# lunarlab-gatech/MorphSym-HGNN

Hardware: NVIDIA B200
Metric: train-step graphs/s (MS-HGNN K4 Mini Cheetah contact, H=128, L=8, fwd+loss+bwd+allreduce+Adam) (higher is better)
Workload: dtype f16x2-split (f32 accumulate)

## Files before the change

include/mshgnn_b200.h:

```cpp
#ifndef MSHGNN_B200_H
#define MSHGNN_B200_H

#include <stdint.h>

#ifdef __cplusplus
extern "C" {
#endif

#define MSHGNN_MAX_NODE_TYPES 4
#define MSHGNN_MAX_EDGE_TYPES 16

#define MSHGNN_OK              0
#define MSHGNN_ERR_ARG        -1
#define MSHGNN_ERR_CUDA       -2
#define MSHGNN_ERR_WORKSPACE  -3

#define MSHGNN_F32 0
#define MSHGNN_F64 1
#define MSHGNN_I64 2
#define MSHGNN_F16 3

#define MSHGNN_MODE_FP32   0
#define MSHGNN_MODE_TC     1
#define MSHGNN_MODE_TC_1X  2

#define MSHGNN_LOSS_MSE 0
#define MSHGNN_LOSS_CE2 1

#define MSHGNN_P_ENC_W   0
#define MSHGNN_P_ENC_B   1
#define MSHGNN_P_REL_W   2
#define MSHGNN_P_REL_B   3
#define MSHGNN_P_ROOT_W  4
#define MSHGNN_P_MLP_W   5
#define MSHGNN_P_MLP_B   6
#define MSHGNN_P_DEC_W   7
#define MSHGNN_P_DEC_B   8

typedef struct mshgnn_plan mshgnn_plan;

typedef struct mshgnn_desc {
    int32_t n_node_types;
    int32_t nodes_per_graph[MSHGNN_MAX_NODE_TYPES];
    int32_t in_width[MSHGNN_MAX_NODE_TYPES];
    int32_t n_edge_types;
    int32_t edge_src_type[MSHGNN_MAX_EDGE_TYPES];
    int32_t edge_dst_type[MSHGNN_MAX_EDGE_TYPES];
    int32_t edge_mean[MSHGNN_MAX_EDGE_TYPES];
    int32_t edge_count[MSHGNN_MAX_EDGE_TYPES];
    const int32_t* edge_src[MSHGNN_MAX_EDGE_TYPES];
    const int32_t* edge_dst[MSHGNN_MAX_EDGE_TYPES];
    int32_t hidden;
    int32_t num_layers;
    int32_t morph_sym;
    int32_t mlp_type;
    int32_t decode_type;
    int32_t out_channels;
    const float* in_sign[MSHGNN_MAX_NODE_TYPES];
    const float* out_sign;
} mshgnn_desc;

int  mshgnn_plan_create(const mshgnn_desc* desc, mshgnn_plan** plan_out);
#define MSHGNN_PLAN_PAD_HIDDEN 1
int  mshgnn_plan_create_ex(const mshgnn_desc* desc, int32_t flags, mshgnn_plan** plan_out);
void mshgnn_plan_destroy(mshgnn_plan* plan);

int64_t mshgnn_param_count(const mshgnn_plan* plan);
int  mshgnn_param_offset(const mshgnn_plan* plan, int32_t kind, int32_t layer, int32_t idx,
                         int64_t* offset_out, int64_t* numel_out);

int64_t mshgnn_workspace_bytes(const mshgnn_plan* plan, int64_t B, int32_t train, int32_t mode);
int64_t mshgnn_out_rows(const mshgnn_plan* plan, int64_t B);

int mshgnn_forward(const mshgnn_plan* plan, int64_t B,
                   const void* const* x, int32_t x_dtype,
                   const float* params, float* out,
                   void* workspace, int64_t workspace_bytes,
                   int32_t train, int32_t mode, void* stream);

int mshgnn_loss(const mshgnn_plan* plan, int64_t B, int32_t loss_kind,
                const float* out, const void* labels, int32_t label_dtype,
                float loss_scale, float* loss_out, float* dout,
                void* workspace, int64_t workspace_bytes, void* stream);

int mshgnn_backward(const mshgnn_plan* plan, int64_t B,
                    const void* const* x, int32_t x_dtype,
                    const float* params, const float* dout, float* grads,
                    void* workspace, int64_t workspace_bytes,
                    int32_t mode, void* stream);

int mshgnn_backward_staged(const mshgnn_plan* plan, int64_t B,
                           const void* const* x, int32_t x_dtype,
                           const float* params, const float* dout, float* grads,
                           void* workspace, int64_t workspace_bytes,
                           int32_t mode, void* stream, void* layers_ready_event);

int mshgnn_input_grad(const mshgnn_plan* plan, int64_t B, const float* params, float* const* dx,
                      void* workspace, int64_t workspace_bytes, int32_t mode, void* stream);

int mshgnn_adam_step(float* params, const float* grads, float* exp_avg, float* exp_avg_sq,
                     int64_t n, int64_t step, float lr, float beta1, float beta2, float eps,
                     float weight_decay, void* stream);
int mshgnn_sgd_step(float* params, const float* grads, int64_t n, float lr, void* stream);

typedef struct mshgnn_window_desc {
    int32_t history_length;
    int32_t seq_cols;
    int32_t label_cols;
    int32_t n_node_types;
    int32_t nodes_per_graph[MSHGNN_MAX_NODE_TYPES];
    int32_t blocks_per_node[MSHGNN_MAX_NODE_TYPES];
    int32_t block_len[MSHGNN_MAX_NODE_TYPES];
    int32_t normalize;
    int32_t n_labels;
    const int32_t* block_col;
    const int32_t* block_sign;
    const int32_t* label_col;
    const int32_t* label_sign;
} mshgnn_window_desc;

int mshgnn_build_windows(const mshgnn_window_desc* desc, const void* seq, const void* label_seq, int32_t seq_dtype,
                         int64_t n_rows, const int64_t* starts, int64_t B, float* const* x, float* y, void* stream);

#define MSHGNN_METRIC_SLOTS   32
#define MSHGNN_METRIC_SCRATCH (296 * 32)
int mshgnn_step_metrics(int32_t loss_kind, int64_t n, int32_t feet, const float* out, const void* labels, int32_t label_dtype,
                        double* batch, double* epoch, double* scratch, void* stream);

#define MSHGNN_METRIC_COM       2
#define MSHGNN_METRIC_GRF_WORLD 3
typedef struct {
    int32_t n_base;
    const double* y_mean;
    const double* y_std;
    const void* quat;
    int32_t quat_dtype;
    int32_t z_only;
} mshgnn_metric_args;
int mshgnn_step_metrics_ex(int32_t kind, const mshgnn_metric_args* args, int64_t n, const float* out, const void* labels,
                           int32_t label_dtype, double* batch, double* epoch, double* scratch, void* stream);

int64_t mshgnn_plan_describe(const mshgnn_plan* plan, char* buf, int64_t cap);

#define MSHGNN_NUM_KERNEL_KINDS 21
int mshgnn_profile_enable(int32_t on);
int mshgnn_profile_read(double* ms_out, int64_t* launches_out, int32_t n);
const char* mshgnn_kernel_kind_name(int32_t kind);

int mshgnn_relu_mask_offset(const mshgnn_plan* plan, int64_t B, int32_t mode, int32_t layer,
                            int64_t* byte_off, int64_t* n_slots, int64_t* rows_padded);

int64_t mshgnn_dw_layout(const mshgnn_plan* plan, int64_t B, int32_t mode, int32_t* out, int64_t cap);

int mshgnn_check_edges(const mshgnn_plan* plan, int64_t B, const int64_t* const* edge_index, int32_t* flag, void* stream);

int mshgnn_set_option(const char* name, int32_t value);
int32_t mshgnn_get_option(const char* name);
int mshgnn_stack_status(const mshgnn_plan* plan, int64_t B, int32_t train, int32_t mode, const void* workspace, int32_t* status_out);
int64_t mshgnn_stack_timing_offset(const mshgnn_plan* plan, int64_t B, int32_t train, int32_t mode);

int64_t mshgnn_launch_count(void);
const char* mshgnn_last_error(void);
const char* mshgnn_version(void);

#ifdef __cplusplus
}
#endif
#endif
```

morphsym-hgnn_b200/csrc/api.cu:

```cuda
#include <algorithm>
#include <atomic>
#include <cmath>
#include <cstdarg>
#include <cstdio>
#include <cstdlib>
#include <cstring>
#include <mutex>
#include <new>
#include <vector>

#include "kernels_simt.cuh"
#include "kernels_tc.cuh"
#include "kernels_enc.cuh"
#include "kernels_dx.cuh"
#include "kernels_stack.cuh"
#include "kernels_stack2.cuh"
#include "kernels_pad.cuh"
#include "plan.cuh"
#include "windows.cuh"
#include "metrics.cuh"

using namespace mshgnn;

struct mshgnn_plan {
    Plan p;
};

namespace {

thread_local char g_err[512] = "";
std::atomic<long long> g_launches{0};

int fail(int code, const char* fmt, ...) {
    va_list ap;
    va_start(ap, fmt);
    vsnprintf(g_err, sizeof g_err, fmt, ap);
    va_end(ap);
    return code;
}

#define CUDA_TRY(expr)                                                                     \
    do {                                                                                   \
        cudaError_t _e = (expr);                                                           \
        if (_e != cudaSuccess)                                                             \
            return fail(MSHGNN_ERR_CUDA, "%s failed: %s (%s:%d)", #expr, cudaGetErrorString(_e), __FILE__, __LINE__); \
    } while (0)

enum Kind : int { K_DERIVE = 0, K_ENC_FWD, K_CONV_FWD, K_MLP_FWD, K_DEC_FWD, K_LOSS, K_DEC_BWD, K_MLP_BWD, K_DX_BWD,
                  K_DW_LAYER, K_DW_ENC, K_REDUCE, K_OPTIM, K_MEMSET, K_WINDOWS, K_METRICS, K_STACK_FWD, K_STACK_BWD, K_EDGES, K_DX_ENC, K_PAD, K_NKINDS };
static_assert(K_NKINDS == MSHGNN_NUM_KERNEL_KINDS, "kernel kind table out of sync with the header");
constexpr int K_NKINDS_V1 = 19;
const char* const kKindNames[MSHGNN_NUM_KERNEL_KINDS] = {
    "derive_weights", "encoder_fwd", "conv_fwd", "base_mlp_fwd", "decoder_fwd", "loss",
    "decoder_bwd", "base_mlp_bwd", "dx_bwd", "dw_layers", "dw_encoder",
    "reduce_partials", "optimizer", "memset", "window_builder", "step_metrics", "stack_fwd", "stack_bwd", "check_edges", "dx_encoder", "pad_params"};
struct ProfRec { int kind; cudaEvent_t a, b; };
std::mutex g_prof_mu;
bool g_prof_on = false;
std::vector<ProfRec> g_prof;
std::vector<cudaEvent_t> g_prof_pool;

struct ProfScope {
    cudaStream_t st; cudaEvent_t a = nullptr, b = nullptr; int kind; bool on;
    ProfScope(int k, cudaStream_t s) : st(s), kind(k), on(g_prof_on) {
        if (!on) return;
        std::lock_guard<std::mutex> lk(g_prof_mu);
        auto get = [&]() { cudaEvent_t e; if (!g_prof_pool.empty()) { e = g_prof_pool.back(); g_prof_pool.pop_back(); } else cudaEventCreate(&e); return e; };
        a = get(); b = get();
        cudaEventRecord(a, st);
    }
    ~ProfScope() {
        if (!on) return;
        cudaEventRecord(b, st);
        std::lock_guard<std::mutex> lk(g_prof_mu);
        g_prof.push_back({kind, a, b});
    }
};

#define LAUNCH_CHECK()                                                                     \
    do {                                                                                   \
        g_launches.fetch_add(1, std::memory_order_relaxed);                                \
        cudaError_t _e = cudaGetLastError();                                               \
        if (_e != cudaSuccess)                                                             \
            return fail(MSHGNN_ERR_CUDA, "kernel launch failed: %s (%s:%d)", cudaGetErrorString(_e), __FILE__, __LINE__); \
    } while (0)

template <typename T>
int upload(const Plan& p, const std::vector<T>& v, T** d) {
    *d = nullptr;
    if (v.empty()) return 0;
    CUDA_TRY(cudaMalloc((void**)d, v.size() * sizeof(T)));
    p.d_allocs.push_back(*d);
    CUDA_TRY(cudaMemcpy(*d, v.data(), v.size() * sizeof(T), cudaMemcpyHostToDevice));
    return 0;
}

int ensure_uploaded(const Plan& p) {
    std::lock_guard<std::mutex> lk(p.mu);
    int dev = -1;
    CUDA_TRY(cudaGetDevice(&dev));
    if (p.uploaded) {
        if (dev != p.device) return fail(MSHGNN_ERR_ARG, "plan tables live on device %d but the current device is %d", p.device, dev);
        return 0;
    }
    int rc;
    if ((rc = upload(p, p.tiles, &p.d_tiles))) return rc;
    if ((rc = upload(p, p.stack_items, &p.d_stack_items))) return rc;
    {
        std::vector<int> tpl;
        for (int e = 0; e < p.n_etypes; ++e) { tpl.insert(tpl.end(), p.e_src[e].begin(), p.e_src[e].end()); tpl.insert(tpl.end(), p.e_dst[e].begin(), p.e_dst[e].end()); }
        if (tpl.empty()) tpl.push_back(0);
        if ((rc = upload(p, tpl, &p.d_edge_tpl))) return rc;
    }
    if ((rc = upload(p, p.rtasks, &p.d_rtasks))) return rc;
    if ((rc = upload(p, p.rpairs, &p.d_rpairs))) return rc;
    if ((rc = upload(p, p.groups, &p.d_groups))) return rc;
    if ((rc = upload(p, p.derive_ops, &p.d_derive))) return rc;
    if ((rc = upload(p, p.derive16_ops, &p.d_derive16))) return rc;
    if ((rc = upload(p, p.signs, &p.d_signs))) return rc;
    if ((rc = upload(p, p.enc_units, &p.d_enc_units))) return rc;
    if ((rc = upload(p, p.enc_groups, &p.d_enc_groups))) return rc;
    if ((rc = upload(p, p.dx_units, &p.d_dx_units))) return rc;
    if ((rc = upload(p, p.pad_segs, &p.d_pad_segs))) return rc;
    p.device = dev;
    p.uploaded = true;
    return 0;
}

void fill_bufs(const Plan& p, const WsLayout& w, char* ws, BufTable& bt) {
    for (int id = 0; id < MAX_BUFS; ++id) bt.p[id] = w.buf[id] < 0 ? nullptr : ws + w.buf[id];
    bt.p[BUF_SIGNS] = p.d_signs;
}

void fill_rows16(const WsLayout& w, BufRows& br) {
    auto row = [](int64_t off) { return off < 0 ? 0 : (int)(off / 256); };
    for (int id = 0; id < MAX_BUFS; ++id) { br.hi[id] = row(w.buf16[id][0]); br.lo[id] = row(w.buf16[id][1]); }
    br.w_hi = row(w.w16[0]); br.w_lo = row(w.w16[1]);
}

__half* image16(char* ws, const WsLayout& w, int id, int i) { return w.buf16[id][i] < 0 ? nullptr : (__half*)(ws + w.buf16[id][i]); }

int launch_rowgemm(int kind, const Plan& p, const Launch& L, const BufTable& bt, int64_t B, int64_t Bp, int x_f64, cudaStream_t st) {
    if (L.count == 0) return 0;
    ProfScope ps(kind, st);
    dim3 grid((unsigned)(Bp / TILE_M), (unsigned)L.count);
    k_rowgemm<<<grid, 256, 0, st>>>(p.d_tiles + L.begin, bt, B, Bp, x_f64);
    LAUNCH_CHECK();
    return 0;
}

typedef CUresult (*EncodeTiledFn)(CUtensorMap*, CUtensorMapDataType, cuuint32_t, void*, const cuuint64_t*, const cuuint64_t*,
                                  const cuuint32_t*, const cuuint32_t*, CUtensorMapInterleave, CUtensorMapSwizzle,
                                  CUtensorMapL2promotion, CUtensorMapFloatOOBfill);

int encode_map(CUtensorMap* m, CUtensorMapDataType type, cuuint32_t rank, const void* base, const cuuint64_t* dims, const cuuint64_t* strides,
               const cuuint32_t* box, CUtensorMapSwizzle sw, const char* what) {
    static EncodeTiledFn enc = nullptr;
    if (!enc) {
        void* ptr = nullptr;
        cudaDriverEntryPointQueryResult qres;
        CUDA_TRY(cudaGetDriverEntryPoint("cuTensorMapEncodeTiled", &ptr, cudaEnableDefault, &qres));
        if (qres != cudaDriverEntryPointSuccess || !ptr) return fail(MSHGNN_ERR_CUDA, "cuTensorMapEncodeTiled is not available in this driver");
        enc = (EncodeTiledFn)ptr;
    }
    static thread_local bool ctx_bound = false;
    if (!ctx_bound) { CUDA_TRY(cudaFree(0)); ctx_bound = true; }
    const cuuint32_t estr[3] = {1, 1, 1};
    CUresult r = enc(m, type, rank, const_cast<void*>(base), dims, strides, box, estr, CU_TENSOR_MAP_INTERLEAVE_NONE,
                     sw, CU_TENSOR_MAP_L2_PROMOTION_L2_256B, CU_TENSOR_MAP_FLOAT_OOB_FILL_NONE);
    if (r != CUDA_SUCCESS) return fail(MSHGNN_ERR_CUDA, "cuTensorMapEncodeTiled%s failed with CUresult %d", what, (int)r);
    return 0;
}

int make_map_2d(CUtensorMap* m, const void* base, int64_t rows, int64_t cols, int box_cols, int box_rows, CUtensorMapSwizzle sw) {
    if (!base || rows < 1) return fail(MSHGNN_ERR_ARG, "internal: bad fp16 tensor for a TMA map");
    const cuuint64_t dims[2] = {(cuuint64_t)cols, (cuuint64_t)rows};
    const cuuint64_t strides[1] = {(cuuint64_t)cols * 2};
    const cuuint32_t box[2] = {(cuuint32_t)box_cols, (cuuint32_t)box_rows};
    return encode_map(m, CU_TENSOR_MAP_DATA_TYPE_FLOAT16, 2, base, dims, strides, box, sw, "");
}

int make_map_x3d(CUtensorMap* m, const void* base, int64_t B, int nodes, int K, int box_rows = 128, int box_cols = 64,
                 CUtensorMapSwizzle sw = CU_TENSOR_MAP_SWIZZLE_NONE) {
    const cuuint64_t dims[3] = {(cuuint64_t)K, (cuuint64_t)nodes, (cuuint64_t)B};
    const cuuint64_t strides[2] = {(cuuint64_t)K * 4, (cuuint64_t)nodes * K * 4};
    const cuuint32_t box[3] = {(cuuint32_t)box_cols, 1, (cuuint32_t)box_rows};
    return encode_map(m, CU_TENSOR_MAP_DATA_TYPE_FLOAT32, 3, base, dims, strides, box, sw, " (features)");
}

struct WsMaps {
    TcMaps tc;
    CUtensorMap dw;
};
int make_ws_maps(WsMaps* m, const void* ws, const WsLayout& w) {
    if (w.total / 256 > 0x7fffffffLL) return fail(MSHGNN_ERR_ARG, "workspace too large for one TMA map");
    int rc;
    if ((rc = make_map_2d(&m->tc.k, ws, w.total / 256, H, TC_KB, 128, CU_TENSOR_MAP_SWIZZLE_64B))) return rc;
    if ((rc = make_map_2d(&m->tc.o, ws, w.total / 256, H, 64, 128, CU_TENSOR_MAP_SWIZZLE_128B))) return rc;
    if ((rc = make_map_2d(&m->dw, ws, w.total / 256, H, 64, DW_KB, CU_TENSOR_MAP_SWIZZLE_128B))) return rc;
    return 0;
}

constexpr int MAX_DEVICES = 64;
int sm_count(int* out) {
    static std::atomic<int> n[MAX_DEVICES];
    int dev = 0;
    CUDA_TRY(cudaGetDevice(&dev));
    int v = dev < MAX_DEVICES ? n[dev].load(std::memory_order_relaxed) : 0;
    if (!v) {
        CUDA_TRY(cudaDeviceGetAttribute(&v, cudaDevAttrMultiProcessorCount, dev));
        if (dev < MAX_DEVICES) n[dev].store(v, std::memory_order_relaxed);
    }
    *out = v;
    return 0;
}
bool first_on_device(std::atomic<bool> (&flags)[MAX_DEVICES]) {
    int dev = 0;
    if (cudaGetDevice(&dev) != cudaSuccess || dev < 0 || dev >= MAX_DEVICES) return true;
    return !flags[dev].exchange(true);
}

static std::atomic<int> g_encoder_kernel{-1}, g_encoder_tpi{0}, g_encoder_dw_tma{-1};

int launch_tc_encoder(const Plan& p, const Launch& L, const WsLayout& w, const BufTable& bt, const BufRows& br, const WsMaps& wm, char* ws,
                      const float* params, int64_t B, int xf64, int split, cudaStream_t st) {
    if (L.count == 0) return 0;
    static std::atomic<bool> attr_set[64];
    static const int which_env = [] { const char* e = getenv("MSHGNN_ENCODER"); return !e ? 0 : (!strcmp(e, "v1") ? 1 : (!strcmp(e, "pair") ? 2 : 0)); }();
    const int which = g_encoder_kernel.load() >= 0 ? g_encoder_kernel.load() : which_env;
    if (first_on_device(attr_set)) {
        CUDA_TRY(cudaFuncSetAttribute(k_tc_encoder, cudaFuncAttributeMaxDynamicSharedMemorySize, ENC_SMEM_BYTES));
        CUDA_TRY(cudaFuncSetAttribute(k_tc_encoder_pair, cudaFuncAttributeMaxDynamicSharedMemorySize, ENCP_SMEM_BYTES));
        CUDA_TRY(cudaFuncSetAttribute(k_tc_encoder_stream, cudaFuncAttributeMaxDynamicSharedMemorySize, ENQ_SMEM_BYTES));
    }
    __half* e_hi = (__half*)(ws + w.wenc16[0]);
    __half* e_lo = (__half*)(ws + w.wenc16[1]);
    EncMaps maps;
    int rc;
    if ((rc = make_map_2d(&maps.w_hi, e_hi, (int64_t)p.n_types * H, p.enc_kmax, 64, 128, CU_TENSOR_MAP_SWIZZLE_128B))) return rc;
    if ((rc = make_map_2d(&maps.w_lo, e_lo, (int64_t)p.n_types * H, p.enc_kmax, 64, 128, CU_TENSOR_MAP_SWIZZLE_128B))) return rc;
    maps.o = wm.tc.o;
    bool stream_ok = xf64 == 0 && L.count <= ENQ_MAX_SLOTS;
    for (int i = 0; i < L.count && stream_ok; ++i) {
        const Chunk& ch = p.tiles[L.begin + i].chunks[0];
        stream_ok = ch.a_buf >= BUF_X0 && ch.a_buf < BUF_X0 + p.n_types && enq_rows_ok(bt.p[ch.a_buf], ch.K, ch.sign_off);
    }
    ProfScope ps(K_ENC_FWD, st);
    const unsigned n_row_tiles = (unsigned)(w.Bp / TILE_M);
    if (which == 1) k_tc_encoder<<<dim3(n_row_tiles, (unsigned)L.count), ENC_THREADS, ENC_SMEM_BYTES, st>>>(maps, p.d_tiles + L.begin, bt, br, B, w.Bp, xf64, split);
    else if (which == 2 || !stream_ok) {
        static const int pf = [] { const char* e = getenv("MSHGNN_ENC_PREFETCH"); return e ? atoi(e) : 0; }();
        k_tc_encoder_pair<<<dim3((n_row_tiles + 1) / 2, (unsigned)L.count), ENC_THREADS, ENCP_SMEM_BYTES, st>>>(maps, p.d_tiles + L.begin, bt, br, B, w.Bp, xf64, split, pf);
    } else {
        int n_sm = 0;
        if ((rc = sm_count(&n_sm))) return rc;
        static const int force_tpi = [] { const char* e = getenv("MSHGNN_ENC_TPI"); return e ? atoi(e) : 0; }();
        const int opt_tpi = g_encoder_tpi.load() ? g_encoder_tpi.load() : force_tpi;
        const int tpi = opt_tpi == 1 || opt_tpi == 2 ? opt_tpi : ((int64_t)L.count * ((n_row_tiles + 1) / 2) >= 4 * (int64_t)n_sm ? 2 : 1);
        const int64_t n_items = (int64_t)L.count * ((n_row_tiles + tpi - 1) / tpi);
        const unsigned grid = (unsigned)(n_items < n_sm ? n_items : n_sm);
        static const int pf_kb = [] { const char* e = getenv("MSHGNN_ENC_PF"); return e ? atoi(e) : 0; }();
        static const int dbg = [] { const char* e = getenv("MSHGNN_ENC_DEBUG"); return e ? atoi(e) : 0; }();
        EnqMaps em;
        em.w_hi = maps.w_hi; em.w_lo = maps.w_lo; em.o = maps.o;
        for (int t = 0; t < p.n_types; ++t) {
            if (p.in_w[t] % 4 || (reinterpret_cast<uintptr_t>(bt.p[BUF_X0 + t]) & 15)) { em.x[t] = maps.o; continue; }
            if ((rc = make_map_x3d(&em.x[t], bt.p[BUF_X0 + t], B, p.nodes[t], p.in_w[t]))) return rc;
        }
        for (int t = p.n_types; t < 4; ++t) em.x[t] = maps.o;
        k_tc_encoder_stream<<<grid, ENQ_THREADS, ENQ_SMEM_BYTES, st>>>(em, p.d_tiles + L.begin, L.count, (int)BUF_X0, bt, br, B, w.Bp, split, (uint32_t*)(ws + w.enc_sync), tpi, pf_kb, dbg);
    }
    LAUNCH_CHECK();
    return 0;
}

int launch_tc_rowgemm(int kind, const Plan& p, const Launch& L, const BufTable& bt, const BufRows& br, const WsMaps& wm,
                      int64_t B, int64_t Bp, int split, cudaStream_t st) {
    if (L.count == 0) return 0;
    static std::atomic<bool> attr_set[64];
    static const bool use_v2 = [] { const char* e = getenv("MSHGNN_ROWGEMM"); return e && !strcmp(e, "tile"); }();
    static const bool use_single = [] { const char* e = getenv("MSHGNN_ROWGEMM"); return e && !strcmp(e, "single"); }();
    if (first_on_device(attr_set)) {
        CUDA_TRY(cudaFuncSetAttribute(k_tc_rowgemm, cudaFuncAttributeMaxDynamicSharedMemorySize, TC_SMEM_BYTES));
        CUDA_TRY(cudaFuncSetAttribute(k_tc_rowgemm_persistent, cudaFuncAttributeMaxDynamicSharedMemorySize, PK_SMEM_BYTES));
        CUDA_TRY(cudaFuncSetAttribute(k_tc_rowgemm_pair, cudaFuncAttributeMaxDynamicSharedMemorySize, PP_SMEM_BYTES));
    }
    for (int i = 0; i < L.count; ++i)
        for (int c = 0; c < p.tiles[L.begin + i].n_chunks; ++c)
            if (p.tiles[L.begin + i].chunks[c].a_kind != A_SLAB)
                return fail(MSHGNN_ERR_ARG, "internal: a tensor-core row-GEMM launch must read slab buffers");
    ProfScope ps(kind, st);
    if (use_v2 || L.count > PK_MAX_TILES) {
        dim3 grid((unsigned)L.count, (unsigned)(Bp / TILE_M));
        k_tc_rowgemm<<<grid, TC_THREADS, TC_SMEM_BYTES, st>>>(wm.tc, p.d_tiles + L.begin, bt, br, B, Bp, split);
    } else {
        int n_sm = 0, rc;
        if ((rc = sm_count(&n_sm))) return rc;
        const bool pair = !use_single && Bp >= 2 * TILE_M && (int64_t)L.count * ((Bp / TILE_M + 1) / 2) >= 4 * (int64_t)n_sm;
        const int64_t n_items = (int64_t)L.count * (pair ? (Bp / TILE_M + 1) / 2 : Bp / TILE_M);
        if (n_items > 0x7fffffffLL) return fail(MSHGNN_ERR_ARG, "batch too large for one row-GEMM launch");
        const unsigned grid = (unsigned)(n_items < n_sm ? n_items : n_sm);
        cudaLaunchConfig_t cfg = {};
        cfg.gridDim = dim3(grid); cfg.blockDim = dim3(PK_THREADS); cfg.dynamicSmemBytes = pair ? PP_SMEM_BYTES : PK_SMEM_BYTES; cfg.stream = st;
        cudaLaunchAttribute at[1];
        at[0].id = cudaLaunchAttributeProgrammaticStreamSerialization;
        at[0].val.programmaticStreamSerializationAllowed = g_prof_on ? 0 : 1;
        cfg.attrs = at; cfg.numAttrs = 1;
        const Tile* d_tiles = p.d_tiles + L.begin;
        const int n_tiles = L.count, n_it = (int)n_items;
        if (pair) CUDA_TRY(cudaLaunchKernelEx(&cfg, k_tc_rowgemm_pair, wm.tc, d_tiles, n_tiles, n_it, bt, br, B, Bp, split));
        else CUDA_TRY(cudaLaunchKernelEx(&cfg, k_tc_rowgemm_persistent, wm.tc, d_tiles, n_tiles, n_it, bt, br, B, Bp, split));
    }
    LAUNCH_CHECK();
    return 0;
}

int launch_tc_dw(int kind, const Plan& p, int layer, const Launch& L, const WsLayout& w, const BufRows& br, const WsMaps& wm, int64_t B, int split,
                 float* part_w, float* part_b, cudaStream_t st) {
    if (L.count == 0) return 0;
    static std::atomic<bool> attr_set[64];
    if (first_on_device(attr_set)) CUDA_TRY(cudaFuncSetAttribute(k_tc_reducegemm, cudaFuncAttributeMaxDynamicSharedMemorySize, DW_SMEM_BYTES));
    for (int i = 0; i < L.count; ++i) {
        const RTask& T = p.rtasks[L.begin + i];
        if (T.n_pairs > DW_MAX_PAIRS) return fail(MSHGNN_ERR_ARG, "internal: weight-gradient task with more than %d pairs", DW_MAX_PAIRS);
        for (int j = 0; j < T.n_pairs; ++j)
            if (p.rpairs[T.pair_begin + j].a_kind != A_SLAB) return fail(MSHGNN_ERR_ARG, "internal: tensor-core weight-gradient task must read slabs");
    }
    ProfScope ps(kind, st);
    dim3 grid((unsigned)L.count, (unsigned)w.dw_ns[layer]);
    k_tc_reducegemm<<<grid, TC_THREADS, DW_SMEM_BYTES, st>>>(wm.dw, p.d_rtasks, p.d_rpairs, L.begin, br, B, w.Bp, w.dw_rows[layer], w.dw_slot0[layer],
                                                             split, part_w, part_b);
    LAUNCH_CHECK();
    return 0;
}

int stack_rows_per_chunk(const Plan& p) {
    static const int env = [] { const char* e = getenv("MSHGNN_STACK_RC"); return e ? atoi(e) : 0; }();
    if (env > 0) return env;
    const int64_t per_row_tile = (int64_t)2 * p.S * TILE_M * H * 4;
    int rc = (int)((int64_t)84 * 1024 * 1024 / per_row_tile);
    return rc < 16 ? 16 : (rc > 64 ? 64 : rc);
}
int stack_delay(const Plan::Stack& sp, int n_row_tiles, int n_sm) {
    static const int env = [] { const char* e = getenv("MSHGNN_STACK_DELAY"); return e ? atoi(e) : 0; }();
    if (env > 0) return env;
    const int per_slot = sp.prog.items_per_row > 0 ? sp.prog.items_per_row : 1;
    int d = (4 * n_sm + per_slot - 1) / per_slot;
    const int most = n_row_tiles / (sp.prog.n_phases > 0 ? sp.prog.n_phases : 1);
    if (d > most) d = most;
    return d < 1 ? 1 : d;
}

int stack_sync_reset(const WsLayout& w, char* ws, cudaStream_t st) {
    if (!w.stack) return 0;
    ProfScope ps(K_MEMSET, st);
    CUDA_TRY(cudaMemsetAsync(ws + w.stack_sync, 0, (size_t)w.stack_sync_bytes, st));
    return 0;
}

int launch_stack(int kind, const Plan& p, const Plan::Stack& sp, const WsLayout& w, const BufTable& bt, const BufRows& br, const WsMaps& wm,
                 char* ws, int64_t B, int split, cudaStream_t st) {
    if (sp.prog.n_phases == 0) return 0;
    static std::atomic<bool> attr_set[64];
    static const bool timing = [] { const char* e = getenv("MSHGNN_STACK_TIMING"); return e && !strcmp(e, "1"); }();
    if (first_on_device(attr_set)) {
        CUDA_TRY(cudaFuncSetAttribute(k_tc_stack<false, false>, cudaFuncAttributeMaxDynamicSharedMemorySize, SK_SMEM_BYTES));
        CUDA_TRY(cudaFuncSetAttribute(k_tc_stack<true, false>, cudaFuncAttributeMaxDynamicSharedMemorySize, SK_SMEM_BYTES));
        CUDA_TRY(cudaFuncSetAttribute(k_tc_stack<false, true>, cudaFuncAttributeMaxDynamicSharedMemorySize, SK_SMEM_BYTES));
        CUDA_TRY(cudaFuncSetAttribute(k_tc_stack<true, true>, cudaFuncAttributeMaxDynamicSharedMemorySize, SK_SMEM_BYTES));
    }
    bool has_priv = false;
    for (int i = 0; i < sp.tiles.count; ++i) {
        const Tile& T = p.tiles[sp.tiles.begin + i];
        has_priv = has_priv || T.priv != 0;
        for (int c = 0; c < T.n_chunks; ++c)
            if (T.chunks[c].a_kind != A_SLAB) return fail(MSHGNN_ERR_ARG, "internal: a stack program must read slab buffers");
    }
    int n_prog_items = 0;
    for (int ph = 0; ph < sp.prog.n_phases; ++ph) n_prog_items = std::max(n_prog_items, sp.prog.first_item[ph] + sp.prog.n_items[ph]);
    for (int i = 0; i < n_prog_items; ++i) {
        const StackItem& it = p.stack_items[sp.item0 + i];
        int chunks = 0;
        for (int st_ = 0; st_ < it.n_steps; ++st_) chunks += p.tiles[sp.tiles.begin + it.tile + st_].n_chunks;
        if (chunks > SK_QCHUNKS || it.n_steps > SK_QSTEPS) return fail(MSHGNN_ERR_ARG, "internal: stack item with %d chunks / %d steps (queue holds %d / %d)", chunks, it.n_steps, SK_QCHUNKS, SK_QSTEPS);
    }
    StackArgs a;
    a.prog = sp.prog;
    a.n_row_tiles = (int)(w.Bp / TILE_M);
    const int64_t n_total = (int64_t)a.n_row_tiles * sp.prog.items_per_row;
    if (n_total > 0x7fffffffLL) return fail(MSHGNN_ERR_ARG, "batch too large for one stack launch");
    a.n_total = (int)n_total;
    a.split = split; a.B = B; a.Bp = w.Bp; a.n_slots = p.S;
    a.sync = (uint32_t*)(ws + w.stack_sync);
    a.err = (uint32_t*)(ws + w.stack_sync + w.stack_sync_bytes - 4);
    a.next = (uint32_t*)(ws + w.stack_sync + w.stack_sync_bytes - 8);
    a.timing = (unsigned long long*)(ws + w.stack_timing);
    a.ws = ws;
    static const int env_dbg = [] { const char* e = getenv("MSHGNN_STACK_DEBUG"); return e ? atoi(e) : 0; }();
    a.debug = env_dbg;
    if ((int64_t)sp.prog.n_phases * a.n_row_tiles * p.S + 2 > w.stack_sync_bytes / 4) return fail(MSHGNN_ERR_WORKSPACE, "internal: stack counters do not fit");
    int n_sm = 0, rc;
    if ((rc = sm_count(&n_sm))) return rc;
    static const bool chunked = [] { const char* e = getenv("MSHGNN_STACK_ORDER"); return !(e && !strcmp(e, "diag")); }();
    static const int env_la = [] { const char* e = getenv("MSHGNN_STACK_LOOKAHEAD"); return e ? atoi(e) : 0; }();
    a.lookahead = env_la > 0 ? (env_la > 4 ? 4 : env_la) : 1;
    a.chunked = chunked ? 1 : 0;
    a.delay = chunked ? stack_rows_per_chunk(p) : stack_delay(sp, a.n_row_tiles, n_sm);
    if (w.stack_pair && !timing) {
        if (a.n_row_tiles & 1) return fail(MSHGNN_ERR_ARG, "internal: the CTA-pair stack kernel needs an even number of row tiles");
        static std::atomic<bool> attr2_set[64];
        static std::atomic<int> max_clusters[64];
        int dev = 0;
        CUDA_TRY(cudaGetDevice(&dev));
        if (first_on_device(attr2_set)) {
            CUDA_TRY(cudaFuncSetAttribute(k_tc_stack2<false>, cudaFuncAttributeMaxDynamicSharedMemorySize, S2_SMEM_BYTES));
            CUDA_TRY(cudaFuncSetAttribute(k_tc_stack2<true>, cudaFuncAttributeMaxDynamicSharedMemorySize, S2_SMEM_BYTES));
        }
        const int64_t n_pairs_total = (int64_t)(a.n_row_tiles / 2) * sp.prog.items_per_row;
        a.n_total = (int)n_pairs_total;
        if (a.chunked) { a.delay = a.delay / 2; if (a.delay < 1) a.delay = 1; }
        else a.delay = stack_delay(sp, a.n_row_tiles / 2, n_sm / 2);
        cudaLaunchConfig_t cfg = {};
        cfg.blockDim = dim3(SK_THREADS); cfg.dynamicSmemBytes = S2_SMEM_BYTES; cfg.stream = st;
        cudaLaunchAttribute at[2];
        at[0].id = cudaLaunchAttributeClusterDimension;
        at[0].val.clusterDim.x = 2; at[0].val.clusterDim.y = 1; at[0].val.clusterDim.z = 1;
        at[1].id = cudaLaunchAttributeProgrammaticStreamSerialization;
        at[1].val.programmaticStreamSerializationAllowed = g_prof_on ? 0 : 1;
        cfg.attrs = at; cfg.numAttrs = 2;
        int mc = dev < 64 ? max_clusters[dev].load(std::memory_order_relaxed) : 0;
        if (!mc) {
            cfg.gridDim = dim3((unsigned)n_sm);
            CUDA_TRY(cudaOccupancyMaxActiveClusters(&mc, k_tc_stack2<true>, &cfg));
            if (mc < 1) return fail(MSHGNN_ERR_CUDA, "the CTA-pair stack kernel does not fit on this device (0 active clusters)");
            if (dev < 64) max_clusters[dev].store(mc, std::memory_order_relaxed);
        }
        const int64_t clusters = n_pairs_total < mc ? n_pairs_total : mc;
        cfg.gridDim = dim3((unsigned)(2 * clusters));
        const Tile* d_tiles = p.d_tiles + sp.tiles.begin;
        const StackItem* d_items = p.d_stack_items + sp.item0;
        ProfScope ps(kind, st);
        if (has_priv) CUDA_TRY(cudaLaunchKernelEx(&cfg, k_tc_stack2<true>, wm.tc, wm.dw, d_tiles, d_items, a, bt, br));
        else CUDA_TRY(cudaLaunchKernelEx(&cfg, k_tc_stack2<false>, wm.tc, wm.dw, d_tiles, d_items, a, bt, br));
        LAUNCH_CHECK();
        return 0;
    }
    ProfScope ps(kind, st);
    cudaLaunchConfig_t cfg = {};
    cfg.gridDim = dim3((unsigned)(n_total < n_sm ? n_total : n_sm)); cfg.blockDim = dim3(SK_THREADS); cfg.dynamicSmemBytes = SK_SMEM_BYTES; cfg.stream = st;
    cudaLaunchAttribute at[1];
    at[0].id = cudaLaunchAttributeProgrammaticStreamSerialization;
    at[0].val.programmaticStreamSerializationAllowed = g_prof_on ? 0 : 1;
    cfg.attrs = at; cfg.numAttrs = 1;
    const Tile* d_tiles = p.d_tiles + sp.tiles.begin;
    const StackItem* d_items = p.d_stack_items + sp.item0;
    if (timing && has_priv) CUDA_TRY(cudaLaunchKernelEx(&cfg, k_tc_stack<true, true>, wm.tc, d_tiles, d_items, a, bt, br));
    else if (timing) CUDA_TRY(cudaLaunchKernelEx(&cfg, k_tc_stack<true, false>, wm.tc, d_tiles, d_items, a, bt, br));
    else if (has_priv) CUDA_TRY(cudaLaunchKernelEx(&cfg, k_tc_stack<false, true>, wm.tc, d_tiles, d_items, a, bt, br));
    else CUDA_TRY(cudaLaunchKernelEx(&cfg, k_tc_stack<false, false>, wm.tc, d_tiles, d_items, a, bt, br));
    LAUNCH_CHECK();
    return 0;
}

int compact_grads(const Plan& p, int first, int count, const float* in, float* ext, cudaStream_t st) {
    if (count == 0) return 0;
    ProfScope ps(K_PAD, st);
    k_compact_grads<<<dim3(PAD_BLOCKS_X, (unsigned)count), 256, 0, st>>>(p.d_pad_segs + first, in, ext);
    LAUNCH_CHECK();
    return 0;
}

float grad_scale(const Plan& p, int64_t B) {
    int e = 0;
    std::frexp((double)(B * p.dec.n_dec), &e);
    return (float)std::ldexp(1.0, e - 1);
}

int check_plan_mode(const mshgnn_plan* plan, int32_t mode) {
    if (!plan) return fail(MSHGNN_ERR_ARG, "plan is NULL");
    if (mode != MSHGNN_MODE_FP32 && mode != MSHGNN_MODE_TC && mode != MSHGNN_MODE_TC_1X) return fail(MSHGNN_ERR_ARG, "unknown mode %d", mode);
    return 0;
}

struct Call {
    const Plan* p = nullptr;
    WsLayout w;
    char* ws = nullptr;
    bool tc = false;
    int split = 0;
    float G = 1.f;
    const float* params = nullptr;
    float* grads = nullptr;
    BufTable bt;
    BufRows br;
    WsMaps wm;
};

int open_call(Call& c, const mshgnn_plan* plan, int64_t B, int train, int32_t mode, void* ws, int64_t ws_bytes) {
    if (B < 1) return fail(MSHGNN_ERR_ARG, "B must be >= 1 (got %lld)", (long long)B);
    const Plan& p = plan->p;
    c.p = &p;
    c.w = ws_layout(p, B, train, mode);
    if (!ws) return fail(MSHGNN_ERR_ARG, "workspace is NULL");
    if (ws_bytes < c.w.total) return fail(MSHGNN_ERR_WORKSPACE, "workspace too small: %lld < %lld bytes", (long long)ws_bytes, (long long)c.w.total);
    if (reinterpret_cast<uintptr_t>(ws) & 255) return fail(MSHGNN_ERR_ARG, "workspace must be 256-byte aligned");
    c.ws = (char*)ws;
    c.tc = mode != MSHGNN_MODE_FP32;
    c.split = mode == MSHGNN_MODE_TC;
    c.G = c.tc ? grad_scale(p, B) : 1.f;
    return 0;
}

int bind_call(Call& c, const float* params, float* grads, const void* const* x) {
    const Plan& p = *c.p;
    int rc;
    if ((rc = ensure_uploaded(p))) return rc;
    if (p.padded) {
        params = (const float*)(c.ws + c.w.pad_params);
        if (grads) grads = (float*)(c.ws + c.w.pad_grads);
    }
    c.params = params;
    c.grads = grads;
    fill_bufs(p, c.w, c.ws, c.bt);
    c.bt.p[BUF_PARAMS] = (void*)params;
    c.bt.p[BUF_GRADS] = grads;
    for (int t = 0; x && t < p.n_types; ++t) {
        if (!x[t]) return fail(MSHGNN_ERR_ARG, "x[%d] is NULL", t);
        c.bt.p[BUF_X0 + t] = (void*)x[t];
    }
    fill_rows16(c.w, c.br);
    if (c.tc && (rc = make_ws_maps(&c.wm, c.ws, c.w))) return rc;
    return 0;
}

int launch_tc_encoder_dw(const Call& c, int64_t B, int xf64, cudaStream_t st) {
    const Plan& p = *c.p;
    const WsLayout& w = c.w;
    const BufTable& bt = c.bt;
    static std::atomic<bool> attr_set[64];
    if (first_on_device(attr_set)) {
        CUDA_TRY(cudaFuncSetAttribute(k_tc_encoder_dw<false>, cudaFuncAttributeMaxDynamicSharedMemorySize, EDW_SMEM_BYTES));
        CUDA_TRY(cudaFuncSetAttribute(k_tc_encoder_dw<true>, cudaFuncAttributeMaxDynamicSharedMemorySize, EDW_SMEM_BYTES));
    }
    static const bool want_xt = [] { const char* e = getenv("MSHGNN_ENC_DW"); return e && !strcmp(e, "tma"); }();
    bool xt = xf64 == 0 && (g_encoder_dw_tma.load() >= 0 ? g_encoder_dw_tma.load() != 0 : want_xt);
    for (const EncDwUnit& eu : p.enc_units)
        if (xt) xt = eu.x_buf >= BUF_X0 && eu.x_buf < BUF_X0 + p.n_types && enq_rows_ok(bt.p[eu.x_buf], eu.K, 0);
    EncXMaps xm;
    int rc;
    for (int t = 0; t < 4; ++t) {
        if (xt && t < p.n_types && p.in_w[t] % 4 == 0 && (reinterpret_cast<uintptr_t>(bt.p[BUF_X0 + t]) & 15) == 0) {
            if ((rc = make_map_x3d(&xm.x[t], bt.p[BUF_X0 + t], B, p.nodes[t], p.in_w[t], 64))) return rc;
        } else xm.x[t] = c.wm.dw;
    }
    float* pe_w = (float*)(c.ws + w.part_enc_w);
    float* pe_b = (float*)(c.ws + w.part_enc_b);
    {
        ProfScope ps(K_DW_ENC, st);
        dim3 grid((unsigned)p.enc_units.size(), (unsigned)w.n_splits_enc);
        if (xt) k_tc_encoder_dw<true><<<grid, ENC_THREADS, EDW_SMEM_BYTES, st>>>(c.wm.dw, xm, (int)BUF_X0, p.d_enc_units, bt, c.br, B, w.Bp, w.rows_per_enc, w.n_splits_enc, xf64,
                                                                                 c.split, pe_w, pe_b);
        else k_tc_encoder_dw<false><<<grid, ENC_THREADS, EDW_SMEM_BYTES, st>>>(c.wm.dw, xm, (int)BUF_X0, p.d_enc_units, bt, c.br, B, w.Bp, w.rows_per_enc, w.n_splits_enc, xf64,
                                                                               c.split, pe_w, pe_b);
        LAUNCH_CHECK();
    }
    {
        ProfScope ps(K_REDUCE, st);
        dim3 grid((unsigned)p.enc_groups.size(), 48);
        k_reduce_enc<<<grid, 256, 0, st>>>(p.d_enc_groups, pe_w, pe_b, w.n_splits_enc, c.grads, 1.f / c.G);
        LAUNCH_CHECK();
    }
    return 0;
}

}

extern "C" {

int mshgnn_plan_create_ex(const mshgnn_desc* desc, int32_t flags, mshgnn_plan** plan_out) {
    if (!plan_out) return fail(MSHGNN_ERR_ARG, "plan_out is NULL");
    *plan_out = nullptr;
    mshgnn_plan* pl = new (std::nothrow) mshgnn_plan();
    if (!pl) return fail(MSHGNN_ERR_ARG, "out of host memory");
    std::string e = build_plan(desc, flags, pl->p);
    if (!e.empty()) { delete pl; return fail(MSHGNN_ERR_ARG, "%s", e.c_str()); }
    *plan_out = pl;
    return 0;
}

int mshgnn_plan_create(const mshgnn_desc* desc, mshgnn_plan** plan_out) { return mshgnn_plan_create_ex(desc, 0, plan_out); }

void mshgnn_plan_destroy(mshgnn_plan* plan) {
    if (!plan) return;
    Plan& p = plan->p;
    for (void* d : p.d_allocs) cudaFree(d);
    delete plan;
}

int64_t mshgnn_param_count(const mshgnn_plan* plan) { return plan ? plan->p.ext.n : -1; }

int mshgnn_param_offset(const mshgnn_plan* plan, int32_t kind, int32_t layer, int32_t idx, int64_t* off, int64_t* numel) {
    if (!plan || !off || !numel) return fail(MSHGNN_ERR_ARG, "NULL argument");
    const Plan& p = plan->p;
    const ParamLayout& y = p.ext;
    const int64_t h = p.hidden;
    auto lay_ok = [&]() { return layer >= 0 && layer < p.L && idx >= 0 && idx < p.n_etypes; };
    switch (kind) {
        case MSHGNN_P_ENC_W: if (idx < 0 || idx >= p.n_types) break; *off = y.enc_w[idx]; *numel = h * p.in_w[idx]; return 0;
        case MSHGNN_P_ENC_B: if (idx < 0 || idx >= p.n_types) break; *off = y.enc_b[idx]; *numel = h; return 0;
        case MSHGNN_P_REL_W: if (!lay_ok()) break; *off = y.rel_w[layer * p.n_etypes + idx]; *numel = h * h; return 0;
        case MSHGNN_P_REL_B: if (!lay_ok()) break; *off = y.rel_b[layer * p.n_etypes + idx]; *numel = h; return 0;
        case MSHGNN_P_ROOT_W: if (!lay_ok()) break; *off = y.root_w[layer * p.n_etypes + idx]; *numel = h * h; return 0;
        case MSHGNN_P_MLP_W: if (!p.morph_sym || idx < 0 || idx > 1) break; *off = y.mlp_w[idx]; *numel = h * h; return 0;
        case MSHGNN_P_MLP_B: if (!p.morph_sym || idx < 0 || idx > 1) break; *off = y.mlp_b[idx]; *numel = h; return 0;
        case MSHGNN_P_DEC_W: *off = y.dec_w; *numel = p.C * h; return 0;
        case MSHGNN_P_DEC_B: *off = y.dec_b; *numel = p.C; return 0;
        default: break;
    }
    return fail(MSHGNN_ERR_ARG, "no such parameter (kind=%d layer=%d idx=%d)", kind, layer, idx);
}

int64_t mshgnn_workspace_bytes(const mshgnn_plan* plan, int64_t B, int32_t train, int32_t mode) {
    if (!plan || B < 1) return -1;
    const WsLayout w = ws_layout(plan->p, B, train, mode);
    if (train && mode != MSHGNN_MODE_FP32 && getenv("MSHGNN_DEBUG_LAYOUT")) {
        fprintf(stderr, "mshgnn layout B=%lld: dW default %d x %d rows, %lld partial slots;", (long long)B, w.n_splits_tc, w.rows_per_tc, (long long)w.part_slots);
        for (size_t l = 0; l < plan->p.dw_layer.size(); ++l) fprintf(stderr, " L%zu[%d tasks]: %d x %d", l, plan->p.dw_layer[l].count, w.dw_ns[l], w.dw_rows[l]);
        fprintf(stderr, "; segments");
        for (int i = 0; i < w.segs.n; ++i) fprintf(stderr, " [tasks %d..%d) x %d @ slot %d", w.segs.begin[i], w.segs.begin[i + 1], w.segs.ns[i], w.segs.base[i]);
        fprintf(stderr, "\n");
    }
    return w.total;
}

int64_t mshgnn_dw_layout(const mshgnn_plan* plan, int64_t B, int32_t mode, int32_t* out, int64_t cap) {
    if (!plan || B < 1 || !out) return -1;
    const Plan& p = plan->p;
    const WsLayout w = ws_layout(p, B, 1, mode);
    const bool tc = mode != MSHGNN_MODE_FP32;
    for (int l = 0; l < p.L && 4 * (int64_t)l + 3 < cap; ++l) {
        out[4 * l] = p.dw_layer[l].count;
        out[4 * l + 1] = tc ? w.dw_ns[l] : w.n_splits;
        out[4 * l + 2] = tc ? w.dw_rows[l] : (int32_t)round_up((B + w.n_splits - 1) / w.n_splits, RG_BK);
        out[4 * l + 3] = w.dw_slot0[l];
    }
    return p.L;
}

int64_t mshgnn_out_rows(const mshgnn_plan* plan, int64_t B) { return plan ? B * plan->p.nodes[plan->p.dec_type] : -1; }

int64_t mshgnn_plan_describe(const mshgnn_plan* plan, char* buf, int64_t cap) {
    if (!plan) return -1;
    const std::string s = describe_plan(plan->p);
    if (buf && cap > 0) {
        const int64_t n = (int64_t)s.size() < cap - 1 ? (int64_t)s.size() : cap - 1;
        memcpy(buf, s.data(), n);
        buf[n] = 0;
    }
    return (int64_t)s.size() + 1;
}

int mshgnn_forward(const mshgnn_plan* plan, int64_t B, const void* const* x, int32_t x_dtype, const float* params,
                   float* out, void* workspace, int64_t workspace_bytes, int32_t train, int32_t mode, void* stream) {
    int rc;
    if ((rc = check_plan_mode(plan, mode))) return rc;
    const Plan& p = plan->p;
    if (x_dtype != MSHGNN_F32 && x_dtype != MSHGNN_F64 && x_dtype != MSHGNN_F16) return fail(MSHGNN_ERR_ARG, "x_dtype must be F32, F64 or F16");
    if (!x || !params || !out) return fail(MSHGNN_ERR_ARG, "NULL argument");
    Call c;
    if ((rc = open_call(c, plan, B, train, mode, workspace, workspace_bytes))) return rc;
    for (int t = 0; t < p.n_types; ++t)
        if (!x[t]) return fail(MSHGNN_ERR_ARG, "x[%d] is NULL", t);
    if ((rc = bind_call(c, params, nullptr, x))) return rc;
    cudaStream_t st = (cudaStream_t)stream;
    const WsLayout& w = c.w;
    const BufTable& bt = c.bt;
    if (p.padded) {
        ProfScope ps(K_PAD, st);
        k_pad_params<<<dim3(PAD_BLOCKS_X, (unsigned)p.pad_segs.size()), 256, 0, st>>>(p.d_pad_segs, params, (float*)c.params);
        LAUNCH_CHECK();
    }
    params = c.params;
    const int xf64 = x_dtype == MSHGNN_F64 ? 1 : (x_dtype == MSHGNN_F16 ? 2 : 0);

    if (!c.tc) {
        {
            ProfScope ps(K_DERIVE, st);
            const unsigned n_ops = (unsigned)p.derive_ops.size();
            if (n_ops > 0) {
                dim3 grid(16, n_ops);
                k_derive<<<grid, 256, 0, st>>>(p.d_derive, params, (float*)bt.p[BUF_DERIVED]);
                LAUNCH_CHECK();
            }
        }
        if ((rc = launch_rowgemm(K_ENC_FWD, p, train ? p.enc_train : p.enc_launch, bt, B, w.Bp, xf64, st))) return rc;
        for (int l = 0; l < p.L; ++l) {
            if ((rc = launch_rowgemm(K_CONV_FWD, p, train ? p.conv_train[l] : p.conv_infer[l], bt, B, w.Bp, 0, st))) return rc;
            if ((rc = launch_rowgemm(K_MLP_FWD, p, (train ? p.mlp1_train[l] : p.mlp1[l]), bt, B, w.Bp, 0, st))) return rc;
            if ((rc = launch_rowgemm(K_MLP_FWD, p, p.mlp2[l], bt, B, w.Bp, 0, st))) return rc;
        }
    } else {
        const BufRows& br = c.br;
        const WsMaps& wm = c.wm;
        __half* w_hi = (__half*)((char*)workspace + w.w16[0]);
        __half* w_lo = (__half*)((char*)workspace + w.w16[1]);
        const int split = c.split;
        {
            ProfScope ps(K_DERIVE, st);
            FwdPrologue fp;
            fp.ops = p.d_derive; fp.n_bias = p.n_derive_bias;
            fp.ops16 = p.d_derive16; fp.n16 = (int)p.derive16_ops.size();
            fp.ed.n_types = p.n_types;
            for (int t = 0; t < p.n_types; ++t) { fp.ed.w_off[t] = p.off_enc_w[t]; fp.ed.K[t] = p.in_w[t]; }
            fp.kmax = p.enc_kmax;
            fp.zero = w.stack ? (uint32_t*)((char*)workspace + w.stack_sync) : nullptr;
            fp.zero_words = w.stack ? w.stack_sync_bytes / 4 : 0;
            fp.zero_blocks = w.stack ? 16 : 0;
            fp.enc_sync = (uint32_t*)((char*)workspace + w.enc_sync);
            const unsigned blocks = (unsigned)(fp.n_bias + 8 * fp.n16 + 64 * p.n_types + fp.zero_blocks);
            k_fwd_prologue<<<blocks, 256, 0, st>>>(fp, params, (float*)bt.p[BUF_DERIVED], w_hi, w_lo, (__half*)((char*)workspace + w.wenc16[0]),
                                                    (__half*)((char*)workspace + w.wenc16[1]));
            LAUNCH_CHECK();
        }
        if ((rc = launch_tc_encoder(p, train ? p.enc_train : p.enc_launch, w, bt, br, wm, (char*)workspace, params, B, xf64, split, st))) return rc;
        if (w.stack) {
            if ((rc = launch_stack(K_STACK_FWD, p, train ? p.stack_train : p.stack_infer, w, bt, br, wm, (char*)workspace, B, split, st))) return rc;
        } else
        for (int l = 0; l < p.L; ++l) {
            if ((rc = launch_tc_rowgemm(K_CONV_FWD, p, train ? p.conv_train[l] : p.conv_infer[l], bt, br, wm, B, w.Bp, split, st))) return rc;
            if ((rc = launch_tc_rowgemm(K_MLP_FWD, p, train ? p.mlp1_train[l] : p.mlp1[l], bt, br, wm, B, w.Bp, split, st))) return rc;
            if ((rc = launch_tc_rowgemm(K_MLP_FWD, p, p.mlp2[l], bt, br, wm, B, w.Bp, split, st))) return rc;
        }
    }
    {
        const int64_t rows = B * p.dec.n_dec;
        int blocks = (int)((rows + 7) / 8);
        if (blocks > 148 * 8) blocks = 148 * 8;
        ProfScope ps(K_DEC_FWD, st);
#define MSHGNN_DEC_FWD(CM) k_decoder_fwd<CM><<<blocks, 256, 0, st>>>(p.dec, (const float*)bt.p[BUF_H0 + p.L], image16(c.ws, w, BUF_H0 + p.L, 0), \
                                              image16(c.ws, w, BUF_H0 + p.L, 1), params, p.d_signs, out, B, w.Bp)
        if (p.dec.C <= 2) MSHGNN_DEC_FWD(2); else if (p.dec.C <= 4) MSHGNN_DEC_FWD(4); else MSHGNN_DEC_FWD(8);
#undef MSHGNN_DEC_FWD
        LAUNCH_CHECK();
    }
    return 0;
}

int mshgnn_loss(const mshgnn_plan* plan, int64_t B, int32_t loss_kind, const float* out, const void* labels,
                int32_t label_dtype, float loss_scale, float* loss_out, float* dout, void* workspace,
                int64_t workspace_bytes, void* stream) {
    if (!plan) return fail(MSHGNN_ERR_ARG, "plan is NULL");
    const Plan& p = plan->p;
    if (!out || !labels || !loss_out || !workspace) return fail(MSHGNN_ERR_ARG, "NULL argument");
    if (B < 1) return fail(MSHGNN_ERR_ARG, "B must be >= 1");
    if (label_dtype < 0 || label_dtype > 2) return fail(MSHGNN_ERR_ARG, "bad label_dtype");
    if (loss_kind == MSHGNN_LOSS_CE2 && p.C != 2) return fail(MSHGNN_ERR_ARG, "CE2 loss needs out_channels == 2");
    if (loss_kind != MSHGNN_LOSS_CE2 && loss_kind != MSHGNN_LOSS_MSE) return fail(MSHGNN_ERR_ARG, "bad loss_kind");
    if (workspace_bytes < LOSS_BLOCKS * 8) return fail(MSHGNN_ERR_WORKSPACE, "workspace too small for the loss partials");
    cudaStream_t st = (cudaStream_t)stream;
    double* partial = (double*)((char*)workspace + ((workspace_bytes - LOSS_BLOCKS * 8) & ~(int64_t)255));
    const int64_t rows = B * p.dec.n_dec;
    const int64_t n = loss_kind == MSHGNN_LOSS_MSE ? rows * p.C : rows;
    int blocks = (int)((n + 255) / 256);
    if (blocks > LOSS_BLOCKS) blocks = LOSS_BLOCKS;
    ProfScope ps(K_LOSS, st);
    k_loss_partial<<<blocks, 256, 0, st>>>(loss_kind, out, labels, label_dtype, n, loss_scale / (float)n, dout, partial);
    LAUNCH_CHECK();
    k_loss_final<<<1, 32, 0, st>>>(partial, blocks, 1.0 / (double)n, loss_kind == MSHGNN_LOSS_CE2, loss_out);
    LAUNCH_CHECK();
    return 0;
}

int mshgnn_backward(const mshgnn_plan* plan, int64_t B, const void* const* x, int32_t x_dtype, const float* params,
                    const float* dout, float* grads, void* workspace, int64_t workspace_bytes, int32_t mode, void* stream) {
    return mshgnn_backward_staged(plan, B, x, x_dtype, params, dout, grads, workspace, workspace_bytes, mode, stream, nullptr);
}

int mshgnn_backward_staged(const mshgnn_plan* plan, int64_t B, const void* const* x, int32_t x_dtype, const float* params,
                           const float* dout, float* grads, void* workspace, int64_t workspace_bytes, int32_t mode, void* stream,
                           void* layers_ready_event) {
    int rc;
    if ((rc = check_plan_mode(plan, mode))) return rc;
    const Plan& p = plan->p;
    if (x_dtype != MSHGNN_F32 && x_dtype != MSHGNN_F64 && x_dtype != MSHGNN_F16) return fail(MSHGNN_ERR_ARG, "x_dtype must be F32, F64 or F16");
    if (!x || !params || !dout) return fail(MSHGNN_ERR_ARG, "NULL argument");
    const bool want_dw = grads != nullptr;
    Call c;
    if ((rc = open_call(c, plan, B, 1, mode, workspace, workspace_bytes))) return rc;
    if ((rc = bind_call(c, params, grads, x))) return rc;
    float* const grads_out = grads;
    grads = c.grads;
    params = c.params;
    cudaStream_t st = (cudaStream_t)stream;
    const WsLayout& w = c.w;
    const BufTable& bt = c.bt;
    const BufRows& br = c.br;
    const WsMaps& wm = c.wm;
    char* ws = c.ws;
    const bool tc = c.tc;
    const int split = c.split;
    const float G = c.G;
    const int xf64 = x_dtype == MSHGNN_F64 ? 1 : (x_dtype == MSHGNN_F16 ? 2 : 0);
    float* part_w = (float*)(ws + w.part_w);
    float* part_b = (float*)(ws + w.part_b);
    float* dec_part = (float*)(ws + w.dec_part);

    if (!want_dw) {
        if ((rc = stack_sync_reset(w, ws, st))) return rc;
    } else if (w.stack && (reinterpret_cast<uintptr_t>(grads) & 15) == 0) {
        ProfScope ps(K_MEMSET, st);
        const int64_t n4 = p.n_params / 4;
        k_bwd_prologue<<<296, 256, 0, st>>>((float4*)grads, n4, grads + n4 * 4, (int)(p.n_params - n4 * 4), (uint32_t*)(ws + w.stack_sync), w.stack_sync_bytes / 4);
        LAUNCH_CHECK();
    } else {
        { ProfScope ps(K_MEMSET, st); CUDA_TRY(cudaMemsetAsync(grads, 0, (size_t)p.n_params * 4, st)); }
        if ((rc = stack_sync_reset(w, ws, st))) return rc;
    }

    {
        const int L = p.L;
        const bool want_dh = p.morph_sym, want_dc = !p.morph_sym || p.dec_type != p.mlp_type;
        const int dhb = BUF_DHL0 + L, dcb = BUF_DCL0 + L - 1;
        float* dh = want_dh ? (float*)bt.p[dhb] : nullptr;
        float* dc = want_dc ? (float*)bt.p[dcb] : nullptr;
        const int mk = want_dc ? MK_BITS : MK_NONE;
        const void* mbuf = want_dc ? bt.p[BUF_MASK0 + L - 1] : nullptr;
        ProfScope ps(K_DEC_BWD, st);
#define MSHGNN_DEC_BWD(CM) k_decoder_bwd<CM><<<DEC_BLOCKS, 256, 0, st>>>(p.dec, (const float*)bt.p[BUF_H0 + L], image16(ws, w, BUF_H0 + L, 0), \
                                                  image16(ws, w, BUF_H0 + L, 1), params, p.d_signs, dout, dh, dc, mk, mbuf, dec_part, B, w.Bp, G, \
                                                  want_dh ? image16(ws, w, dhb, 0) : nullptr, want_dh ? image16(ws, w, dhb, 1) : nullptr, \
                                                  want_dc ? image16(ws, w, dcb, 0) : nullptr, want_dc ? image16(ws, w, dcb, 1) : nullptr)
        if (p.dec.C <= 2) MSHGNN_DEC_BWD(2); else if (p.dec.C <= 4) MSHGNN_DEC_BWD(4); else MSHGNN_DEC_BWD(8);
#undef MSHGNN_DEC_BWD
        LAUNCH_CHECK();
        if (want_dw) {
            k_decoder_bwd_reduce<<<p.dec.C * H + p.dec.C, 256, 0, st>>>(p.dec, dec_part, DEC_BLOCKS, grads, 1.f / G);
            LAUNCH_CHECK();
        }
    }
    const int ngl = p.n_groups_layers, nge = (int)p.groups.size() - ngl;
    auto reduce_layers = [&]() -> int {
        if (ngl > 0 && want_dw) {
            dim3 grid((unsigned)ngl, 64);
            ProfScope ps(K_REDUCE, st);
            k_reduce_partials<<<grid, 256, 0, st>>>(p.d_groups, part_w, part_b, w.segs, grads, 1.f / G);
            LAUNCH_CHECK();
        }
        return 0;
    };
    if (tc) {
        if (w.stack) {
            if ((rc = launch_stack(K_STACK_BWD, p, p.stack_bwd, w, bt, br, wm, ws, B, split, st))) return rc;
            if (want_dw && w.dw_merged) {
                Launch all{p.dw_layer[p.L - 1].begin, 0};
                for (int l = 0; l < p.L; ++l) all.count += p.dw_layer[l].count;
                if ((rc = launch_tc_dw(K_DW_LAYER, p, p.L - 1, all, w, br, wm, B, split, part_w, part_b, st))) return rc;
            } else if (want_dw) {
                for (int l = p.L - 1; l >= 0; --l)
                    if ((rc = launch_tc_dw(K_DW_LAYER, p, l, p.dw_layer[l], w, br, wm, B, split, part_w, part_b, st))) return rc;
            }
        } else {
            for (int l = p.L - 1; l >= 0; --l) {
                if ((rc = launch_tc_rowgemm(K_MLP_BWD, p, p.bwd_m1[l], bt, br, wm, B, w.Bp, split, st))) return rc;
                if ((rc = launch_tc_rowgemm(K_MLP_BWD, p, p.bwd_m2[l], bt, br, wm, B, w.Bp, split, st))) return rc;
                if (want_dw && (rc = launch_tc_dw(K_DW_LAYER, p, l, p.dw_layer[l], w, br, wm, B, split, part_w, part_b, st))) return rc;
                if ((rc = launch_tc_rowgemm(K_DX_BWD, p, p.bwd_dx[l], bt, br, wm, B, w.Bp, split, st))) return rc;
            }
        }
        if ((rc = reduce_layers())) return rc;
        if (p.padded && want_dw && (rc = compact_grads(p, p.n_pad_enc, (int)p.pad_segs.size() - p.n_pad_enc, grads, grads_out, st))) return rc;
        if (layers_ready_event) CUDA_TRY(cudaEventRecord((cudaEvent_t)layers_ready_event, st));
        if (!p.enc_units.empty() && want_dw && (rc = launch_tc_encoder_dw(c, B, xf64, st))) return rc;
        if (p.padded && want_dw && (rc = compact_grads(p, 0, p.n_pad_enc, grads, grads_out, st))) return rc;
    } else {
        auto launch_dw = [&](int kind, const Launch& L) -> int {
            if (L.count == 0 || !want_dw) return 0;
            ProfScope ps(kind, st);
            dim3 grid((unsigned)L.count, (unsigned)w.n_splits);
            k_reducegemm<<<grid, 256, 0, st>>>(p.d_rtasks, p.d_rpairs, L.begin, bt, B, w.Bp, xf64, w.n_splits, part_w, part_b);
            LAUNCH_CHECK();
            return 0;
        };
        for (int l = p.L - 1; l >= 0; --l) {
            if ((rc = launch_rowgemm(K_MLP_BWD, p, p.bwd_m1[l], bt, B, w.Bp, 0, st))) return rc;
            if ((rc = launch_rowgemm(K_MLP_BWD, p, p.bwd_m2[l], bt, B, w.Bp, 0, st))) return rc;
            if ((rc = launch_dw(K_DW_LAYER, p.dw_layer[l]))) return rc;
            if ((rc = launch_rowgemm(K_DX_BWD, p, p.bwd_dx[l], bt, B, w.Bp, 0, st))) return rc;
        }
        if ((rc = launch_dw(K_DW_ENC, p.dw_enc))) return rc;
        if ((rc = reduce_layers())) return rc;
        if (nge > 0 && want_dw) {
            dim3 grid((unsigned)nge, 32);
            ProfScope ps(K_REDUCE, st);
            k_reduce_partials<<<grid, 256, 0, st>>>(p.d_groups + ngl, part_w, part_b, w.segs, grads, 1.f / G);
            LAUNCH_CHECK();
        }
        if (p.padded && want_dw && (rc = compact_grads(p, 0, (int)p.pad_segs.size(), grads, grads_out, st))) return rc;
        if (layers_ready_event) CUDA_TRY(cudaEventRecord((cudaEvent_t)layers_ready_event, st));
    }
    return 0;
}

int mshgnn_input_grad(const mshgnn_plan* plan, int64_t B, const float* params, float* const* dx, void* workspace, int64_t workspace_bytes,
                      int32_t mode, void* stream) {
    int rc;
    if ((rc = check_plan_mode(plan, mode))) return rc;
    const Plan& p = plan->p;
    if (!params || !dx) return fail(MSHGNN_ERR_ARG, "NULL argument");
    Call c;
    if ((rc = open_call(c, plan, B, 1, mode, workspace, workspace_bytes))) return rc;
    DxOut o;
    memset(&o, 0, sizeof o);
    unsigned n_kb = 1;
    bool any = false;
    for (int t = 0; t < p.n_types; ++t) {
        if (dx[t] && (reinterpret_cast<uintptr_t>(dx[t]) & 3)) return fail(MSHGNN_ERR_ARG, "dx[%d] must be 4-byte aligned", t);
        o.p[t] = dx[t]; o.nodes[t] = p.nodes[t]; o.w_off[t] = p.off_enc_w[t];
        n_kb = std::max(n_kb, (unsigned)((p.in_w[t] + 63) / 64));
        any = any || dx[t];
    }
    if (!any) return 0;
    if ((rc = bind_call(c, params, nullptr, nullptr))) return rc;
    cudaStream_t st = (cudaStream_t)stream;
    const WsLayout& w = c.w;
    const unsigned n_units = (unsigned)p.dx_units.size();
    if (!c.tc) {
        ProfScope ps(K_DX_ENC, st);
        k_encoder_dx<<<dim3((unsigned)((B + 15) / 16), n_units, n_kb), 256, 0, st>>>(p.d_dx_units, o, (const float*)c.bt.p[BUF_DCL0 - 1], c.params, p.d_signs, B, w.Bp);
        LAUNCH_CHECK();
        return 0;
    }
    static std::atomic<bool> attr_set[64];
    if (first_on_device(attr_set)) CUDA_TRY(cudaFuncSetAttribute(k_tc_encoder_dx, cudaFuncAttributeMaxDynamicSharedMemorySize, DX_SMEM_BYTES));
    DxMaps maps;
    maps.a = c.wm.tc.o;
    if ((rc = make_map_2d(&maps.w_hi, c.ws + w.wenc16[0], (int64_t)p.n_types * H, p.enc_kmax, 64, 64, CU_TENSOR_MAP_SWIZZLE_128B))) return rc;
    if ((rc = make_map_2d(&maps.w_lo, c.ws + w.wenc16[1], (int64_t)p.n_types * H, p.enc_kmax, 64, 64, CU_TENSOR_MAP_SWIZZLE_128B))) return rc;
    for (int t = 0; t < 4; ++t) {
        maps.x[t] = c.wm.tc.o;
        if (t < p.n_types && dx[t] && enq_rows_ok(dx[t], p.in_w[t], -1)) {
            if ((rc = make_map_x3d(&maps.x[t], dx[t], B, p.nodes[t], p.in_w[t], 128, 32, CU_TENSOR_MAP_SWIZZLE_128B))) return rc;
            o.tma |= 1 << t;
        }
    }
    const float scale = TC_W_UNSCALE / c.G;
    ProfScope ps(K_DX_ENC, st);
    k_tc_encoder_dx<<<dim3((unsigned)(w.Bp / TILE_M), n_units), DX_THREADS, DX_SMEM_BYTES, st>>>(maps, p.d_dx_units, o, p.d_signs, c.br.hi[BUF_DC1_ID],
                                                                                               c.br.lo[BUF_DC1_ID], B, w.Bp, c.split, scale);
    LAUNCH_CHECK();
    return 0;
}

int mshgnn_adam_step(float* params,const float* grads, float* exp_avg, float* exp_avg_sq, int64_t n, int64_t step,
                     float lr, float beta1, float beta2, float eps, float weight_decay, void* stream) {
    if (!params || !grads || !exp_avg || !exp_avg_sq || n < 1 || step < 1) return fail(MSHGNN_ERR_ARG, "bad argument");
    const float bc1 = 1.f - (float)std::pow((double)beta1, (double)step);
    const float bc2s = (float)std::sqrt(1.0 - std::pow((double)beta2, (double)step));
    int blocks = (int)((n + 255) / 256);
    if (blocks > 148 * 8) blocks = 148 * 8;
    ProfScope ps(K_OPTIM, (cudaStream_t)stream);
    k_adam<<<blocks, 256, 0, (cudaStream_t)stream>>>(params, grads, exp_avg, exp_avg_sq, n, lr, beta1, beta2, eps, weight_decay, bc1, bc2s);
    LAUNCH_CHECK();
    return 0;
}

int mshgnn_sgd_step(float* params, const float* grads, int64_t n, float lr, void* stream) {
    if (!params || !grads || n < 1) return fail(MSHGNN_ERR_ARG, "bad argument");
    int blocks = (int)((n + 255) / 256);
    if (blocks > 148 * 8) blocks = 148 * 8;
    ProfScope ps(K_OPTIM, (cudaStream_t)stream);
    k_sgd<<<blocks, 256, 0, (cudaStream_t)stream>>>(params, grads, n, lr);
    LAUNCH_CHECK();
    return 0;
}

int mshgnn_build_windows(const mshgnn_window_desc* d, const void* seq, const void* label_seq, int32_t seq_dtype, int64_t n_rows,
                         const int64_t* starts, int64_t B, float* const* x, float* y, void* stream) {
    if (!d || !seq || !starts || !x || B < 1) return fail(MSHGNN_ERR_ARG, "bad argument");
    if (seq_dtype != MSHGNN_F32 && seq_dtype != MSHGNN_F64) return fail(MSHGNN_ERR_ARG, "seq_dtype must be F32 or F64");
    const int T = d->history_length, C = d->seq_cols;
    if (T < 1 || (d->normalize && T < 2)) return fail(MSHGNN_ERR_ARG, "history_length %d unsupported (normalisation needs >= 2 rows)", T);
    if (C < 1 || C > WIN_MAX_COLS) return fail(MSHGNN_ERR_ARG, "seq_cols %d outside [1, %d]", C, WIN_MAX_COLS);
    if (n_rows < T) return fail(MSHGNN_ERR_ARG, "sequence has %lld rows, fewer than history_length %d", (long long)n_rows, T);
    if (d->n_node_types < 1 || d->n_node_types > 4) return fail(MSHGNN_ERR_ARG, "n_node_types out of range");
    if (d->n_labels < 0 || d->n_labels > WIN_MAX_LABELS) return fail(MSHGNN_ERR_ARG, "n_labels out of range");
    if (y && d->n_labels > 0 && (!label_seq || d->label_cols < 1 || !d->label_col)) return fail(MSHGNN_ERR_ARG, "labels requested without a label sequence");
    WindowTable tb;
    memset(&tb, 0, sizeof tb);
    tb.T = T; tb.C = C; tb.CL = d->label_cols; tb.n_types = d->n_node_types; tb.normalize = d->normalize != 0;
    tb.n_labels = y ? d->n_labels : 0;
    WindowPtrs out;
    memset(&out, 0, sizeof out);
    int nb = 0;
    for (int t = 0; t < d->n_node_types; ++t) {
        const int nodes = d->nodes_per_graph[t], blocks = d->blocks_per_node[t], len = d->block_len[t];
        if (nodes < 0 || blocks < 0 || (nodes * blocks > 0 && len != T && len != 1)) return fail(MSHGNN_ERR_ARG, "type %d: bad block shape", t);
        if (nodes * blocks > 0 && !x[t]) return fail(MSHGNN_ERR_ARG, "type %d: null output", t);
        tb.nodes[t] = nodes; tb.blocks[t] = blocks > 0 ? blocks : 1; tb.blen[t] = len; tb.first_block[t] = nb;
        out.x[t] = x[t];
        if (nb + nodes * blocks > WIN_MAX_BLOCKS) return fail(MSHGNN_ERR_ARG, "more than %d feature blocks per graph", WIN_MAX_BLOCKS);
        for (int i = 0; i < nodes * blocks; ++i) {
            const int c = d->block_col[nb + i], sg = d->block_sign ? d->block_sign[nb + i] : 1;
            if (c >= C) return fail(MSHGNN_ERR_ARG, "block %d reads column %d of a %d-column sequence", nb + i, c, C);
            if (c >= 0 && len != T) return fail(MSHGNN_ERR_ARG, "type %d: a constant-length block cannot read a column", t);
            if (sg < -127 || sg > 127) return fail(MSHGNN_ERR_ARG, "block factor out of range");
            tb.col[nb + i] = (int16_t)(c < 0 ? -1 : c); tb.sign[nb + i] = (int8_t)sg;
            if (c >= 0) tb.col_used[c] = 1;
        }
        nb += nodes * blocks;
    }
    tb.n_blocks = nb;
    for (int i = 0; i < tb.n_labels; ++i) {
        const int c = d->label_col[i];
        if (c < 0 || c >= d->label_cols) return fail(MSHGNN_ERR_ARG, "label column out of range");
        tb.label_col[i] = (int16_t)c; tb.label_sign[i] = (int8_t)(d->label_sign ? d->label_sign[i] : 1);
    }
    cudaStream_t st = (cudaStream_t)stream;
    const int Tp = T | 1;
    const size_t esz = seq_dtype == MSHGNN_F64 ? 8 : 4;
    const int vw = (int)(16 / esz);
    const int Cp = (C + vw - 1) / vw * vw;
    if (Cp / vw > WIN_THREADS) return fail(MSHGNN_ERR_ARG, "seq_cols exceeds the CTA size");
    const int nrg = std::min(WIN_THREADS / (Cp / vw), WIN_MAX_RG);
    const size_t nz_bytes = (std::max((size_t)C * Tp * 4, (size_t)nrg * Cp * 16) + 127) / 128 * 128;
    const size_t smem = nz_bytes + (size_t)T * Cp * esz;
    if (smem > 200 * 1024) return fail(MSHGNN_ERR_ARG, "window of %d x %d does not fit in shared memory", T, C);
    const int bulk = ((size_t)C * esz) % 16 == 0 && ((uintptr_t)seq % 16) == 0 && ((size_t)T * C * esz) < (1u << 20);
    int dev = 0, sms = 148;
    CUDA_TRY(cudaGetDevice(&dev));
    CUDA_TRY(cudaDeviceGetAttribute(&sms, cudaDevAttrMultiProcessorCount, dev));
    const int per_sm = (int)std::max<size_t>(1, std::min<size_t>(8, (220 * 1024) / (smem + 1024)));
    const int grid = (int)std::min<int64_t>(B, (int64_t)sms * per_sm);
    ProfScope ps(K_WINDOWS, st);
    if (seq_dtype == MSHGNN_F64) {
        CUDA_TRY(cudaFuncSetAttribute(k_build_windows<double>, cudaFuncAttributeMaxDynamicSharedMemorySize, (int)smem));
        k_build_windows<double><<<grid, WIN_THREADS, smem, st>>>(tb, (const double*)seq, (const double*)label_seq, n_rows, starts, B, out, y, bulk, (int)nz_bytes);
    } else {
        CUDA_TRY(cudaFuncSetAttribute(k_build_windows<float>, cudaFuncAttributeMaxDynamicSharedMemorySize, (int)smem));
        k_build_windows<float><<<grid, WIN_THREADS, smem, st>>>(tb, (const float*)seq, (const float*)label_seq, n_rows, starts, B, out, y, bulk, (int)nz_bytes);
    }
    LAUNCH_CHECK();
    return 0;
}

int mshgnn_step_metrics(int32_t loss_kind, int64_t n, int32_t feet, const float* out, const void* labels, int32_t label_dtype,
                        double* batch, double* epoch, double* scratch, void* stream) {
    if (!out || !labels || !batch || !scratch || n < 1) return fail(MSHGNN_ERR_ARG, "bad argument");
    if (loss_kind != MSHGNN_LOSS_MSE && loss_kind != MSHGNN_LOSS_CE2) return fail(MSHGNN_ERR_ARG, "bad loss_kind");
    if (loss_kind == MSHGNN_LOSS_CE2 && (feet < 1 || feet > 4)) return fail(MSHGNN_ERR_ARG, "classification metrics need 1..4 rows per graph");
    if (label_dtype < 0 || label_dtype > 2) return fail(MSHGNN_ERR_ARG, "bad label_dtype");
    cudaStream_t st = (cudaStream_t)stream;
    int blocks = (int)((n + 255) / 256);
    if (blocks > MET_BLOCKS) blocks = MET_BLOCKS;
    ProfScope ps(K_METRICS, st);
    k_metrics_partial<<<blocks, 256, 0, st>>>(loss_kind, feet, out, labels, label_dtype, n, scratch);
    LAUNCH_CHECK();
    k_metrics_final<<<1, 32, 0, st>>>(loss_kind, scratch, blocks, batch, epoch);
    LAUNCH_CHECK();
    return 0;
}

int mshgnn_step_metrics_ex(int32_t kind, const mshgnn_metric_args* args, int64_t n, const float* out, const void* labels,
                           int32_t label_dtype, double* batch, double* epoch, double* scratch, void* stream) {
    if (!args || !out || !labels || !batch || !scratch || n < 1) return fail(MSHGNN_ERR_ARG, "bad argument");
    if (kind != MSHGNN_METRIC_COM && kind != MSHGNN_METRIC_GRF_WORLD) return fail(MSHGNN_ERR_ARG, "bad metric kind");
    if (label_dtype < 0 || label_dtype > 2) return fail(MSHGNN_ERR_ARG, "bad label_dtype");
    if (kind == MSHGNN_METRIC_COM) {
        if (args->n_base < 1 || args->n_base > 4) return fail(MSHGNN_ERR_ARG, "COM metrics need n_base in 1..4");
        if (!args->y_mean || !args->y_std) return fail(MSHGNN_ERR_ARG, "COM metrics need y_mean and y_std");
    } else {
        if (!args->quat) return fail(MSHGNN_ERR_ARG, "world-frame GRF metrics need the quaternions");
        if (args->quat_dtype != MSHGNN_F32 && args->quat_dtype != MSHGNN_F64) return fail(MSHGNN_ERR_ARG, "bad quat_dtype");
    }
    cudaStream_t st = (cudaStream_t)stream;
    int blocks = (int)((n + 255) / 256);
    if (blocks > MET_BLOCKS) blocks = MET_BLOCKS;
    ProfScope ps(K_METRICS, st);
    k_metrics_partial_ex<<<blocks, 256, 0, st>>>(kind, *args, out, labels, label_dtype, n, scratch);
    LAUNCH_CHECK();
    k_metrics_final<<<1, 32, 0, st>>>(kind, scratch, blocks, batch, epoch);
    LAUNCH_CHECK();
    return 0;
}

int mshgnn_profile_enable(int32_t on) {
    std::lock_guard<std::mutex> lk(g_prof_mu);
    g_prof_on = on != 0;
    return 0;
}

int mshgnn_profile_read(double* ms_out, int64_t* launches_out, int32_t n) {
    if (!ms_out || !launches_out || n < K_NKINDS_V1) return fail(MSHGNN_ERR_ARG, "bad argument");
    std::vector<ProfRec> recs;
    {
        std::lock_guard<std::mutex> lk(g_prof_mu);
        recs.swap(g_prof);
    }
    for (int i = 0; i < n; ++i) { ms_out[i] = 0.0; launches_out[i] = 0; }
    for (auto& r : recs) {
        CUDA_TRY(cudaEventSynchronize(r.b));
        float ms = 0.f;
        CUDA_TRY(cudaEventElapsedTime(&ms, r.a, r.b));
        if (r.kind < n) { ms_out[r.kind] += ms; launches_out[r.kind] += 1; }
    }
    std::lock_guard<std::mutex> lk(g_prof_mu);
    for (auto& r : recs) { g_prof_pool.push_back(r.a); g_prof_pool.push_back(r.b); }
    return 0;
}

const char* mshgnn_kernel_kind_name(int32_t kind) {
    return (kind >= 0 && kind < MSHGNN_NUM_KERNEL_KINDS) ? kKindNames[kind] : "";
}

int mshgnn_relu_mask_offset(const mshgnn_plan* plan, int64_t B, int32_t mode, int32_t layer, int64_t* byte_off, int64_t* n_slots,
                            int64_t* rows_padded) {
    if (!plan || !byte_off || !n_slots || !rows_padded || B < 1) return fail(MSHGNN_ERR_ARG, "bad argument");
    const Plan& p = plan->p;
    if (layer < -1 || layer >= p.L) return fail(MSHGNN_ERR_ARG, "layer out of range");
    const WsLayout w = ws_layout(p, B, 1, mode);
    *byte_off = w.buf[layer < 0 ? BUF_MASKE : BUF_MASK0 + layer];
    *n_slots = layer < 0 ? p.S : p.S + p.nm;
    *rows_padded = w.Bp;
    return 0;
}

int mshgnn_check_edges(const mshgnn_plan* plan, int64_t B, const int64_t* const* edge_index, int32_t* flag, void* stream) {
    if (!plan || !edge_index || !flag || B < 1) return fail(MSHGNN_ERR_ARG, "bad argument");
    const Plan& p = plan->p;
    int rc;
    if ((rc = ensure_uploaded(p))) return rc;
    EdgeCheck ec;
    memset(&ec, 0, sizeof ec);
    ec.n_etypes = p.n_etypes;
    int off = 0;
    int64_t most = 0;
    for (int e = 0; e < p.n_etypes; ++e) {
        ec.E[e] = (int)p.e_src[e].size();
        ec.n_src[e] = p.nodes[p.e_src_t[e]]; ec.n_dst[e] = p.nodes[p.e_dst_t[e]];
        ec.tpl_off[e] = off; off += 2 * ec.E[e];
        if (ec.E[e] > 0 && !edge_index[e]) return fail(MSHGNN_ERR_ARG, "edge_index[%d] is NULL", e);
        ec.ei[e] = (const long long*)edge_index[e];
        most = std::max<int64_t>(most, (int64_t)ec.E[e] * B);
    }
    if (most == 0) return 0;
    cudaStream_t st = (cudaStream_t)stream;
    const unsigned blocks = (unsigned)std::min<int64_t>((most + 1023) / 1024, 148 * 4);
    ProfScope ps(K_EDGES, st);
    k_check_edges<<<dim3(blocks, (unsigned)p.n_etypes), 256, 0, st>>>(ec, p.d_edge_tpl, (long long)B, flag);
    LAUNCH_CHECK();
    return 0;
}

int mshgnn_set_option(const char* name, int32_t value) {
    if (!name) return fail(MSHGNN_ERR_ARG, "option name is NULL");
    if (!strcmp(name, "stack")) { set_stack_enabled(value); return 0; }
    if (!strcmp(name, "stack_pair")) { set_stack_pair_mode(value); return 0; }
    if (!strcmp(name, "encoder")) { g_encoder_kernel.store(value < 0 || value > 2 ? -1 : value); return 0; }
    if (!strcmp(name, "encoder_tpi")) { g_encoder_tpi.store(value == 1 || value == 2 ? value : 0); return 0; }
    if (!strcmp(name, "encoder_dw_tma")) { g_encoder_dw_tma.store(value < 0 ? -1 : (value ? 1 : 0)); return 0; }
    return fail(MSHGNN_ERR_ARG, "unknown option '%s'", name);
}

int32_t mshgnn_get_option(const char* name) {
    if (name && !strcmp(name, "stack")) return stack_enabled() ? 1 : 0;
    if (name && !strcmp(name, "stack_pair")) return stack_pair_mode();
    if (name && !strcmp(name, "encoder")) return g_encoder_kernel.load();
    if (name && !strcmp(name, "encoder_tpi")) return g_encoder_tpi.load();
    if (name && !strcmp(name, "encoder_dw_tma")) return g_encoder_dw_tma.load();
    return -1;
}

int mshgnn_stack_status(const mshgnn_plan* plan, int64_t B, int32_t train, int32_t mode, const void* workspace, int32_t* status_out) {
    if (!plan || !workspace || !status_out || B < 1) return fail(MSHGNN_ERR_ARG, "bad argument");
    const WsLayout w = ws_layout(plan->p, B, train, mode);
    *status_out = 0;
    if (!w.stack) return 0;
    uint32_t word = 0;
    CUDA_TRY(cudaMemcpy(&word, (const char*)workspace + w.stack_sync + w.stack_sync_bytes - 4, 4, cudaMemcpyDeviceToHost));
    *status_out = word ? 1 : 0;
    return 0;
}

int64_t mshgnn_stack_timing_offset(const mshgnn_plan* plan, int64_t B, int32_t train, int32_t mode) {
    if (!plan || B < 1) return -1;
    const WsLayout w = ws_layout(plan->p, B, train, mode);
    return w.stack ? w.stack_timing : -1;
}

int64_t mshgnn_launch_count(void) { return g_launches.load(); }
const char* mshgnn_last_error(void) { return g_err; }
const char* mshgnn_version(void) { return "mshgnn_b200 0.1 (sm_100a)"; }

}
```

morphsym-hgnn_b200/csrc/kernels_simt.cuh:

```cuda
#pragma once
#include "../../include/mshgnn_b200.h"
#include "common.cuh"

namespace mshgnn {

__device__ __forceinline__ float ld_x(const void* base, int dtype_f64, int64_t idx) {
    if (dtype_f64 == 2) return __half2float(__ldg((const __half*)base + idx));
    return dtype_f64 ? (float)__ldg((const double*)base + idx) : __ldg((const float*)base + idx);
}

__device__ __forceinline__ void split_store4(__half* hi, __half* lo, int64_t off, const float (&v)[4]) {
    __half2 h[2], l[2];
#pragma unroll
    for (int j = 0; j < 2; ++j) {
        const __half ha = __float2half_rn(v[2 * j]), hb = __float2half_rn(v[2 * j + 1]);
        h[j] = __halves2half2(ha, hb);
        l[j] = __halves2half2(__float2half_rn((v[2 * j] - __half2float(ha)) * LO_SCALE), __float2half_rn((v[2 * j + 1] - __half2float(hb)) * LO_SCALE));
    }
    *reinterpret_cast<uint2*>(hi + off) = *reinterpret_cast<uint2*>(h);
    *reinterpret_cast<uint2*>(lo + off) = *reinterpret_cast<uint2*>(l);
}

__device__ __forceinline__ float4 load_h4(const float* slab, const __half* hi, const __half* lo, int64_t off) {
    if (slab) return *reinterpret_cast<const float4*>(slab + off);
    const uint2 a = *reinterpret_cast<const uint2*>(hi + off), b = *reinterpret_cast<const uint2*>(lo + off);
    const float2 a0 = __half22float2(*reinterpret_cast<const __half2*>(&a.x)), a1 = __half22float2(*reinterpret_cast<const __half2*>(&a.y));
    const float2 b0 = __half22float2(*reinterpret_cast<const __half2*>(&b.x)), b1 = __half22float2(*reinterpret_cast<const __half2*>(&b.y));
    const float u = 1.f / LO_SCALE;
    return make_float4(fmaf(b0.x, u, a0.x), fmaf(b0.y, u, a0.y), fmaf(b1.x, u, a1.x), fmaf(b1.y, u, a1.y));
}

constexpr int RG_BK = 16;
constexpr int RG_AS = TILE_M + 4;

struct RgRegs {
    float a[2][4];
    float4 w[2];
};

__device__ __forceinline__ void rg_load(const Tile& t, const BufTable& bt, int c, int k0, int row0, int64_t B,
                                        int64_t Bp, int x_f64, int tid, RgRegs& r) {
    const Chunk& ch = t.chunks[c];
    const int ak = (tid & 3) * 4;
    const int K = ch.K;
#pragma unroll
    for (int h = 0; h < 2; ++h) {
        const int64_t row = row0 + (tid >> 2) + 64 * h;
        float v0 = 0.f, v1 = 0.f, v2 = 0.f, v3 = 0.f;
        if (row < B) {
            const int k = k0 + ak;
            if (ch.a_kind == A_SLAB) {
                const float* p = (const float*)bt.p[ch.a_buf] + ((int64_t)ch.a_slot * Bp + row) * H + k;
                const float4 q = *reinterpret_cast<const float4*>(p);
                v0 = q.x; v1 = q.y; v2 = q.z; v3 = q.w;
            } else {
                const int64_t idx = row * (int64_t)ch.lda + ch.a_off + k;
                const void* xb = bt.p[ch.a_buf];
                const float* pf = (const float*)xb + idx;
                if (x_f64 == 0 && k + 3 < K && ((reinterpret_cast<uintptr_t>(pf) & 15) == 0)) {
                    const float4 q = __ldg(reinterpret_cast<const float4*>(pf));
                    v0 = q.x; v1 = q.y; v2 = q.z; v3 = q.w;
                } else {
                    if (k + 0 < K) v0 = ld_x(xb, x_f64, idx + 0);
                    if (k + 1 < K) v1 = ld_x(xb, x_f64, idx + 1);
                    if (k + 2 < K) v2 = ld_x(xb, x_f64, idx + 2);
                    if (k + 3 < K) v3 = ld_x(xb, x_f64, idx + 3);
                }
                if (ch.sign_off >= 0) {
                    const float* s = (const float*)bt.p[2] + ch.sign_off + k;
                    if (k + 0 < K) v0 *= __ldg(s + 0);
                    if (k + 1 < K) v1 *= __ldg(s + 1);
                    if (k + 2 < K) v2 *= __ldg(s + 2);
                    if (k + 3 < K) v3 *= __ldg(s + 3);
                }
            }
        }
        r.a[h][0] = v0; r.a[h][1] = v1; r.a[h][2] = v2; r.a[h][3] = v3;
    }
    const float* W = (const float*)bt.p[ch.w_buf] + ch.w_off;
#pragma unroll
    for (int h = 0; h < 2; ++h) {
        const int k = k0 + (tid >> 5) + 8 * h;
        r.w[h] = (k < K) ? __ldg(reinterpret_cast<const float4*>(W + (int64_t)k * H + (tid & 31) * 4))
                         : make_float4(0.f, 0.f, 0.f, 0.f);
    }
}

__global__ void __launch_bounds__(256, 2)
k_rowgemm(const Tile* __restrict__ tiles, const BufTable bt, const int64_t B, const int64_t Bp, const int x_f64) {
    __shared__ Tile t;
    __shared__ __align__(16) float As[RG_BK][RG_AS];
    __shared__ __align__(16) float Ws[RG_BK][H];

    const int tid = threadIdx.x;
    {
        const int* src = reinterpret_cast<const int*>(tiles + blockIdx.y);
        int* dst = reinterpret_cast<int*>(&t);
        for (int i = tid; i < (int)(sizeof(Tile) / 4); i += 256) dst[i] = src[i];
    }
    __syncthreads();

    const int row0 = blockIdx.x * TILE_M;
    const int tx = tid & 15, ty = tid >> 4;
    float acc[8][8];
#pragma unroll
    for (int i = 0; i < 8; ++i)
#pragma unroll
        for (int j = 0; j < 8; ++j) acc[i][j] = 0.f;

    int c = 0, k0 = 0;
    RgRegs r;
    const int nch = t.n_chunks;
    if (nch > 0) rg_load(t, bt, 0, 0, row0, B, Bp, x_f64, tid, r);
    bool more = nch > 0;
    while (more) {
        {
            const int ak = (tid & 3) * 4;
#pragma unroll
            for (int h = 0; h < 2; ++h) {
                const int rr = (tid >> 2) + 64 * h;
#pragma unroll
                for (int i = 0; i < 4; ++i) As[ak + i][rr] = r.a[h][i];
                *reinterpret_cast<float4*>(&Ws[(tid >> 5) + 8 * h][(tid & 31) * 4]) = r.w[h];
            }
        }
        __syncthreads();
        k0 += RG_BK;
        if (k0 >= t.chunks[c].K) { ++c; k0 = 0; }
        more = c < nch;
        if (more) rg_load(t, bt, c, k0, row0, B, Bp, x_f64, tid, r);
#pragma unroll
        for (int k = 0; k < RG_BK; ++k) {
            const float4 a0 = *reinterpret_cast<const float4*>(&As[k][ty * 4]);
            const float4 a1 = *reinterpret_cast<const float4*>(&As[k][64 + ty * 4]);
            const float4 b0 = *reinterpret_cast<const float4*>(&Ws[k][tx * 4]);
            const float4 b1 = *reinterpret_cast<const float4*>(&Ws[k][64 + tx * 4]);
            const float a[8] = {a0.x, a0.y, a0.z, a0.w, a1.x, a1.y, a1.z, a1.w};
            const float b[8] = {b0.x, b0.y, b0.z, b0.w, b1.x, b1.y, b1.z, b1.w};
#pragma unroll
            for (int i = 0; i < 8; ++i)
#pragma unroll
                for (int j = 0; j < 8; ++j) acc[i][j] = fmaf(a[i], b[j], acc[i][j]);
        }
        __syncthreads();
    }

    float bias[8];
#pragma unroll
    for (int j = 0; j < 8; ++j) bias[j] = 0.f;
    if (t.bias_buf >= 0) {
        const float* bp = (const float*)bt.p[t.bias_buf] + t.bias_off;
        const float4 q0 = __ldg(reinterpret_cast<const float4*>(bp + tx * 4));
        const float4 q1 = __ldg(reinterpret_cast<const float4*>(bp + 64 + tx * 4));
        bias[0] = q0.x; bias[1] = q0.y; bias[2] = q0.z; bias[3] = q0.w;
        bias[4] = q1.x; bias[5] = q1.y; bias[6] = q1.z; bias[7] = q1.w;
    }
    const int lane_shift = (tx & 7) * 4;
#pragma unroll
    for (int i = 0; i < 8; ++i) {
        const int64_t row = row0 + ty * 4 + (i & 3) + (i >> 2) * 64;
        const bool live = row < B;
#pragma unroll
        for (int hh = 0; hh < 2; ++hh) {
            const int col = tx * 4 + 64 * hh;
            float v[4];
            unsigned nib = 0;
#pragma unroll
            for (int j = 0; j < 4; ++j) {
                float x = acc[i][hh * 4 + j] + bias[hh * 4 + j];
                if (x > 0.f) nib |= 1u << j;
                if (t.relu) x = fmaxf(x, 0.f);
                v[j] = x;
            }
            if (t.mask_out_buf >= 0) {
                unsigned word = nib << lane_shift;
                word |= __shfl_xor_sync(0xffffffffu, word, 1);
                word |= __shfl_xor_sync(0xffffffffu, word, 2);
                word |= __shfl_xor_sync(0xffffffffu, word, 4);
                if (live && (tx & 7) == 0) {
                    unsigned* mp = (unsigned*)bt.p[t.mask_out_buf] + ((int64_t)t.mask_out_slot * Bp + row) * 4 + hh * 2 + (tx >> 3);
                    *mp = word;
                }
            }
            if (!live) continue;
            if (t.posmask_buf >= 0) {
                const unsigned w = *((const unsigned*)bt.p[t.posmask_buf] +
                                     ((int64_t)t.posmask_slot * Bp + row) * 4 + hh * 2 + (tx >> 3));
                const unsigned nb = (w >> lane_shift) & 0xFu;
#pragma unroll
                for (int j = 0; j < 4; ++j) v[j] = ((nb >> j) & 1u) ? v[j] : 0.f;
            }
            if (t.res_buf >= 0) {
                const float4 q = *reinterpret_cast<const float4*>(
                    (const float*)bt.p[t.res_buf] + ((int64_t)t.res_slot * Bp + row) * H + col);
                v[0] += q.x; v[1] += q.y; v[2] += q.z; v[3] += q.w;
            }
            if (t.out_buf >= 0) {
                const int64_t off = ((int64_t)t.out_slot * Bp + row) * H + col;
                *reinterpret_cast<float4*>((float*)bt.p[t.out_buf] + off) = make_float4(v[0], v[1], v[2], v[3]);
            }
            if (t.out2_buf >= 0) {
                if (t.out2_mask_kind == MK_BITS) {
                    const unsigned w = *((const unsigned*)bt.p[t.out2_mask_buf] +
                                         ((int64_t)t.out2_mask_slot * Bp + row) * 4 + hh * 2 + (tx >> 3));
                    const unsigned nb = (w >> lane_shift) & 0xFu;
#pragma unroll
                    for (int j = 0; j < 4; ++j) v[j] = ((nb >> j) & 1u) ? v[j] : 0.f;
                }
                const int64_t off2 = ((int64_t)t.out2_slot * Bp + row) * H + col;
                *reinterpret_cast<float4*>((float*)bt.p[t.out2_buf] + off2) = make_float4(v[0], v[1], v[2], v[3]);
            }
        }
    }
}

struct RdRegs {
    float4 d[2];
    float4 a[2];
};

__device__ __forceinline__ void rd_load(const RPair& p, const RTask& t, const BufTable& bt, int64_t r0, int64_t r_end,
                                        int64_t Bp, int x_f64, int tid, RdRegs& r) {
    const int col = (tid & 31) * 4;
#pragma unroll
    for (int h = 0; h < 2; ++h) {
        const int64_t row = r0 + (tid >> 5) + 8 * h;
        float4 d = make_float4(0.f, 0.f, 0.f, 0.f), a = d;
        if (row < r_end) {
            d = *reinterpret_cast<const float4*>((const float*)bt.p[p.d_buf] + ((int64_t)p.d_slot * Bp + row) * H + col);
            if (p.a_kind == A_SLAB) {
                a = *reinterpret_cast<const float4*>((const float*)bt.p[p.a_buf] + ((int64_t)p.a_slot * Bp + row) * H + col);
            } else {
                const int k = t.k0 + col;
                const int64_t idx = row * (int64_t)p.lda + p.a_off + k;
                const void* xb = bt.p[p.a_buf];
                const float* pf = (const float*)xb + idx;
                float v[4] = {0.f, 0.f, 0.f, 0.f};
                if (x_f64 == 0 && k + 3 < t.K && ((reinterpret_cast<uintptr_t>(pf) & 15) == 0)) {
                    const float4 q = __ldg(reinterpret_cast<const float4*>(pf));
                    v[0] = q.x; v[1] = q.y; v[2] = q.z; v[3] = q.w;
                } else {
#pragma unroll
                    for (int j = 0; j < 4; ++j)
                        if (k + j < t.K) v[j] = ld_x(xb, x_f64, idx + j);
                }
                if (p.sign_off >= 0) {
                    const float* s = (const float*)bt.p[2] + p.sign_off + k;
#pragma unroll
                    for (int j = 0; j < 4; ++j)
                        if (k + j < t.K) v[j] *= __ldg(s + j);
                }
                a = make_float4(v[0], v[1], v[2], v[3]);
            }
        }
        r.d[h] = d; r.a[h] = a;
    }
}

__global__ void __launch_bounds__(256, 2)
k_reducegemm(const RTask* __restrict__ tasks, const RPair* __restrict__ pairs, const int task0, const BufTable bt,
             const int64_t B, const int64_t Bp, const int x_f64, const int n_splits,
             float* __restrict__ part_w, float* __restrict__ part_b) {
    __shared__ __align__(16) float Ds[RG_BK][H];
    __shared__ __align__(16) float As[RG_BK][H];
    __shared__ RTask t;
    const int tid = threadIdx.x;
    const int task = task0 + blockIdx.x;
    if (tid < (int)(sizeof(RTask) / 4)) reinterpret_cast<int*>(&t)[tid] = reinterpret_cast<const int*>(tasks + task)[tid];
    __syncthreads();

    const int split = blockIdx.y;
    const int64_t rows_per = round_up((B + n_splits - 1) / n_splits, RG_BK);
    const int64_t r_begin = split * rows_per;
    const int64_t r_end = (r_begin + rows_per < B) ? (r_begin + rows_per) : B;
    const int64_t n_steps_pair = (r_end > r_begin) ? (r_end - r_begin + RG_BK - 1) / RG_BK : 0;

    const int tx = tid & 15, ty = tid >> 4;
    float acc[8][8];
#pragma unroll
    for (int i = 0; i < 8; ++i)
#pragma unroll
        for (int j = 0; j < 8; ++j) acc[i][j] = 0.f;
    float cs = 0.f;

    float* pw = part_w + ((int64_t)task * n_splits + split) * (H * H);
    const int64_t total = n_steps_pair * t.n_pairs;
    RdRegs r;
    int64_t step = 0;
    if (total > 0) rd_load(pairs[t.pair_begin], t, bt, r_begin, r_end, Bp, x_f64, tid, r);
    while (step < total) {
#pragma unroll
        for (int h = 0; h < 2; ++h) {
            *reinterpret_cast<float4*>(&Ds[(tid >> 5) + 8 * h][(tid & 31) * 4]) = r.d[h];
            *reinterpret_cast<float4*>(&As[(tid >> 5) + 8 * h][(tid & 31) * 4]) = r.a[h];
        }
        __syncthreads();
        ++step;
        if (step < total) {
            const int pi = (int)(step / n_steps_pair);
            const int64_t r0 = r_begin + (step % n_steps_pair) * RG_BK;
            rd_load(pairs[t.pair_begin + pi], t, bt, r0, r_end, Bp, x_f64, tid, r);
        }
#pragma unroll
        for (int k = 0; k < RG_BK; ++k) {
            const float4 d0 = *reinterpret_cast<const float4*>(&Ds[k][ty * 4]);
            const float4 d1 = *reinterpret_cast<const float4*>(&Ds[k][64 + ty * 4]);
            const float4 a0 = *reinterpret_cast<const float4*>(&As[k][tx * 4]);
            const float4 a1 = *reinterpret_cast<const float4*>(&As[k][64 + tx * 4]);
            const float d[8] = {d0.x, d0.y, d0.z, d0.w, d1.x, d1.y, d1.z, d1.w};
            const float a[8] = {a0.x, a0.y, a0.z, a0.w, a1.x, a1.y, a1.z, a1.w};
#pragma unroll
            for (int i = 0; i < 8; ++i)
#pragma unroll
                for (int j = 0; j < 8; ++j) acc[i][j] = fmaf(d[i], a[j], acc[i][j]);
        }
        if (t.want_colsum && tid < H) {
#pragma unroll
            for (int k = 0; k < RG_BK; ++k) cs += Ds[k][tid];
        }
        __syncthreads();
    }
#pragma unroll
    for (int i = 0; i < 8; ++i) {
        const int o = ty * 4 + (i & 3) + (i >> 2) * 64;
        *reinterpret_cast<float4*>(pw + o * H + tx * 4) = make_float4(acc[i][0], acc[i][1], acc[i][2], acc[i][3]);
        *reinterpret_cast<float4*>(pw + o * H + 64 + tx * 4) = make_float4(acc[i][4], acc[i][5], acc[i][6], acc[i][7]);
    }
    if (t.want_colsum && tid < H) part_b[((int64_t)task * n_splits + split) * H + tid] = cs;
}

__global__ void __launch_bounds__(256)
k_reduce_partials(const OutGroup* __restrict__ groups, const float* __restrict__ part_w,
                  const float* __restrict__ part_b, const __grid_constant__ PartSegs segs,
                  float* __restrict__ grads, const float rscale) {
    const OutGroup g = groups[blockIdx.x];
    if (g.kind == 0) {
        const int per = (H * H) / gridDim.y;
        for (int e = blockIdx.y * per + threadIdx.x; e < (blockIdx.y + 1) * per; e += 256) {
            const int o = e / H, i = e % H;
            if (g.k0 + i >= g.K) continue;
            double sd = 0.0;
            for (int ti = 0; ti < g.n_tasks; ++ti) {
                int64_t slot0; int n_splits;
                part_lookup(segs, g.tasks[ti], slot0, n_splits);
                const float* p = part_w + slot0 * (H * H) + e;
                int sp = 0;
                for (; sp + 16 <= n_splits; sp += 16) {
                    float v[16];
#pragma unroll
                    for (int j = 0; j < 16; ++j) v[j] = __ldg(p + (int64_t)(sp + j) * (H * H));
#pragma unroll
                    for (int j = 0; j < 16; ++j) sd += (double)v[j];
                }
                for (; sp + 8 <= n_splits; sp += 8) {
                    float v[8];
#pragma unroll
                    for (int j = 0; j < 8; ++j) v[j] = __ldg(p + (int64_t)(sp + j) * (H * H));
#pragma unroll
                    for (int j = 0; j < 8; ++j) sd += (double)v[j];
                }
                for (; sp < n_splits; ++sp) sd += (double)__ldg(p + (int64_t)sp * (H * H));
            }
            const float s = (float)(sd * (double)g.scale * (double)rscale);
            for (int oi = 0; oi < g.n_outs; ++oi) grads[(int64_t)g.outs[oi] + (int64_t)o * g.K + g.k0 + i] = s;
        }
    } else {
        if (blockIdx.y != 0) return;
        for (int e = threadIdx.x; e < H; e += 256) {
            double sd = 0.0;
            for (int ti = 0; ti < g.n_tasks; ++ti) {
                int64_t slot0; int n_splits;
                part_lookup(segs, g.tasks[ti], slot0, n_splits);
                const float* p = part_b + slot0 * H + e;
                for (int sp = 0; sp < n_splits; ++sp) sd += (double)p[(int64_t)sp * H];
            }
            const float s = (float)(sd * (double)g.scale * (double)rscale);
            for (int oi = 0; oi < g.n_outs; ++oi) grads[(int64_t)g.outs[oi] + e] = s;
        }
    }
}

__global__ void __launch_bounds__(256)
k_derive(const DeriveOp* __restrict__ ops, const float* __restrict__ params, float* __restrict__ derived) {
    const DeriveOp op = ops[blockIdx.y];
    const int n = op.rows * op.cols;
    for (int e = blockIdx.x * 256 + threadIdx.x; e < n; e += gridDim.x * 256) {
        int r, c;
        if (op.transpose) { c = e / op.rows; r = e % op.rows; } else { r = e / op.cols; c = e % op.cols; }
        float s = 0.f;
        for (int i = 0; i < op.n_src; ++i) s += params[(int64_t)op.src_off[i] + (int64_t)r * op.cols + c];
        derived[(int64_t)op.dst_off + e] = s;
    }
}

template <int CMAX>
__global__ void __launch_bounds__(256)
k_decoder_fwd(const DecoderDesc dd, const float* __restrict__ hslab, const __half* __restrict__ h_hi, const __half* __restrict__ h_lo,
              const float* __restrict__ params, const float* __restrict__ signs, float* __restrict__ out, const int64_t B, const int64_t Bp) {
    const int lane = threadIdx.x & 31;
    const int64_t warp = (int64_t)blockIdx.x * 8 + (threadIdx.x >> 5);
    const int64_t n_rows = B * dd.n_dec;
    const int64_t stride = (int64_t)gridDim.x * 8;
    float4 w[CMAX];
#pragma unroll
    for (int c = 0; c < CMAX; ++c)
        w[c] = (c < dd.C) ? __ldg(reinterpret_cast<const float4*>(params + dd.w_off + c * H + lane * 4))
                          : make_float4(0.f, 0.f, 0.f, 0.f);
#pragma unroll 2
    for (int64_t row = warp; row < n_rows; row += stride) {
        const int64_t g = row / dd.n_dec;
        const int j = (int)(row % dd.n_dec);
        const float4 h = load_h4(hslab, h_hi, h_lo, ((int64_t)dd.slots[j] * Bp + g) * H + lane * 4);
#pragma unroll
        for (int c = 0; c < CMAX; ++c) {
            if (c >= dd.C) break;
            float s = h.x * w[c].x + h.y * w[c].y + h.z * w[c].z + h.w * w[c].w;
#pragma unroll
            for (int o = 16; o > 0; o >>= 1) s += __shfl_xor_sync(0xffffffffu, s, o);
            if (lane == 0) {
                float v = s + __ldg(params + dd.b_off + c);
                if (dd.sign_off >= 0) v *= __ldg(signs + dd.sign_off + j * dd.C + c);
                out[row * dd.C + c] = v;
            }
        }
    }
}

template <int CMAX>
__global__ void __launch_bounds__(256)
k_decoder_bwd(const DecoderDesc dd, const float* __restrict__ hslab, const __half* __restrict__ h_hi, const __half* __restrict__ h_lo,
              const float* __restrict__ params,
              const float* __restrict__ signs, const float* __restrict__ dout,
              float* __restrict__ dh, float* __restrict__ dc, const int mask_kind, const void* __restrict__ mask_buf,
              float* __restrict__ part, const int64_t B, const int64_t Bp, const float gscale,
              __half* __restrict__ dh_hi, __half* __restrict__ dh_lo, __half* __restrict__ dc_hi, __half* __restrict__ dc_lo) {
    __shared__ float red[8][CMAX][H + 1];
    __shared__ float redb[8][CMAX];
    const int lane = threadIdx.x & 31, wid = threadIdx.x >> 5;
    const int64_t warp = (int64_t)blockIdx.x * 8 + wid;
    const int64_t n_rows = B * dd.n_dec;
    const int64_t stride = (int64_t)gridDim.x * 8;
    float4 w[CMAX], gw[CMAX];
    float gb[CMAX];
#pragma unroll
    for (int c = 0; c < CMAX; ++c) {
        w[c] = (c < dd.C) ? __ldg(reinterpret_cast<const float4*>(params + dd.w_off + c * H + lane * 4))
                          : make_float4(0.f, 0.f, 0.f, 0.f);
        gw[c] = make_float4(0.f, 0.f, 0.f, 0.f);
        gb[c] = 0.f;
    }
#pragma unroll 2
    for (int64_t row = warp; row < n_rows; row += stride) {
        const int64_t g = row / dd.n_dec;
        const int j = (int)(row % dd.n_dec);
        const int64_t off = ((int64_t)dd.slots[j] * Bp + g) * H + lane * 4;
        const float4 h = load_h4(hslab, h_hi, h_lo, off);
        float4 d = make_float4(0.f, 0.f, 0.f, 0.f);
#pragma unroll
        for (int c = 0; c < CMAX; ++c) {
            if (c >= dd.C) break;
            float dv = __ldg(dout + row * dd.C + c) * gscale;
            if (dd.sign_off >= 0) dv *= __ldg(signs + dd.sign_off + j * dd.C + c);
            d.x = fmaf(dv, w[c].x, d.x); d.y = fmaf(dv, w[c].y, d.y);
            d.z = fmaf(dv, w[c].z, d.z); d.w = fmaf(dv, w[c].w, d.w);
            gw[c].x = fmaf(dv, h.x, gw[c].x); gw[c].y = fmaf(dv, h.y, gw[c].y);
            gw[c].z = fmaf(dv, h.z, gw[c].z); gw[c].w = fmaf(dv, h.w, gw[c].w);
            gb[c] += dv;
        }
        if (dh) *reinterpret_cast<float4*>(dh + off) = d;
        if (dh_hi) { const float vv[4] = {d.x, d.y, d.z, d.w}; split_store4(dh_hi, dh_lo, off, vv); }
        if (dc || dc_hi) {
            if (mask_kind == MK_BITS) {
                const unsigned wd = *((const unsigned*)mask_buf + ((int64_t)dd.slots[j] * Bp + g) * 4 + (lane >> 3));
                const unsigned nb = (wd >> ((lane & 7) * 4)) & 0xFu;
                d.x = (nb & 1u) ? d.x : 0.f; d.y = (nb & 2u) ? d.y : 0.f;
                d.z = (nb & 4u) ? d.z : 0.f; d.w = (nb & 8u) ? d.w : 0.f;
            }
            if (dc) *reinterpret_cast<float4*>(dc + off) = d;
            if (dc_hi) { const float vv[4] = {d.x, d.y, d.z, d.w}; split_store4(dc_hi, dc_lo, off, vv); }
        }
    }
    if (dh_hi || dc_hi) {
        const int64_t pad = Bp - B;
        const float z[4] = {0.f, 0.f, 0.f, 0.f};
        for (int64_t r = warp; r < pad * dd.n_dec; r += stride) {
            const int64_t off = ((int64_t)dd.slots[r / pad] * Bp + B + r % pad) * H + lane * 4;
            if (dh_hi) split_store4(dh_hi, dh_lo, off, z);
            if (dc_hi) split_store4(dc_hi, dc_lo, off, z);
        }
    }
#pragma unroll
    for (int c = 0; c < CMAX; ++c) {
        if (c >= dd.C) break;
        red[wid][c][lane * 4 + 0] = gw[c].x; red[wid][c][lane * 4 + 1] = gw[c].y;
        red[wid][c][lane * 4 + 2] = gw[c].z; red[wid][c][lane * 4 + 3] = gw[c].w;
        if (lane == 0) redb[wid][c] = gb[c];
    }
    __syncthreads();
    float* pb = part + (int64_t)blockIdx.x * (DEC_MAXC * H + DEC_MAXC);
    for (int e = threadIdx.x; e < dd.C * H; e += 256) {
        const int c = e / H, k = e % H;
        float s = 0.f;
#pragma unroll
        for (int wv = 0; wv < 8; ++wv) s += red[wv][c][k];
        pb[e] = s;
    }
    if ((int)threadIdx.x < dd.C) {
        float s = 0.f;
#pragma unroll
        for (int wv = 0; wv < 8; ++wv) s += redb[wv][threadIdx.x];
        pb[DEC_MAXC * H + threadIdx.x] = s;
    }
}

__global__ void __launch_bounds__(256)
k_decoder_bwd_reduce(const DecoderDesc dd, const float* __restrict__ part, const int n_blocks, float* __restrict__ grads,
                     const float scale) {
    __shared__ float sh[256];
    const int e = blockIdx.x;
    const int src = (e < dd.C * H) ? e : (DEC_MAXC * H + (e - dd.C * H));
    float s = 0.f;
    for (int b = threadIdx.x; b < n_blocks; b += 256) s += __ldg(part + (int64_t)b * (DEC_MAXC * H + DEC_MAXC) + src);
    sh[threadIdx.x] = s;
    __syncthreads();
    for (int o = 128; o > 0; o >>= 1) {
        if ((int)threadIdx.x < o) sh[threadIdx.x] += sh[threadIdx.x + o];
        __syncthreads();
    }
    if (threadIdx.x == 0) {
        const float r = sh[0] * scale;
        if (e < dd.C * H) grads[dd.w_off + e] = r; else grads[dd.b_off + (e - dd.C * H)] = r;
    }
}

__global__ void __launch_bounds__(256)
k_encoder_dx(const DxUnit* __restrict__ units, const DxOut out, const float* __restrict__ dpre, const float* __restrict__ params,
             const float* __restrict__ signs, const int64_t B, const int64_t Bp) {
    __shared__ float D[16][H + 1];
    __shared__ float W[H][64];
    const DxUnit u = units[blockIdx.y];
    float* dx = out.p[u.type];
    const int64_t g0 = (int64_t)blockIdx.x * 16;
    const int k0 = blockIdx.z * 64, K = u.K;
    if (!dx || k0 >= K || g0 >= B) return;
    const int tid = threadIdx.x, ty = tid >> 4, tx = tid & 15;
    float acc[4] = {0.f, 0.f, 0.f, 0.f};
    if (u.live) {
        const float* dp = dpre + ((int64_t)u.slot * Bp + g0) * H;
        for (int e = tid; e < 16 * H; e += 256) D[e / H][e % H] = dp[e];
        const float* w = params + out.w_off[u.type];
        for (int e = tid; e < H * 64; e += 256) {
            const int c = e / 64, kk = e % 64;
            W[c][kk] = k0 + kk < K ? w[(int64_t)c * K + k0 + kk] : 0.f;
        }
        __syncthreads();
#pragma unroll 4
        for (int c = 0; c < H; ++c) {
            const float d = D[ty][c];
#pragma unroll
            for (int i = 0; i < 4; ++i) acc[i] = fmaf(d, W[c][tx + 16 * i], acc[i]);
        }
    }
    const int64_t g = g0 + ty;
    if (g >= B) return;
    float* row = dx + (g * out.nodes[u.type] + u.node) * K;
#pragma unroll
    for (int i = 0; i < 4; ++i) {
        const int k = k0 + tx + 16 * i;
        if (k < K) row[k] = u.live ? (u.sign_off >= 0 ? acc[i] * signs[u.sign_off + k] : acc[i]) : 0.f;
    }
}

__device__ __forceinline__ double ld_label(const void* p, int dtype, int64_t i) {
    if (dtype == 1) return ((const double*)p)[i];
    if (dtype == 2) return (double)((const long long*)p)[i];
    return (double)((const float*)p)[i];
}

__device__ __forceinline__ double block_sum(double v, double* sh) {
#pragma unroll
    for (int o = 16; o > 0; o >>= 1) v += __shfl_xor_sync(0xffffffffu, v, o);
    const int lane = threadIdx.x & 31, wid = threadIdx.x >> 5;
    if (lane == 0) sh[wid] = v;
    __syncthreads();
    double s = 0.0;
    if (threadIdx.x == 0)
        for (int i = 0; i < (int)(blockDim.x >> 5); ++i) s += sh[i];
    return s;
}

__global__ void __launch_bounds__(256)
k_loss_partial(const int kind, const float* __restrict__ out, const void* __restrict__ labels, const int label_dtype,
               const int64_t n, const float dscale, float* __restrict__ dout, double* __restrict__ partial) {
    __shared__ double sh[8];
    double acc = 0.0;
    for (int64_t i = (int64_t)blockIdx.x * 256 + threadIdx.x; i < n; i += (int64_t)gridDim.x * 256) {
        if (kind == 0) {
            const float d = out[i] - (float)ld_label(labels, label_dtype, i);
            acc += (double)d * (double)d;
            if (dout) dout[i] = 2.f * d * dscale;
        } else {
            const float a = out[2 * i], b = out[2 * i + 1];
            const int y = ld_label(labels, label_dtype, i) != 0.0;
            const float m = fmaxf(a, b);
            const float ea = expf(a - m), eb = expf(b - m);
            const float lse = m + logf(ea + eb);
            acc += (double)(lse - (y ? b : a));
            if (dout) {
                const float inv = 1.f / (ea + eb);
                dout[2 * i] = (ea * inv - (y ? 0.f : 1.f)) * dscale;
                dout[2 * i + 1] = (eb * inv - (y ? 1.f : 0.f)) * dscale;
            }
        }
    }
    const double s = block_sum(acc, sh);
    if (threadIdx.x == 0) partial[blockIdx.x] = s;
}

__global__ void k_loss_final(const double* __restrict__ partial, const int n_blocks, const double inv_n,
                             const int round_f32, float* __restrict__ loss_out) {
    double s = 0.0;
    for (int i = threadIdx.x; i < n_blocks; i += 32) s += partial[i];
#pragma unroll
    for (int o = 16; o > 0; o >>= 1) s += __shfl_xor_sync(0xffffffffu, s, o);
    if (threadIdx.x == 0) loss_out[0] = round_f32 ? (float)((double)(float)s * inv_n) : (float)(s * inv_n);
}

__global__ void __launch_bounds__(256)
k_adam(float* __restrict__ p, const float* __restrict__ g, float* __restrict__ m, float* __restrict__ v, const int64_t n,
       const float lr, const float b1, const float b2, const float eps, const float wd, const float bc1, const float bc2s) {
    for (int64_t i = (int64_t)blockIdx.x * 256 + threadIdx.x; i < n; i += (int64_t)gridDim.x * 256) {
        float gi = g[i];
        const float pi = p[i];
        if (wd != 0.f) gi = fmaf(wd, pi, gi);
        const float mi = m[i] + (1.f - b1) * (gi - m[i]);
        const float vi = b2 * v[i] + (1.f - b2) * gi * gi;
        m[i] = mi; v[i] = vi;
        const float denom = sqrtf(vi) / bc2s + eps;
        p[i] = pi - (lr / bc1) * (mi / denom);
    }
}

__global__ void __launch_bounds__(256)
k_sgd(float* __restrict__ p, const float* __restrict__ g, const int64_t n, const float lr) {
    for (int64_t i = (int64_t)blockIdx.x * 256 + threadIdx.x; i < n; i += (int64_t)gridDim.x * 256) p[i] -= lr * g[i];
}

struct EdgeCheck {
    int n_etypes;
    int E[MSHGNN_MAX_EDGE_TYPES];
    int n_src[MSHGNN_MAX_EDGE_TYPES], n_dst[MSHGNN_MAX_EDGE_TYPES];
    int tpl_off[MSHGNN_MAX_EDGE_TYPES];
    const long long* ei[MSHGNN_MAX_EDGE_TYPES];
};
__global__ void __launch_bounds__(256)
k_check_edges(const EdgeCheck ec, const int* __restrict__ tpl, const long long B, int* __restrict__ flag) {
    const int e = blockIdx.y;
    const int E = ec.E[e];
    const long long n = (long long)E * B;
    const long long* src = ec.ei[e];
    const long long* dst = src + n;
    const int* ts = tpl + ec.tpl_off[e];
    const int* td = ts + E;
    bool bad = false;
    for (long long i = (long long)blockIdx.x * 256 + threadIdx.x; i < n; i += (long long)gridDim.x * 256) {
        const long long g = i / E;
        const int j = (int)(i - g * E);
        bad |= __ldg(src + i) != (long long)ts[j] + g * ec.n_src[e];
        bad |= __ldg(dst + i) != (long long)td[j] + g * ec.n_dst[e];
    }
    if (bad) *reinterpret_cast<volatile int*>(flag) = 1 + e;
}

}
```

morphsym-hgnn_b200/ms_hgnn/_native.py:

```python
from __future__ import annotations

import ctypes as C
import importlib.util
import os
from typing import Optional, Sequence

_PKG = os.path.dirname(os.path.abspath(__file__))
_ROOT = os.path.dirname(_PKG)
LIB_PATH = os.path.join(_ROOT, "lib", "libmshgnn_b200.so")

MAX_NODE_TYPES = 4
MAX_EDGE_TYPES = 16

F32, F64, I64, F16 = 0, 1, 2, 3
MODE_FP32, MODE_TC, MODE_TC_1X = 0, 1, 2
PLAN_PAD_HIDDEN = 1
LOSS_MSE, LOSS_CE2 = 0, 1
METRIC_COM, METRIC_GRF_WORLD = 2, 3
COM_SSE, COM_N, COM_SSE_LIN, COM_SSE_ANG, COM_N_HALF, COM_COS_LIN, COM_COS_ANG, COM_ROWS = range(8)
COM_MSE, COM_RMSE, COM_MSE_LIN, COM_MSE_ANG, COM_COS_SIM_LIN, COM_COS_SIM_ANG, COM_AVG_COS_SIM = range(20, 27)
GRF_SSE, GRF_SAE, GRF_N, GRF_SSE_WORLD, GRF_SAE_WORLD, GRF_N_WORLD = range(6)
GRF_MSE, GRF_RMSE, GRF_L1, GRF_MSE_WORLD, GRF_RMSE_WORLD, GRF_L1_WORLD = range(20, 26)
P_ENC_W, P_ENC_B, P_REL_W, P_REL_B, P_ROOT_W, P_MLP_W, P_MLP_B, P_DEC_W, P_DEC_B = range(9)

EXPORTS = (
    "mshgnn_plan_create", "mshgnn_plan_destroy", "mshgnn_param_count", "mshgnn_param_offset",
    "mshgnn_workspace_bytes", "mshgnn_out_rows", "mshgnn_forward", "mshgnn_loss", "mshgnn_backward",
    "mshgnn_adam_step", "mshgnn_sgd_step", "mshgnn_plan_describe", "mshgnn_launch_count",
    "mshgnn_last_error", "mshgnn_version", "mshgnn_profile_enable", "mshgnn_profile_read", "mshgnn_kernel_kind_name",
    "mshgnn_relu_mask_offset", "mshgnn_build_windows", "mshgnn_step_metrics", "mshgnn_dw_layout",
    "mshgnn_check_edges", "mshgnn_set_option", "mshgnn_get_option", "mshgnn_stack_status", "mshgnn_stack_timing_offset",
    "mshgnn_backward_staged", "mshgnn_input_grad", "mshgnn_plan_create_ex", "mshgnn_step_metrics_ex",
)


class Desc(C.Structure):
    _fields_ = [
        ("n_node_types", C.c_int32),
        ("nodes_per_graph", C.c_int32 * MAX_NODE_TYPES),
        ("in_width", C.c_int32 * MAX_NODE_TYPES),
        ("n_edge_types", C.c_int32),
        ("edge_src_type", C.c_int32 * MAX_EDGE_TYPES),
        ("edge_dst_type", C.c_int32 * MAX_EDGE_TYPES),
        ("edge_mean", C.c_int32 * MAX_EDGE_TYPES),
        ("edge_count", C.c_int32 * MAX_EDGE_TYPES),
        ("edge_src", C.POINTER(C.c_int32) * MAX_EDGE_TYPES),
        ("edge_dst", C.POINTER(C.c_int32) * MAX_EDGE_TYPES),
        ("hidden", C.c_int32),
        ("num_layers", C.c_int32),
        ("morph_sym", C.c_int32),
        ("mlp_type", C.c_int32),
        ("decode_type", C.c_int32),
        ("out_channels", C.c_int32),
        ("in_sign", C.POINTER(C.c_float) * MAX_NODE_TYPES),
        ("out_sign", C.POINTER(C.c_float)),
    ]


class WindowDesc(C.Structure):
    _fields_ = [
        ("history_length", C.c_int32), ("seq_cols", C.c_int32), ("label_cols", C.c_int32), ("n_node_types", C.c_int32),
        ("nodes_per_graph", C.c_int32 * MAX_NODE_TYPES), ("blocks_per_node", C.c_int32 * MAX_NODE_TYPES),
        ("block_len", C.c_int32 * MAX_NODE_TYPES),
        ("normalize", C.c_int32), ("n_labels", C.c_int32),
        ("block_col", C.POINTER(C.c_int32)), ("block_sign", C.POINTER(C.c_int32)),
        ("label_col", C.POINTER(C.c_int32)), ("label_sign", C.POINTER(C.c_int32)),
    ]


class MetricArgs(C.Structure):
    _fields_ = [("n_base", C.c_int32), ("y_mean", C.c_void_p), ("y_std", C.c_void_p), ("quat", C.c_void_p),
                ("quat_dtype", C.c_int32), ("z_only", C.c_int32)]


_lib: Optional[C.CDLL] = None


def _build_if_needed() -> None:
    spec = importlib.util.spec_from_file_location("_mshgnn_build", os.path.join(_ROOT, "build.py"))
    mod = importlib.util.module_from_spec(spec)
    spec.loader.exec_module(mod)
    mod.build()


def lib() -> C.CDLL:
    global _lib
    if _lib is not None:
        return _lib
    override = os.environ.get("MSHGNN_LIB")
    if override:
        if not os.path.exists(override):
            raise RuntimeError(f"MSHGNN_LIB={override} does not exist")
        path = override
    else:
        path = LIB_PATH
        try:
            _build_if_needed()
        except Exception as e:
            if not os.path.exists(LIB_PATH):
                raise RuntimeError(f"libmshgnn_b200.so is missing and could not be built: {e}") from e
    L = C.CDLL(path)
    vp, i32, i64, f32 = C.c_void_p, C.c_int32, C.c_int64, C.c_float
    L.mshgnn_plan_create.argtypes = [C.POINTER(Desc), C.POINTER(vp)]; L.mshgnn_plan_create.restype = C.c_int
    if hasattr(L, "mshgnn_plan_create_ex"):
        L.mshgnn_plan_create_ex.argtypes = [C.POINTER(Desc), i32, C.POINTER(vp)]; L.mshgnn_plan_create_ex.restype = C.c_int
    L.mshgnn_plan_destroy.argtypes = [vp]; L.mshgnn_plan_destroy.restype = None
    L.mshgnn_param_count.argtypes = [vp]; L.mshgnn_param_count.restype = i64
    L.mshgnn_param_offset.argtypes = [vp, i32, i32, i32, C.POINTER(i64), C.POINTER(i64)]; L.mshgnn_param_offset.restype = C.c_int
    L.mshgnn_workspace_bytes.argtypes = [vp, i64, i32, i32]; L.mshgnn_workspace_bytes.restype = i64
    L.mshgnn_dw_layout.argtypes = [vp, i64, i32, C.POINTER(C.c_int32), i64]; L.mshgnn_dw_layout.restype = i64
    L.mshgnn_out_rows.argtypes = [vp, i64]; L.mshgnn_out_rows.restype = i64
    L.mshgnn_forward.argtypes = [vp, i64, C.POINTER(vp), i32, vp, vp, vp, i64, i32, i32, vp]; L.mshgnn_forward.restype = C.c_int
    L.mshgnn_loss.argtypes = [vp, i64, i32, vp, vp, i32, f32, vp, vp, vp, i64, vp]; L.mshgnn_loss.restype = C.c_int
    L.mshgnn_backward.argtypes = [vp, i64, C.POINTER(vp), i32, vp, vp, vp, vp, i64, i32, vp]; L.mshgnn_backward.restype = C.c_int
    L.mshgnn_backward_staged.argtypes = [vp, i64, C.POINTER(vp), i32, vp, vp, vp, vp, i64, i32, vp, vp]; L.mshgnn_backward_staged.restype = C.c_int
    if hasattr(L, "mshgnn_input_grad"):
        L.mshgnn_input_grad.argtypes = [vp, i64, vp, C.POINTER(vp), vp, i64, i32, vp]; L.mshgnn_input_grad.restype = C.c_int
    L.mshgnn_adam_step.argtypes = [vp, vp, vp, vp, i64, i64, f32, f32, f32, f32, f32, vp]; L.mshgnn_adam_step.restype = C.c_int
    L.mshgnn_sgd_step.argtypes = [vp, vp, i64, f32, vp]; L.mshgnn_sgd_step.restype = C.c_int
    L.mshgnn_plan_describe.argtypes = [vp, C.c_char_p, i64]; L.mshgnn_plan_describe.restype = i64
    L.mshgnn_launch_count.argtypes = []; L.mshgnn_launch_count.restype = i64
    L.mshgnn_last_error.argtypes = []; L.mshgnn_last_error.restype = C.c_char_p
    L.mshgnn_version.argtypes = []; L.mshgnn_version.restype = C.c_char_p
    L.mshgnn_profile_enable.argtypes = [i32]; L.mshgnn_profile_enable.restype = C.c_int
    L.mshgnn_profile_read.argtypes = [C.POINTER(C.c_double), C.POINTER(i64), i32]; L.mshgnn_profile_read.restype = C.c_int
    L.mshgnn_kernel_kind_name.argtypes = [i32]; L.mshgnn_kernel_kind_name.restype = C.c_char_p
    L.mshgnn_relu_mask_offset.argtypes = [vp, i64, i32, i32, C.POINTER(i64), C.POINTER(i64), C.POINTER(i64)]
    L.mshgnn_relu_mask_offset.restype = C.c_int
    L.mshgnn_build_windows.argtypes = [C.POINTER(WindowDesc), vp, vp, i32, i64, vp, i64, C.POINTER(vp), vp, vp]
    L.mshgnn_build_windows.restype = C.c_int
    L.mshgnn_step_metrics.argtypes = [i32, i64, i32, vp, vp, i32, vp, vp, vp, vp]; L.mshgnn_step_metrics.restype = C.c_int
    if hasattr(L, "mshgnn_step_metrics_ex"):
        L.mshgnn_step_metrics_ex.argtypes = [i32, C.POINTER(MetricArgs), i64, vp, vp, i32, vp, vp, vp, vp]
        L.mshgnn_step_metrics_ex.restype = C.c_int
    L.mshgnn_check_edges.argtypes = [vp, i64, C.POINTER(vp), vp, vp]; L.mshgnn_check_edges.restype = C.c_int
    L.mshgnn_set_option.argtypes = [C.c_char_p, i32]; L.mshgnn_set_option.restype = C.c_int
    L.mshgnn_get_option.argtypes = [C.c_char_p]; L.mshgnn_get_option.restype = i32
    L.mshgnn_stack_status.argtypes = [vp, i64, i32, i32, vp, C.POINTER(i32)]; L.mshgnn_stack_status.restype = C.c_int
    L.mshgnn_stack_timing_offset.argtypes = [vp, i64, i32, i32]; L.mshgnn_stack_timing_offset.restype = i64
    _lib = L
    return L


def check(rc: int, what: str) -> None:
    if rc != 0:
        raise RuntimeError(f"{what} failed (code {rc}): {lib().mshgnn_last_error().decode()}")


NUM_KERNEL_KINDS = 21


def profile_enable(on: bool) -> None:
    check(lib().mshgnn_profile_enable(int(on)), "mshgnn_profile_enable")


def profile_read() -> dict:
    ms = (C.c_double * NUM_KERNEL_KINDS)()
    cnt = (C.c_int64 * NUM_KERNEL_KINDS)()
    check(lib().mshgnn_profile_read(ms, cnt, NUM_KERNEL_KINDS), "mshgnn_profile_read")
    out = {}
    for k in range(NUM_KERNEL_KINDS):
        name = lib().mshgnn_kernel_kind_name(k).decode()
        if name and cnt[k]:
            out[name] = (float(ms[k]), int(cnt[k]))
    return out


def launch_count() -> int:
    return int(lib().mshgnn_launch_count())


def set_option(name: str, value: int) -> None:
    check(lib().mshgnn_set_option(name.encode(), int(value)), "mshgnn_set_option")


def get_option(name: str) -> int:
    return int(lib().mshgnn_get_option(name.encode()))


class NativePlan:

    def __init__(self, spec: dict):
        L = lib()
        d = Desc()
        nt = len(spec["nodes_per_graph"])
        d.n_node_types = nt
        self._keep = []
        for t in range(nt):
            d.nodes_per_graph[t] = int(spec["nodes_per_graph"][t])
            d.in_width[t] = int(spec["in_width"][t])
            s = spec["in_sign"][t]
            if s is not None:
                arr = (C.c_float * len(s))(*[float(v) for v in s])
                self._keep.append(arr)
                d.in_sign[t] = C.cast(arr, C.POINTER(C.c_float))
        edges = spec["edges"]
        d.n_edge_types = len(edges)
        for e, (st, dt, mean, src, dst) in enumerate(edges):
            d.edge_src_type[e] = st; d.edge_dst_type[e] = dt; d.edge_mean[e] = int(bool(mean)); d.edge_count[e] = len(src)
            a = (C.c_int32 * max(len(src), 1))(*[int(v) for v in src]); b = (C.c_int32 * max(len(dst), 1))(*[int(v) for v in dst])
            self._keep += [a, b]
            d.edge_src[e] = C.cast(a, C.POINTER(C.c_int32)); d.edge_dst[e] = C.cast(b, C.POINTER(C.c_int32))
        d.hidden = int(spec["hidden"]); d.num_layers = int(spec["num_layers"])
        d.morph_sym = int(bool(spec["morph_sym"])); d.mlp_type = int(spec["mlp_type"])
        d.decode_type = int(spec["decode_type"]); d.out_channels = int(spec["out_channels"])
        if spec.get("out_sign") is not None:
            arr = (C.c_float * len(spec["out_sign"]))(*[float(v) for v in spec["out_sign"]])
            self._keep.append(arr)
            d.out_sign = C.cast(arr, C.POINTER(C.c_float))
        h = C.c_void_p()
        if spec.get("pad_hidden") and hasattr(L, "mshgnn_plan_create_ex"):
            check(L.mshgnn_plan_create_ex(C.byref(d), PLAN_PAD_HIDDEN, C.byref(h)), "mshgnn_plan_create_ex")
        else:
            check(L.mshgnn_plan_create(C.byref(d), C.byref(h)), "mshgnn_plan_create")
        self.handle = h
        self.spec = spec
        self.n_params = int(L.mshgnn_param_count(h))

    def __del__(self):
        try:
            if getattr(self, "handle", None):
                lib().mshgnn_plan_destroy(self.handle)
                self.handle = None
        except Exception:
            pass

    def param_offset(self, kind: int, layer: int = 0, idx: int = 0):
        off, n = C.c_int64(), C.c_int64()
        check(lib().mshgnn_param_offset(self.handle, kind, layer, idx, C.byref(off), C.byref(n)), "mshgnn_param_offset")
        return off.value, n.value

    def workspace_bytes(self, B: int, train: bool, mode: int = MODE_FP32) -> int:
        n = int(lib().mshgnn_workspace_bytes(self.handle, B, int(train), mode))
        if n < 0:
            raise RuntimeError("mshgnn_workspace_bytes failed")
        return n

    def dw_layout(self, B: int, mode: int = MODE_TC):
        buf = (C.c_int32 * 64)()
        n = int(lib().mshgnn_dw_layout(self.handle, B, mode, buf, 64))
        if n < 0:
            raise RuntimeError("mshgnn_dw_layout failed")
        return [tuple(buf[4 * l + k] for k in range(4)) for l in range(n)]

    def out_rows(self, B: int) -> int:
        return int(lib().mshgnn_out_rows(self.handle, B))

    def relu_mask_offset(self, B: int, mode: int, layer: int):
        off, ns, bp = C.c_int64(), C.c_int64(), C.c_int64()
        check(lib().mshgnn_relu_mask_offset(self.handle, B, mode, layer, C.byref(off), C.byref(ns), C.byref(bp)), "mshgnn_relu_mask_offset")
        return off.value, ns.value, bp.value

    def describe(self) -> dict:
        import json
        n = int(lib().mshgnn_plan_describe(self.handle, None, 0))
        buf = C.create_string_buffer(n)
        lib().mshgnn_plan_describe(self.handle, buf, n)
        return json.loads(buf.value.decode())

    def check_edges(self, B, ei_ptrs: Sequence[int], flag_ptr, stream):
        arr = (C.c_void_p * len(ei_ptrs))(*ei_ptrs)
        check(lib().mshgnn_check_edges(self.handle, B, arr, flag_ptr, stream), "mshgnn_check_edges")

    def stack_status(self, B, train, mode, ws_ptr) -> int:
        out = C.c_int32()
        check(lib().mshgnn_stack_status(self.handle, B, int(train), mode, ws_ptr, C.byref(out)), "mshgnn_stack_status")
        return out.value

    def stack_timing_offset(self, B, train, mode) -> int:
        return int(lib().mshgnn_stack_timing_offset(self.handle, B, int(train), mode))

    def forward(self, B, x_ptrs: Sequence[int], x_dtype, params_ptr, out_ptr, ws_ptr, ws_bytes, train, mode, stream):
        arr = (C.c_void_p * len(x_ptrs))(*x_ptrs)
        check(lib().mshgnn_forward(self.handle, B, arr, x_dtype, params_ptr, out_ptr, ws_ptr, ws_bytes, int(train), mode, stream),
              "mshgnn_forward")

    def loss(self, B, kind, out_ptr, labels_ptr, label_dtype, loss_scale, loss_ptr, dout_ptr, ws_ptr, ws_bytes, stream):
        check(lib().mshgnn_loss(self.handle, B, kind, out_ptr, labels_ptr, label_dtype, loss_scale, loss_ptr, dout_ptr,
                                ws_ptr, ws_bytes, stream), "mshgnn_loss")

    def backward(self, B, x_ptrs, x_dtype, params_ptr, dout_ptr, grads_ptr, ws_ptr, ws_bytes, mode, stream, layers_ready_event=None):
        arr = (C.c_void_p * len(x_ptrs))(*x_ptrs)
        check(lib().mshgnn_backward_staged(self.handle, B, arr, x_dtype, params_ptr, dout_ptr, grads_ptr, ws_ptr, ws_bytes, mode, stream,
                                           layers_ready_event), "mshgnn_backward")

    def input_grad(self, B, params_ptr, dx_ptrs, ws_ptr, ws_bytes, mode, stream):
        arr = (C.c_void_p * len(dx_ptrs))(*dx_ptrs)
        check(lib().mshgnn_input_grad(self.handle, B, params_ptr, arr, ws_ptr, ws_bytes, mode, stream), "mshgnn_input_grad")


METRIC_SLOTS, METRIC_SCRATCH = 32, 296 * 32


def step_metrics(kind, n, feet, out_ptr, labels_ptr, label_dtype, batch_ptr, epoch_ptr, scratch_ptr, stream):
    check(lib().mshgnn_step_metrics(kind, n, feet, out_ptr, labels_ptr, label_dtype, batch_ptr, epoch_ptr, scratch_ptr, stream),
          "mshgnn_step_metrics")


def step_metrics_ex(kind, args: MetricArgs, n, out_ptr, labels_ptr, label_dtype, batch_ptr, epoch_ptr, scratch_ptr, stream):
    check(lib().mshgnn_step_metrics_ex(kind, C.byref(args), n, out_ptr, labels_ptr, label_dtype, batch_ptr, epoch_ptr, scratch_ptr,
                                       stream), "mshgnn_step_metrics_ex")


def adam_step(params_ptr, grads_ptr, m_ptr, v_ptr, n, step, lr, b1, b2, eps, wd, stream):
    check(lib().mshgnn_adam_step(params_ptr, grads_ptr, m_ptr, v_ptr, n, step, lr, b1, b2, eps, wd, stream), "mshgnn_adam_step")


def sgd_step(params_ptr, grads_ptr, n, lr, stream):
    check(lib().mshgnn_sgd_step(params_ptr, grads_ptr, n, lr, stream), "mshgnn_sgd_step")
```

morphsym-hgnn_b200/ms_hgnn/engine.py:

```python
from __future__ import annotations

from typing import Dict, List, Optional, Sequence, Tuple

import torch

from . import _native as N

EdgeType = Tuple[str, str, str]


def build_spec(node_types: Sequence[str], nodes_per_graph: Dict[str, int], in_width: Dict[str, int],
               edge_types: Sequence[EdgeType], edges: Dict[EdgeType, Tuple[List[int], List[int]]],
               mean_relations: Sequence[str], hidden: int, num_layers: int, morph_sym: bool, mlp_type: Optional[str],
               decode_type: str, out_channels: int, in_sign: Dict[str, Optional[List[float]]],
               out_sign: Optional[List[float]], pad_hidden: bool = False) -> dict:
    ti = {t: i for i, t in enumerate(node_types)}
    spec = {
        "node_types": list(node_types),
        "edge_types": [tuple(e) for e in edge_types],
        "nodes_per_graph": [int(nodes_per_graph[t]) for t in node_types],
        "in_width": [int(in_width[t]) for t in node_types],
        "edges": [(ti[e[0]], ti[e[2]], e[1] in mean_relations, list(edges[tuple(e)][0]), list(edges[tuple(e)][1]))
                  for e in edge_types],
        "hidden": hidden, "num_layers": num_layers, "morph_sym": morph_sym,
        "mlp_type": ti[mlp_type] if (morph_sym and mlp_type is not None) else -1,
        "decode_type": ti[decode_type], "out_channels": out_channels,
        "in_sign": [in_sign.get(t) for t in node_types], "out_sign": out_sign,
    }
    if pad_hidden:
        spec["pad_hidden"] = True
    return spec


def _dtype_code(t: torch.Tensor) -> int:
    if t.dtype == torch.float32:
        return N.F32
    if t.dtype == torch.float64:
        return N.F64
    if t.dtype == torch.float16:
        return N.F16
    if t.dtype == torch.int64:
        return N.I64
    raise TypeError(f"unsupported dtype {t.dtype} (float32, float64, float16 features or int64 labels expected)")


class Engine:

    def __init__(self, spec: dict, mode: int = N.MODE_FP32):
        self.spec = spec
        self.plan = N.NativePlan(spec)
        self.mode = mode
        self.n_params = self.plan.n_params
        self._ws: Optional[torch.Tensor] = None
        self._ws_key = None
        self._train_ctx = None

    def param_layout(self) -> List[Tuple[str, int, Tuple[int, ...]]]:
        s = self.spec
        H = s["hidden"]
        out = []
        for i, t in enumerate(s["node_types"]):
            o, _ = self.plan.param_offset(N.P_ENC_W, 0, i); out.append((f"encoder.lins.{t}.weight", o, (H, s["in_width"][i])))
            o, _ = self.plan.param_offset(N.P_ENC_B, 0, i); out.append((f"encoder.lins.{t}.bias", o, (H,)))
        for l in range(s["num_layers"]):
            for e, et in enumerate(s["edge_types"]):
                key = "<" + "___".join(et) + ">"
                o, _ = self.plan.param_offset(N.P_REL_W, l, e); out.append((f"convs.{l}.convs.{key}.lin_rel.weight", o, (H, H)))
                o, _ = self.plan.param_offset(N.P_REL_B, l, e); out.append((f"convs.{l}.convs.{key}.lin_rel.bias", o, (H,)))
                o, _ = self.plan.param_offset(N.P_ROOT_W, l, e); out.append((f"convs.{l}.convs.{key}.lin_root.weight", o, (H, H)))
        if s["morph_sym"]:
            for i, j in ((0, 0), (1, 2)):
                o, _ = self.plan.param_offset(N.P_MLP_W, 0, i); out.append((f"base_transform.{j}.weight", o, (H, H)))
                o, _ = self.plan.param_offset(N.P_MLP_B, 0, i); out.append((f"base_transform.{j}.bias", o, (H,)))
        o, _ = self.plan.param_offset(N.P_DEC_W); out.append(("decoder.weight", o, (s["out_channels"], H)))
        o, _ = self.plan.param_offset(N.P_DEC_B); out.append(("decoder.bias", o, (s["out_channels"],)))
        return out

    def workspace(self, B: int, train: bool, device) -> torch.Tensor:
        need = self.plan.workspace_bytes(B, train, self.mode)
        if self._ws is None or self._ws.numel() < need or self._ws.device != device:
            self._ws = None
            self._ws = torch.empty(need, dtype=torch.uint8, device=device)
        return self._ws

    def _check_inputs(self, x: Sequence[torch.Tensor]) -> Tuple[int, int]:
        s = self.spec
        if len(x) != len(s["node_types"]):
            raise ValueError("one feature tensor per node type expected")
        dev = x[0].device
        if dev.type != "cuda":
            raise RuntimeError("ms_hgnn (B200-native) has no CPU path: node features must be CUDA tensors")
        B = None
        for i, t in enumerate(x):
            if t.device != dev:
                raise ValueError("all node feature tensors must live on the same device")
            if t.dim() != 2 or t.shape[1] != s["in_width"][i]:
                raise ValueError(f"x[{s['node_types'][i]}] must be [B*{s['nodes_per_graph'][i]}, {s['in_width'][i]}], got {tuple(t.shape)}")
            if t.shape[0] % s["nodes_per_graph"][i]:
                raise ValueError(f"x[{s['node_types'][i]}] has {t.shape[0]} rows, not a multiple of {s['nodes_per_graph'][i]}")
            b = t.shape[0] // s["nodes_per_graph"][i]
            if B is None:
                B = b
            elif b != B:
                raise ValueError("node feature tensors disagree on the number of graphs")
            if t.dtype != x[0].dtype:
                raise TypeError("all node feature tensors must share one dtype")
        if B is None or B < 1:
            raise ValueError("empty batch")
        return B, _dtype_code(x[0])

    def forward(self, x: Sequence[torch.Tensor], flat_params: torch.Tensor, train: bool) -> torch.Tensor:
        B, xd = self._check_inputs(x)
        x = [t.contiguous() for t in x]
        dev = x[0].device
        if flat_params.device != dev or flat_params.dtype != torch.float32 or flat_params.numel() != self.n_params:
            raise RuntimeError("flat parameter buffer mismatch")
        ws = self.workspace(B, train, dev)
        out = torch.empty(self.plan.out_rows(B), self.spec["out_channels"], dtype=torch.float32, device=dev)
        stream = torch.cuda.current_stream(dev).cuda_stream
        with torch.cuda.device(dev):
            self.plan.forward(B, [t.data_ptr() for t in x], xd, flat_params.data_ptr(), out.data_ptr(), ws.data_ptr(),
                              ws.numel(), train, self.mode, stream)
        self._train_ctx = (B, x, xd) if train else None
        return out

    def loss(self, out: torch.Tensor, labels: torch.Tensor, kind: int, want_grad: bool = True, loss_scale: float = 1.0):
        dev = out.device
        B = out.shape[0] // self.spec["nodes_per_graph"][self.spec["decode_type"]]
        labels = labels.contiguous()
        n_expected = out.numel() if kind == N.LOSS_MSE else out.shape[0]
        if labels.numel() != n_expected:
            raise ValueError(f"labels have {labels.numel()} elements, expected {n_expected}")
        if labels.device != dev:
            raise ValueError("labels must live on the same device as the predictions")
        ws = self.workspace(B, self._train_ctx is not None, dev)
        loss = torch.empty(1, dtype=torch.float32, device=dev)
        dout = torch.empty_like(out) if want_grad else None
        stream = torch.cuda.current_stream(dev).cuda_stream
        with torch.cuda.device(dev):
            self.plan.loss(B, kind, out.data_ptr(), labels.data_ptr(), _dtype_code(labels), float(loss_scale), loss.data_ptr(),
                           dout.data_ptr() if want_grad else None, ws.data_ptr(), ws.numel(), stream)
        return loss, dout

    def encoder_param_end(self) -> int:
        return min(o for (name, o, _) in self.param_layout() if not name.startswith("encoder."))

    def backward(self, dout: torch.Tensor, flat_params: torch.Tensor, grads: Optional[torch.Tensor] = None,
                 layers_ready: Optional[torch.cuda.Event] = None, param_grads: bool = True) -> Optional[torch.Tensor]:
        if self._train_ctx is None:
            raise RuntimeError("backward() needs a preceding forward(train=True) on the same engine")
        B, x, xd = self._train_ctx
        dev = x[0].device
        dout = dout.contiguous()
        if dout.dtype != torch.float32:
            dout = dout.float()
        if dout.numel() != self.plan.out_rows(B) * self.spec["out_channels"]:
            raise ValueError("dout has the wrong number of elements")
        if not param_grads:
            grads = None
        elif grads is None:
            grads = torch.empty(self.n_params, dtype=torch.float32, device=dev)
        ws = self.workspace(B, True, dev)
        stream = torch.cuda.current_stream(dev).cuda_stream
        with torch.cuda.device(dev):
            if layers_ready is not None:
                if layers_ready.cuda_event == 0:
                    layers_ready.record(torch.cuda.current_stream(dev))
            self.plan.backward(B, [t.data_ptr() for t in x], xd, flat_params.data_ptr(), dout.data_ptr(),
                               grads.data_ptr() if grads is not None else None,
                               ws.data_ptr(), ws.numel(), self.mode, stream,
                               layers_ready.cuda_event if layers_ready is not None else None)
        return grads

    def input_grad(self, which: Sequence[bool], flat_params: torch.Tensor) -> List[Optional[torch.Tensor]]:
        if self._train_ctx is None:
            raise RuntimeError("input_grad() needs a preceding forward(train=True) and backward() on the same engine")
        B, x, _ = self._train_ctx
        dev = x[0].device
        out = [torch.empty(t.shape, dtype=torch.float32, device=dev) if w else None for t, w in zip(x, which)]
        ws = self.workspace(B, True, dev)
        stream = torch.cuda.current_stream(dev).cuda_stream
        with torch.cuda.device(dev):
            self.plan.input_grad(B, flat_params.data_ptr(), [t.data_ptr() if t is not None else None for t in out], ws.data_ptr(),
                                 ws.numel(), self.mode, stream)
        return out
```

morphsym-hgnn_b200/ms_hgnn/train.py:

```python
from __future__ import annotations

from typing import Optional

import torch

from . import _native as N


def allreduce_flat_(grads: torch.Tensor, world: int, group=None) -> torch.Tensor:
    if world > 1:
        torch.distributed.all_reduce(grads, op=torch.distributed.ReduceOp.SUM, group=group)
    return grads


class FusedTrainer:
    def __init__(self, module, optimizer: Optional[str] = None, lr: Optional[float] = None, process_group=None,
                 betas=(0.9, 0.999), eps: float = 1e-8, weight_decay: float = 0.0):
        self.module = module
        self.model = getattr(module, "model", module)
        self.optimizer = optimizer or getattr(module, "optimizer", "adam")
        self.lr = float(lr if lr is not None else getattr(module, "lr", 1e-3))
        if self.optimizer not in ("adam", "sgd"):
            raise ValueError("Invalid optimizer setting")
        self.betas, self.eps, self.weight_decay = betas, eps, weight_decay
        self.pg = process_group
        self.world = 1
        if process_group is not None or (torch.distributed.is_available() and torch.distributed.is_initialized()):
            self.world = torch.distributed.get_world_size(process_group)
        self.step_count = 0
        self.grads = None
        self.exp_avg = None
        self.exp_avg_sq = None
        self.overlap_allreduce = True
        self.skip_allreduce = False
        self._side = None
        self._layers_ready = None
        self._synced_params = False
        self._graphs = {}

    def _loss_kind(self) -> int:
        regression = getattr(self.module, "regression", getattr(self.model, "regression", True))
        return N.LOSS_MSE if regression else N.LOSS_CE2

    def _prepare(self, batch):
        x_dict = batch.x_dict
        model = self.model
        eng, B = model._engine_for(x_dict, batch.edge_index_dict)
        model._last_engine = eng
        dev = x_dict[model.node_types[0]].device
        model._ensure_flat(dev)
        return eng, B, [x_dict[t] for t in model.node_types], dev

    def _sync_parameters(self, flat: torch.Tensor) -> None:
        if self.world > 1 and not self._synced_params:
            torch.distributed.broadcast(flat, src=torch.distributed.get_global_rank(self.pg, 0) if self.pg is not None else 0, group=self.pg)
        self._synced_params = True

    def _backward_and_reduce(self, eng, dout, flat, dev) -> None:
        if self.world == 1 or self.skip_allreduce or not self.overlap_allreduce:
            eng.backward(dout, flat, grads=self.grads)
            if not self.skip_allreduce:
                allreduce_flat_(self.grads, self.world, self.pg)
            return
        if self._side is None:
            self._side = torch.cuda.Stream(dev)
            self._layers_ready = torch.cuda.Event()
        cur = torch.cuda.current_stream(dev)
        eng.backward(dout, flat, grads=self.grads, layers_ready=self._layers_ready)
        cut = eng.encoder_param_end()
        self._side.wait_event(self._layers_ready)
        with torch.cuda.stream(self._side):
            torch.distributed.all_reduce(self.grads[cut:], op=torch.distributed.ReduceOp.SUM, group=self.pg)
        torch.distributed.all_reduce(self.grads[:cut], op=torch.distributed.ReduceOp.SUM, group=self.pg)
        cur.wait_stream(self._side)

    def train_step(self, batch) -> torch.Tensor:
        eng, B, xs, dev = self._prepare(batch)
        model = self.model
        flat = model._flat
        n = flat.numel()
        if self.grads is None or self.grads.device != dev or self.grads.numel() != n:
            self.grads = torch.empty(n, dtype=torch.float32, device=dev)
            self.exp_avg = torch.zeros(n, dtype=torch.float32, device=dev)
            self.exp_avg_sq = torch.zeros(n, dtype=torch.float32, device=dev)
        self._sync_parameters(flat)
        out = eng.forward(xs, flat, train=True)
        model._fwd_token = object()
        loss, dout = eng.loss(out, batch.y, self._loss_kind(), want_grad=True, loss_scale=1.0 / self.world)
        self._backward_and_reduce(eng, dout, flat, dev)
        self.step_count += 1
        self._optimizer_step(flat, n, dev)
        return loss

    def _optimizer_step(self, flat, n, dev) -> None:
        stream = torch.cuda.current_stream(dev).cuda_stream
        with torch.cuda.device(dev):
            if self.optimizer == "adam":
                N.adam_step(flat.data_ptr(), self.grads.data_ptr(), self.exp_avg.data_ptr(), self.exp_avg_sq.data_ptr(), n,
                            self.step_count, self.lr, self.betas[0], self.betas[1], self.eps, self.weight_decay, stream)
            else:
                N.sgd_step(flat.data_ptr(), self.grads.data_ptr(), n, self.lr, stream)

    def train_step_graphed(self, batch) -> torch.Tensor:
        key = id(batch)
        ent = self._graphs.get(key)
        if ent is None:
            loss = self.train_step(batch)
            eng, B, xs, dev = self._prepare(batch)
            model = self.model
            flat = model._flat
            g = torch.cuda.CUDAGraph()
            static_loss = torch.empty(1, dtype=torch.float32, device=dev)
            torch.cuda.synchronize(dev)
            with torch.cuda.graph(g):
                out = eng.forward(xs, flat, train=True)
                l, dout = eng.loss(out, batch.y, self._loss_kind(), want_grad=True, loss_scale=1.0 / self.world)
                eng.backward(dout, flat, grads=self.grads)
                static_loss.copy_(l)
            self._graphs[key] = (g, static_loss, batch, flat.numel(), dev)
            return loss
        g, static_loss, _, n, dev = ent
        model = self.model
        flat = model._flat
        g.replay()
        model._fwd_token = object()
        if not self.skip_allreduce:
            allreduce_flat_(self.grads, self.world, self.pg)
        self.step_count += 1
        self._optimizer_step(flat, n, dev)
        return static_loss

    @torch.no_grad()
    def infer(self, batch) -> torch.Tensor:
        eng, B, xs, dev = self._prepare(batch)
        return self.model._finish(eng.forward(xs, self.model._flat, train=False), B)
```

Baseline: 5.560 million.

## Fuse decoder forward, loss, and decoder backward into a single train-head kernel

Adds a train-head path that skips the decoder in the forward pass. One kernel then runs the decoder output, the loss gradient and the decoder backward, and a tail kernel reduces the decoder weight gradients and the loss. The backward pass gets a head-done flag so it skips the grad memset and the decoder stage, and the training loop uses this path in the tensor-core modes. This removes the separate decoder-forward, loss and decoder-backward launches and the round trips through the out and dout buffers. In exchange it adds new kernels and reuses workspace areas for the loss terms.

```diff
diff --git a/include/mshgnn_b200.h b/include/mshgnn_b200.h
--- a/include/mshgnn_b200.h
+++ b/include/mshgnn_b200.h
@@ -95,6 +95,26 @@
                            void* workspace, int64_t workspace_bytes,
                            int32_t mode, void* stream, void* layers_ready_event);
 
+#define MSHGNN_FWD_NO_DECODER 1
+#define MSHGNN_BWD_HEAD_DONE  1
+
+int mshgnn_forward_ex(const mshgnn_plan* plan, int64_t B,
+                      const void* const* x, int32_t x_dtype,
+                      const float* params, float* out,
+                      void* workspace, int64_t workspace_bytes,
+                      int32_t train, int32_t mode, void* stream, int32_t flags);
+
+int mshgnn_train_head(const mshgnn_plan* plan, int64_t B, int32_t loss_kind,
+                      const void* labels, int32_t label_dtype, float loss_scale,
+                      const float* params, float* out, float* loss_out, float* grads,
+                      void* workspace, int64_t workspace_bytes, int32_t mode, void* stream);
+
+int mshgnn_backward_ex(const mshgnn_plan* plan, int64_t B,
+                       const void* const* x, int32_t x_dtype,
+                       const float* params, const float* dout, float* grads,
+                       void* workspace, int64_t workspace_bytes,
+                       int32_t mode, void* stream, void* layers_ready_event, int32_t flags);
+
 int mshgnn_input_grad(const mshgnn_plan* plan, int64_t B, const float* params, float* const* dx,
                       void* workspace, int64_t workspace_bytes, int32_t mode, void* stream);
 
diff --git a/morphsym-hgnn_b200/csrc/api.cu b/morphsym-hgnn_b200/csrc/api.cu
--- a/morphsym-hgnn_b200/csrc/api.cu
+++ b/morphsym-hgnn_b200/csrc/api.cu
@@ -662,11 +662,20 @@
 
 int mshgnn_forward(const mshgnn_plan* plan, int64_t B, const void* const* x, int32_t x_dtype, const float* params,
                    float* out, void* workspace, int64_t workspace_bytes, int32_t train, int32_t mode, void* stream) {
+    return mshgnn_forward_ex(plan, B, x, x_dtype, params, out, workspace, workspace_bytes, train, mode, stream, 0);
+}
+
+int mshgnn_forward_ex(const mshgnn_plan* plan, int64_t B, const void* const* x, int32_t x_dtype, const float* params,
+                      float* out, void* workspace, int64_t workspace_bytes, int32_t train, int32_t mode, void* stream, int32_t flags) {
     int rc;
     if ((rc = check_plan_mode(plan, mode))) return rc;
     const Plan& p = plan->p;
     if (x_dtype != MSHGNN_F32 && x_dtype != MSHGNN_F64 && x_dtype != MSHGNN_F16) return fail(MSHGNN_ERR_ARG, "x_dtype must be F32, F64 or F16");
-    if (!x || !params || !out) return fail(MSHGNN_ERR_ARG, "NULL argument");
+    if (flags & ~MSHGNN_FWD_NO_DECODER) return fail(MSHGNN_ERR_ARG, "unknown forward flags 0x%x", (unsigned)flags);
+    const bool decode = !(flags & MSHGNN_FWD_NO_DECODER);
+    if (!decode && (!train || mode == MSHGNN_MODE_FP32))
+        return fail(MSHGNN_ERR_ARG, "MSHGNN_FWD_NO_DECODER is for train-mode forwards in the tensor-core modes (mshgnn_train_head decodes)");
+    if (!x || !params || (decode && !out)) return fail(MSHGNN_ERR_ARG, "NULL argument");
     Call c;
     if ((rc = open_call(c, plan, B, train, mode, workspace, workspace_bytes))) return rc;
     for (int t = 0; t < p.n_types; ++t)
@@ -732,7 +741,7 @@
             if ((rc = launch_tc_rowgemm(K_MLP_FWD, p, p.mlp2[l], bt, br, wm, B, w.Bp, split, st))) return rc;
         }
     }
-    {
+    if (decode) {
         const int64_t rows = B * p.dec.n_dec;
         int blocks = (int)((rows + 7) / 8);
         if (blocks > 148 * 8) blocks = 148 * 8;
@@ -771,19 +780,88 @@
     return 0;
 }
 
+int mshgnn_train_head(const mshgnn_plan* plan, int64_t B, int32_t loss_kind, const void* labels, int32_t label_dtype, float loss_scale,
+                      const float* params, float* out, float* loss_out, float* grads, void* workspace, int64_t workspace_bytes,
+                      int32_t mode, void* stream) {
+    int rc;
+    if ((rc = check_plan_mode(plan, mode))) return rc;
+    const Plan& p = plan->p;
+    if (mode == MSHGNN_MODE_FP32) return fail(MSHGNN_ERR_ARG, "mshgnn_train_head needs a tensor-core mode (fp32: mshgnn_forward, mshgnn_loss, mshgnn_backward)");
+    if (!labels || !params || !out || !loss_out || !grads) return fail(MSHGNN_ERR_ARG, "NULL argument");
+    if (label_dtype < 0 || label_dtype > 2) return fail(MSHGNN_ERR_ARG, "bad label_dtype");
+    if (loss_kind != MSHGNN_LOSS_CE2 && loss_kind != MSHGNN_LOSS_MSE) return fail(MSHGNN_ERR_ARG, "bad loss_kind");
+    if (loss_kind == MSHGNN_LOSS_CE2 && p.C != 2) return fail(MSHGNN_ERR_ARG, "CE2 loss needs out_channels == 2");
+    Call c;
+    if ((rc = open_call(c, plan, B, 1, mode, workspace, workspace_bytes))) return rc;
+    const int64_t rows = B * p.dec.n_dec;
+    const int64_t n = loss_kind == MSHGNN_LOSS_MSE ? rows * p.C : rows;
+    const WsLayout& w = c.w;
+    if (w.part_slots * H * H < n) return fail(MSHGNN_ERR_WORKSPACE, "internal: the loss terms do not fit the weight-gradient partials");
+    if ((rc = bind_call(c, params, grads, nullptr))) return rc;
+    cudaStream_t st = (cudaStream_t)stream;
+    char* ws = c.ws;
+    const int L = p.L;
+    const bool want_dh = p.morph_sym, want_dc = !p.morph_sym || p.dec_type != p.mlp_type;
+    const int dhb = BUF_DHL0 + L, dcb = BUF_DCL0 + L - 1;
+    HeadArgs a;
+    a.h_hi = image16(ws, w, BUF_H0 + L, 0); a.h_lo = image16(ws, w, BUF_H0 + L, 1);
+    a.params = c.params; a.signs = p.d_signs;
+    a.labels = labels; a.label_dtype = label_dtype; a.loss_kind = loss_kind;
+    a.dscale = loss_scale / (float)n;
+    a.gscale = c.G;
+    a.out = out;
+    a.terms = (float*)(ws + w.part_w);
+    a.part = (float*)(ws + w.dec_part);
+    a.mask_kind = want_dc ? MK_BITS : MK_NONE;
+    a.mask_buf = want_dc ? c.bt.p[BUF_MASK0 + L - 1] : nullptr;
+    a.dh_hi = want_dh ? image16(ws, w, dhb, 0) : nullptr; a.dh_lo = want_dh ? image16(ws, w, dhb, 1) : nullptr;
+    a.dc_hi = want_dc ? image16(ws, w, dcb, 0) : nullptr; a.dc_lo = want_dc ? image16(ws, w, dcb, 1) : nullptr;
+    a.grads = c.grads; a.n_grads = p.n_params;
+    a.zero = w.stack ? (uint32_t*)(ws + w.stack_sync) : nullptr;
+    a.zero_words = w.stack ? w.stack_sync_bytes / 4 : 0;
+    a.counter = (uint32_t*)(ws + w.enc_sync) + 1;
+    a.B = B; a.Bp = w.Bp;
+    {
+        ProfScope ps(K_DEC_BWD, st);
+        if (p.dec.C <= 2) k_train_head<2><<<DEC_BLOCKS, 256, 0, st>>>(p.dec, a);
+        else if (p.dec.C <= 4) k_train_head<4><<<DEC_BLOCKS, 256, 0, st>>>(p.dec, a);
+        else k_train_head<8><<<DEC_BLOCKS, 256, 0, st>>>(p.dec, a);
+        LAUNCH_CHECK();
+    }
+    {
+        int n_loss = (int)((n + 255) / 256);
+        if (n_loss > LOSS_BLOCKS) n_loss = LOSS_BLOCKS;
+        ProfScope ps(K_LOSS, st);
+        k_head_tail<<<p.dec.C * H + p.dec.C + n_loss, 256, 0, st>>>(p.dec, a.part, DEC_BLOCKS, c.grads, 1.f / c.G, loss_kind, a.terms, n,
+                                                                    (double*)(ws + w.loss_part), a.counter, 1.0 / (double)n, loss_out);
+        LAUNCH_CHECK();
+    }
+    return 0;
+}
+
 int mshgnn_backward(const mshgnn_plan* plan, int64_t B, const void* const* x, int32_t x_dtype, const float* params,
                     const float* dout, float* grads, void* workspace, int64_t workspace_bytes, int32_t mode, void* stream) {
-    return mshgnn_backward_staged(plan, B, x, x_dtype, params, dout, grads, workspace, workspace_bytes, mode, stream, nullptr);
+    return mshgnn_backward_ex(plan, B, x, x_dtype, params, dout, grads, workspace, workspace_bytes, mode, stream, nullptr, 0);
 }
 
 int mshgnn_backward_staged(const mshgnn_plan* plan, int64_t B, const void* const* x, int32_t x_dtype, const float* params,
                            const float* dout, float* grads, void* workspace, int64_t workspace_bytes, int32_t mode, void* stream,
                            void* layers_ready_event) {
+    return mshgnn_backward_ex(plan, B, x, x_dtype, params, dout, grads, workspace, workspace_bytes, mode, stream, layers_ready_event, 0);
+}
+
+int mshgnn_backward_ex(const mshgnn_plan* plan, int64_t B, const void* const* x, int32_t x_dtype, const float* params,
+                       const float* dout, float* grads, void* workspace, int64_t workspace_bytes, int32_t mode, void* stream,
+                       void* layers_ready_event, int32_t flags) {
     int rc;
     if ((rc = check_plan_mode(plan, mode))) return rc;
     const Plan& p = plan->p;
     if (x_dtype != MSHGNN_F32 && x_dtype != MSHGNN_F64 && x_dtype != MSHGNN_F16) return fail(MSHGNN_ERR_ARG, "x_dtype must be F32, F64 or F16");
-    if (!x || !params || !dout) return fail(MSHGNN_ERR_ARG, "NULL argument");
+    if (flags & ~MSHGNN_BWD_HEAD_DONE) return fail(MSHGNN_ERR_ARG, "unknown backward flags 0x%x", (unsigned)flags);
+    const bool head_done = flags & MSHGNN_BWD_HEAD_DONE;
+    if (head_done && (mode == MSHGNN_MODE_FP32 || !grads))
+        return fail(MSHGNN_ERR_ARG, "MSHGNN_BWD_HEAD_DONE follows mshgnn_train_head: tensor-core modes, with grads");
+    if (!x || !params || (!head_done && !dout)) return fail(MSHGNN_ERR_ARG, "NULL argument");
     const bool want_dw = grads != nullptr;
     Call c;
     if ((rc = open_call(c, plan, B, 1, mode, workspace, workspace_bytes))) return rc;
@@ -805,7 +883,8 @@
     float* part_b = (float*)(ws + w.part_b);
     float* dec_part = (float*)(ws + w.dec_part);
 
-    if (!want_dw) {
+    if (head_done) {
+    } else if (!want_dw) {
         if ((rc = stack_sync_reset(w, ws, st))) return rc;
     } else if (w.stack && (reinterpret_cast<uintptr_t>(grads) & 15) == 0) {
         ProfScope ps(K_MEMSET, st);
@@ -817,7 +896,7 @@
         if ((rc = stack_sync_reset(w, ws, st))) return rc;
     }
 
-    {
+    if (!head_done) {
         const int L = p.L;
         const bool want_dh = p.morph_sym, want_dc = !p.morph_sym || p.dec_type != p.mlp_type;
         const int dhb = BUF_DHL0 + L, dcb = BUF_DCL0 + L - 1;
diff --git a/morphsym-hgnn_b200/csrc/kernels_simt.cuh b/morphsym-hgnn_b200/csrc/kernels_simt.cuh
--- a/morphsym-hgnn_b200/csrc/kernels_simt.cuh
+++ b/morphsym-hgnn_b200/csrc/kernels_simt.cuh
@@ -393,6 +393,15 @@
     }
 }
 
+__device__ __forceinline__ float dec_out(const DecoderDesc& dd, const float4 h, const float4 w, const float* __restrict__ params,
+                                         const float* __restrict__ signs, const int j, const int c) {
+    float s = h.x * w.x + h.y * w.y + h.z * w.z + h.w * w.w;
+#pragma unroll
+    for (int o = 16; o > 0; o >>= 1) s += __shfl_xor_sync(0xffffffffu, s, o);
+    float v = s + __ldg(params + dd.b_off + c);
+    if (dd.sign_off >= 0) v *= __ldg(signs + dd.sign_off + j * dd.C + c);
+    return v;
+}
 template <int CMAX>
 __global__ void __launch_bounds__(256)
 k_decoder_fwd(const DecoderDesc dd, const float* __restrict__ hslab, const __half* __restrict__ h_hi, const __half* __restrict__ h_lo,
@@ -414,15 +423,78 @@
 #pragma unroll
         for (int c = 0; c < CMAX; ++c) {
             if (c >= dd.C) break;
-            float s = h.x * w[c].x + h.y * w[c].y + h.z * w[c].z + h.w * w[c].w;
-#pragma unroll
-            for (int o = 16; o > 0; o >>= 1) s += __shfl_xor_sync(0xffffffffu, s, o);
-            if (lane == 0) {
-                float v = s + __ldg(params + dd.b_off + c);
-                if (dd.sign_off >= 0) v *= __ldg(signs + dd.sign_off + j * dd.C + c);
-                out[row * dd.C + c] = v;
-            }
-        }
+            const float v = dec_out(dd, h, w[c], params, signs, j, c);
+            if (lane == 0) out[row * dd.C + c] = v;
+        }
+    }
+}
+
+template <int CMAX>
+__device__ __forceinline__ void dec_bwd_row(const DecoderDesc& dd, const float4 h, const float4 (&w)[CMAX], const float (&dv)[CMAX],
+                                            float4 (&gw)[CMAX], float (&gb)[CMAX], float* __restrict__ dh, float* __restrict__ dc,
+                                            const int mask_kind, const void* __restrict__ mask_buf, const int64_t Bp, const int64_t g,
+                                            const int j, const int64_t off, const int lane,
+                                            __half* __restrict__ dh_hi, __half* __restrict__ dh_lo, __half* __restrict__ dc_hi, __half* __restrict__ dc_lo) {
+    float4 d = make_float4(0.f, 0.f, 0.f, 0.f);
+#pragma unroll
+    for (int c = 0; c < CMAX; ++c) {
+        if (c >= dd.C) break;
+        d.x = fmaf(dv[c], w[c].x, d.x); d.y = fmaf(dv[c], w[c].y, d.y);
+        d.z = fmaf(dv[c], w[c].z, d.z); d.w = fmaf(dv[c], w[c].w, d.w);
+        gw[c].x = fmaf(dv[c], h.x, gw[c].x); gw[c].y = fmaf(dv[c], h.y, gw[c].y);
+        gw[c].z = fmaf(dv[c], h.z, gw[c].z); gw[c].w = fmaf(dv[c], h.w, gw[c].w);
+        gb[c] += dv[c];
+    }
+    if (dh) *reinterpret_cast<float4*>(dh + off) = d;
+    if (dh_hi) { const float vv[4] = {d.x, d.y, d.z, d.w}; split_store4(dh_hi, dh_lo, off, vv); }
+    if (dc || dc_hi) {
+        if (mask_kind == MK_BITS) {
+            const unsigned wd = *((const unsigned*)mask_buf + ((int64_t)dd.slots[j] * Bp + g) * 4 + (lane >> 3));
+            const unsigned nb = (wd >> ((lane & 7) * 4)) & 0xFu;
+            d.x = (nb & 1u) ? d.x : 0.f; d.y = (nb & 2u) ? d.y : 0.f;
+            d.z = (nb & 4u) ? d.z : 0.f; d.w = (nb & 8u) ? d.w : 0.f;
+        }
+        if (dc) *reinterpret_cast<float4*>(dc + off) = d;
+        if (dc_hi) { const float vv[4] = {d.x, d.y, d.z, d.w}; split_store4(dc_hi, dc_lo, off, vv); }
+    }
+}
+
+template <int CMAX>
+__device__ __forceinline__ void dec_bwd_finish(const DecoderDesc& dd, const float4 (&gw)[CMAX], const float (&gb)[CMAX],
+                                               float (*red)[CMAX][H + 1], float (*redb)[CMAX], float* __restrict__ part,
+                                               const int64_t warp, const int64_t stride, const int lane, const int wid,
+                                               const int64_t B, const int64_t Bp,
+                                               __half* __restrict__ dh_hi, __half* __restrict__ dh_lo, __half* __restrict__ dc_hi, __half* __restrict__ dc_lo) {
+    if (dh_hi || dc_hi) {
+        const int64_t pad = Bp - B;
+        const float z[4] = {0.f, 0.f, 0.f, 0.f};
+        for (int64_t r = warp; r < pad * dd.n_dec; r += stride) {
+            const int64_t off = ((int64_t)dd.slots[r / pad] * Bp + B + r % pad) * H + lane * 4;
+            if (dh_hi) split_store4(dh_hi, dh_lo, off, z);
+            if (dc_hi) split_store4(dc_hi, dc_lo, off, z);
+        }
+    }
+#pragma unroll
+    for (int c = 0; c < CMAX; ++c) {
+        if (c >= dd.C) break;
+        red[wid][c][lane * 4 + 0] = gw[c].x; red[wid][c][lane * 4 + 1] = gw[c].y;
+        red[wid][c][lane * 4 + 2] = gw[c].z; red[wid][c][lane * 4 + 3] = gw[c].w;
+        if (lane == 0) redb[wid][c] = gb[c];
+    }
+    __syncthreads();
+    float* pb = part + (int64_t)blockIdx.x * (DEC_MAXC * H + DEC_MAXC);
+    for (int e = threadIdx.x; e < dd.C * H; e += 256) {
+        const int c = e / H, k = e % H;
+        float s = 0.f;
+#pragma unroll
+        for (int wv = 0; wv < 8; ++wv) s += red[wv][c][k];
+        pb[e] = s;
+    }
+    if ((int)threadIdx.x < dd.C) {
+        float s = 0.f;
+#pragma unroll
+        for (int wv = 0; wv < 8; ++wv) s += redb[wv][threadIdx.x];
+        pb[DEC_MAXC * H + threadIdx.x] = s;
     }
 }
 
@@ -455,69 +527,21 @@
         const int j = (int)(row % dd.n_dec);
         const int64_t off = ((int64_t)dd.slots[j] * Bp + g) * H + lane * 4;
         const float4 h = load_h4(hslab, h_hi, h_lo, off);
-        float4 d = make_float4(0.f, 0.f, 0.f, 0.f);
+        float dv[CMAX];
 #pragma unroll
         for (int c = 0; c < CMAX; ++c) {
             if (c >= dd.C) break;
-            float dv = __ldg(dout + row * dd.C + c) * gscale;
-            if (dd.sign_off >= 0) dv *= __ldg(signs + dd.sign_off + j * dd.C + c);
-            d.x = fmaf(dv, w[c].x, d.x); d.y = fmaf(dv, w[c].y, d.y);
-            d.z = fmaf(dv, w[c].z, d.z); d.w = fmaf(dv, w[c].w, d.w);
-            gw[c].x = fmaf(dv, h.x, gw[c].x); gw[c].y = fmaf(dv, h.y, gw[c].y);
-            gw[c].z = fmaf(dv, h.z, gw[c].z); gw[c].w = fmaf(dv, h.w, gw[c].w);
-            gb[c] += dv;
-        }
-        if (dh) *reinterpret_cast<float4*>(dh + off) = d;
-        if (dh_hi) { const float vv[4] = {d.x, d.y, d.z, d.w}; split_store4(dh_hi, dh_lo, off, vv); }
-        if (dc || dc_hi) {
-            if (mask_kind == MK_BITS) {
-                const unsigned wd = *((const unsigned*)mask_buf + ((int64_t)dd.slots[j] * Bp + g) * 4 + (lane >> 3));
-                const unsigned nb = (wd >> ((lane & 7) * 4)) & 0xFu;
-                d.x = (nb & 1u) ? d.x : 0.f; d.y = (nb & 2u) ? d.y : 0.f;
-                d.z = (nb & 4u) ? d.z : 0.f; d.w = (nb & 8u) ? d.w : 0.f;
-            }
-            if (dc) *reinterpret_cast<float4*>(dc + off) = d;
-            if (dc_hi) { const float vv[4] = {d.x, d.y, d.z, d.w}; split_store4(dc_hi, dc_lo, off, vv); }
-        }
-    }
-    if (dh_hi || dc_hi) {
-        const int64_t pad = Bp - B;
-        const float z[4] = {0.f, 0.f, 0.f, 0.f};
-        for (int64_t r = warp; r < pad * dd.n_dec; r += stride) {
-            const int64_t off = ((int64_t)dd.slots[r / pad] * Bp + B + r % pad) * H + lane * 4;
-            if (dh_hi) split_store4(dh_hi, dh_lo, off, z);
-            if (dc_hi) split_store4(dc_hi, dc_lo, off, z);
-        }
-    }
-#pragma unroll
-    for (int c = 0; c < CMAX; ++c) {
-        if (c >= dd.C) break;
-        red[wid][c][lane * 4 + 0] = gw[c].x; red[wid][c][lane * 4 + 1] = gw[c].y;
-        red[wid][c][lane * 4 + 2] = gw[c].z; red[wid][c][lane * 4 + 3] = gw[c].w;
-        if (lane == 0) redb[wid][c] = gb[c];
-    }
-    __syncthreads();
-    float* pb = part + (int64_t)blockIdx.x * (DEC_MAXC * H + DEC_MAXC);
-    for (int e = threadIdx.x; e < dd.C * H; e += 256) {
-        const int c = e / H, k = e % H;
-        float s = 0.f;
-#pragma unroll
-        for (int wv = 0; wv < 8; ++wv) s += red[wv][c][k];
-        pb[e] = s;
-    }
-    if ((int)threadIdx.x < dd.C) {
-        float s = 0.f;
-#pragma unroll
-        for (int wv = 0; wv < 8; ++wv) s += redb[wv][threadIdx.x];
-        pb[DEC_MAXC * H + threadIdx.x] = s;
-    }
-}
-
-__global__ void __launch_bounds__(256)
-k_decoder_bwd_reduce(const DecoderDesc dd, const float* __restrict__ part, const int n_blocks, float* __restrict__ grads,
-                     const float scale) {
+            dv[c] = __ldg(dout + row * dd.C + c) * gscale;
+            if (dd.sign_off >= 0) dv[c] *= __ldg(signs + dd.sign_off + j * dd.C + c);
+        }
+        dec_bwd_row<CMAX>(dd, h, w, dv, gw, gb, dh, dc, mask_kind, mask_buf, Bp, g, j, off, lane, dh_hi, dh_lo, dc_hi, dc_lo);
+    }
+    dec_bwd_finish<CMAX>(dd, gw, gb, red, redb, part, warp, stride, lane, wid, B, Bp, dh_hi, dh_lo, dc_hi, dc_lo);
+}
+
+__device__ __forceinline__ void dec_reduce_elem(const DecoderDesc& dd, const float* __restrict__ part, const int n_blocks, float* __restrict__ grads,
+                                                const float scale, const int e) {
     __shared__ float sh[256];
-    const int e = blockIdx.x;
     const int src = (e < dd.C * H) ? e : (DEC_MAXC * H + (e - dd.C * H));
     float s = 0.f;
     for (int b = threadIdx.x; b < n_blocks; b += 256) s += __ldg(part + (int64_t)b * (DEC_MAXC * H + DEC_MAXC) + src);
@@ -531,6 +555,12 @@
         const float r = sh[0] * scale;
         if (e < dd.C * H) grads[dd.w_off + e] = r; else grads[dd.b_off + (e - dd.C * H)] = r;
     }
+}
+
+__global__ void __launch_bounds__(256)
+k_decoder_bwd_reduce(const DecoderDesc dd, const float* __restrict__ part, const int n_blocks, float* __restrict__ grads,
+                     const float scale) {
+    dec_reduce_elem(dd, part, n_blocks, grads, scale, blockIdx.x);
 }
 
 __global__ void __launch_bounds__(256)
@@ -589,6 +619,19 @@
     return s;
 }
 
+__device__ __forceinline__ float mse_diff(const float o, const void* __restrict__ labels, const int label_dtype, const int64_t i) {
+    return o - (float)ld_label(labels, label_dtype, i);
+}
+__device__ __forceinline__ float ce2_row(const float a, const float b, const int y, const float dscale, float& ga, float& gb) {
+    const float m = fmaxf(a, b);
+    const float ea = expf(a - m), eb = expf(b - m);
+    const float lse = m + logf(ea + eb);
+    const float inv = 1.f / (ea + eb);
+    ga = (ea * inv - (y ? 0.f : 1.f)) * dscale;
+    gb = (eb * inv - (y ? 1.f : 0.f)) * dscale;
+    return lse - (y ? b : a);
+}
+
 __global__ void __launch_bounds__(256)
 k_loss_partial(const int kind, const float* __restrict__ out, const void* __restrict__ labels, const int label_dtype,
                const int64_t n, const float dscale, float* __restrict__ dout, double* __restrict__ partial) {
@@ -596,34 +639,139 @@
     double acc = 0.0;
     for (int64_t i = (int64_t)blockIdx.x * 256 + threadIdx.x; i < n; i += (int64_t)gridDim.x * 256) {
         if (kind == 0) {
-            const float d = out[i] - (float)ld_label(labels, label_dtype, i);
+            const float d = mse_diff(out[i], labels, label_dtype, i);
             acc += (double)d * (double)d;
             if (dout) dout[i] = 2.f * d * dscale;
         } else {
-            const float a = out[2 * i], b = out[2 * i + 1];
-            const int y = ld_label(labels, label_dtype, i) != 0.0;
-            const float m = fmaxf(a, b);
-            const float ea = expf(a - m), eb = expf(b - m);
-            const float lse = m + logf(ea + eb);
-            acc += (double)(lse - (y ? b : a));
-            if (dout) {
-                const float inv = 1.f / (ea + eb);
-                dout[2 * i] = (ea * inv - (y ? 0.f : 1.f)) * dscale;
-                dout[2 * i + 1] = (eb * inv - (y ? 1.f : 0.f)) * dscale;
-            }
+            float ga, gb;
+            acc += (double)ce2_row(out[2 * i], out[2 * i + 1], ld_label(labels, label_dtype, i) != 0.0, dscale, ga, gb);
+            if (dout) { dout[2 * i] = ga; dout[2 * i + 1] = gb; }
         }
     }
     const double s = block_sum(acc, sh);
     if (threadIdx.x == 0) partial[blockIdx.x] = s;
 }
 
+__device__ __forceinline__ void loss_final_warp(const double* __restrict__ partial, const int n_blocks, const double inv_n,
+                                                const int round_f32, float* __restrict__ loss_out) {
+    double s = 0.0;
+    for (int i = threadIdx.x; i < n_blocks; i += 32) s += __ldcg(partial + i);
+#pragma unroll
+    for (int o = 16; o > 0; o >>= 1) s += __shfl_xor_sync(0xffffffffu, s, o);
+    if (threadIdx.x == 0) loss_out[0] = round_f32 ? (float)((double)(float)s * inv_n) : (float)(s * inv_n);
+}
+
 __global__ void k_loss_final(const double* __restrict__ partial, const int n_blocks, const double inv_n,
                              const int round_f32, float* __restrict__ loss_out) {
-    double s = 0.0;
-    for (int i = threadIdx.x; i < n_blocks; i += 32) s += partial[i];
-#pragma unroll
-    for (int o = 16; o > 0; o >>= 1) s += __shfl_xor_sync(0xffffffffu, s, o);
-    if (threadIdx.x == 0) loss_out[0] = round_f32 ? (float)((double)(float)s * inv_n) : (float)(s * inv_n);
+    loss_final_warp(partial, n_blocks, inv_n, round_f32, loss_out);
+}
+
+struct HeadArgs {
+    const __half* h_hi; const __half* h_lo;
+    const float* params; const float* signs;
+    const void* labels; int label_dtype; int loss_kind;
+    float dscale, gscale;
+    float* out; float* terms; float* part;
+    const void* mask_buf; int mask_kind;
+    __half* dh_hi; __half* dh_lo; __half* dc_hi; __half* dc_lo;
+    float* grads; int64_t n_grads;
+    uint32_t* zero; int64_t zero_words;
+    uint32_t* counter;
+    int64_t B, Bp;
+};
+
+template <int CMAX>
+__global__ void __launch_bounds__(256)
+k_train_head(const DecoderDesc dd, const HeadArgs a) {
+    __shared__ float red[8][CMAX][H + 1];
+    __shared__ float redb[8][CMAX];
+    const int lane = threadIdx.x & 31, wid = threadIdx.x >> 5;
+    const int64_t warp = (int64_t)blockIdx.x * 8 + wid;
+    const int64_t n_rows = a.B * dd.n_dec;
+    const int64_t stride = (int64_t)gridDim.x * 8;
+    {
+        const int64_t tid = (int64_t)blockIdx.x * 256 + threadIdx.x, nt = (int64_t)gridDim.x * 256;
+        if ((reinterpret_cast<uintptr_t>(a.grads) & 15) == 0) {
+            const int64_t n4 = a.n_grads / 4;
+            for (int64_t i = tid; i < n4; i += nt) reinterpret_cast<float4*>(a.grads)[i] = make_float4(0.f, 0.f, 0.f, 0.f);
+            for (int64_t i = 4 * n4 + tid; i < a.n_grads; i += nt) a.grads[i] = 0.f;
+        } else {
+            for (int64_t i = tid; i < a.n_grads; i += nt) a.grads[i] = 0.f;
+        }
+        for (int64_t i = tid; i < a.zero_words; i += nt) a.zero[i] = 0u;
+        if (tid == 0) *a.counter = 0u;
+    }
+    float4 w[CMAX], gw[CMAX];
+    float gb[CMAX];
+#pragma unroll
+    for (int c = 0; c < CMAX; ++c) {
+        w[c] = (c < dd.C) ? __ldg(reinterpret_cast<const float4*>(a.params + dd.w_off + c * H + lane * 4))
+                          : make_float4(0.f, 0.f, 0.f, 0.f);
+        gw[c] = make_float4(0.f, 0.f, 0.f, 0.f);
+        gb[c] = 0.f;
+    }
+#pragma unroll 2
+    for (int64_t row = warp; row < n_rows; row += stride) {
+        const int64_t g = row / dd.n_dec;
+        const int j = (int)(row % dd.n_dec);
+        const int64_t off = ((int64_t)dd.slots[j] * a.Bp + g) * H + lane * 4;
+        const float4 h = load_h4(nullptr, a.h_hi, a.h_lo, off);
+        float o[CMAX], dv[CMAX];
+#pragma unroll
+        for (int c = 0; c < CMAX; ++c) {
+            if (c >= dd.C) break;
+            o[c] = dec_out(dd, h, w[c], a.params, a.signs, j, c);
+            if (lane == 0) a.out[row * dd.C + c] = o[c];
+        }
+        if (a.loss_kind == 0) {
+#pragma unroll
+            for (int c = 0; c < CMAX; ++c) {
+                if (c >= dd.C) break;
+                const int64_t i = row * dd.C + c;
+                const float d = mse_diff(o[c], a.labels, a.label_dtype, i);
+                if (lane == 0) a.terms[i] = d;
+                dv[c] = 2.f * d * a.dscale;
+            }
+        } else {
+            const float t = ce2_row(o[0], o[1], ld_label(a.labels, a.label_dtype, row) != 0.0, a.dscale, dv[0], dv[1]);
+            if (lane == 0) a.terms[row] = t;
+        }
+#pragma unroll
+        for (int c = 0; c < CMAX; ++c) {
+            if (c >= dd.C) break;
+            dv[c] = dv[c] * a.gscale;
+            if (dd.sign_off >= 0) dv[c] *= __ldg(a.signs + dd.sign_off + j * dd.C + c);
+        }
+        dec_bwd_row<CMAX>(dd, h, w, dv, gw, gb, nullptr, nullptr, a.mask_kind, a.mask_buf, a.Bp, g, j, off, lane, a.dh_hi, a.dh_lo, a.dc_hi, a.dc_lo);
+    }
+    dec_bwd_finish<CMAX>(dd, gw, gb, red, redb, a.part, warp, stride, lane, wid, a.B, a.Bp, a.dh_hi, a.dh_lo, a.dc_hi, a.dc_lo);
+}
+
+__global__ void __launch_bounds__(256)
+k_head_tail(const DecoderDesc dd, const float* __restrict__ part, const int n_dec_blocks, float* __restrict__ grads, const float rscale,
+            const int loss_kind, const float* __restrict__ terms, const int64_t n, double* __restrict__ partial, uint32_t* __restrict__ counter,
+            const double inv_n, float* __restrict__ loss_out) {
+    const int n_dw = dd.C * H + dd.C;
+    if ((int)blockIdx.x < n_dw) { dec_reduce_elem(dd, part, n_dec_blocks, grads, rscale, blockIdx.x); return; }
+    const int b = blockIdx.x - n_dw, nb = gridDim.x - n_dw;
+    __shared__ double sh[8];
+    __shared__ bool last;
+    double acc = 0.0;
+    for (int64_t i = (int64_t)b * 256 + threadIdx.x; i < n; i += (int64_t)nb * 256) {
+        const float t = terms[i];
+        acc += loss_kind == 0 ? (double)t * (double)t : (double)t;
+    }
+    const double s = block_sum(acc, sh);
+    if (threadIdx.x == 0) {
+        partial[b] = s;
+        __threadfence();
+        last = atomicAdd(counter, 1u) == (uint32_t)(nb - 1);
+    }
+    __syncthreads();
+    if (!last) return;
+    __threadfence();
+    if (threadIdx.x < 32) loss_final_warp(partial, nb, inv_n, loss_kind == 1, loss_out);
+    if (threadIdx.x == 0) *counter = 0u;
 }
 
 __global__ void __launch_bounds__(256)
diff --git a/morphsym-hgnn_b200/ms_hgnn/_native.py b/morphsym-hgnn_b200/ms_hgnn/_native.py
--- a/morphsym-hgnn_b200/ms_hgnn/_native.py
+++ b/morphsym-hgnn_b200/ms_hgnn/_native.py
@@ -31,7 +31,11 @@
     "mshgnn_relu_mask_offset", "mshgnn_build_windows", "mshgnn_step_metrics", "mshgnn_dw_layout",
     "mshgnn_check_edges", "mshgnn_set_option", "mshgnn_get_option", "mshgnn_stack_status", "mshgnn_stack_timing_offset",
     "mshgnn_backward_staged", "mshgnn_input_grad", "mshgnn_plan_create_ex", "mshgnn_step_metrics_ex",
+    "mshgnn_forward_ex", "mshgnn_train_head", "mshgnn_backward_ex",
 )
+
+FWD_NO_DECODER = 1
+BWD_HEAD_DONE = 1
 
 
 class Desc(C.Structure):
@@ -116,6 +120,11 @@
     L.mshgnn_backward_staged.argtypes = [vp, i64, C.POINTER(vp), i32, vp, vp, vp, vp, i64, i32, vp, vp]; L.mshgnn_backward_staged.restype = C.c_int
     if hasattr(L, "mshgnn_input_grad"):
         L.mshgnn_input_grad.argtypes = [vp, i64, vp, C.POINTER(vp), vp, i64, i32, vp]; L.mshgnn_input_grad.restype = C.c_int
+    if hasattr(L, "mshgnn_train_head"):
+        L.mshgnn_forward_ex.argtypes = [vp, i64, C.POINTER(vp), i32, vp, vp, vp, i64, i32, i32, vp, i32]; L.mshgnn_forward_ex.restype = C.c_int
+        L.mshgnn_train_head.argtypes = [vp, i64, i32, vp, i32, f32, vp, vp, vp, vp, vp, i64, i32, vp]; L.mshgnn_train_head.restype = C.c_int
+        L.mshgnn_backward_ex.argtypes = [vp, i64, C.POINTER(vp), i32, vp, vp, vp, vp, i64, i32, vp, vp, i32]
+        L.mshgnn_backward_ex.restype = C.c_int
     L.mshgnn_adam_step.argtypes = [vp, vp, vp, vp, i64, i64, f32, f32, f32, f32, f32, vp]; L.mshgnn_adam_step.restype = C.c_int
     L.mshgnn_sgd_step.argtypes = [vp, vp, i64, f32, vp]; L.mshgnn_sgd_step.restype = C.c_int
     L.mshgnn_plan_describe.argtypes = [vp, C.c_char_p, i64]; L.mshgnn_plan_describe.restype = i64
@@ -270,17 +279,31 @@
     def stack_timing_offset(self, B, train, mode) -> int:
         return int(lib().mshgnn_stack_timing_offset(self.handle, B, int(train), mode))
 
-    def forward(self, B, x_ptrs: Sequence[int], x_dtype, params_ptr, out_ptr, ws_ptr, ws_bytes, train, mode, stream):
+    def forward(self, B, x_ptrs: Sequence[int], x_dtype, params_ptr, out_ptr, ws_ptr, ws_bytes, train, mode, stream, flags=0):
         arr = (C.c_void_p * len(x_ptrs))(*x_ptrs)
+        if flags:
+            check(lib().mshgnn_forward_ex(self.handle, B, arr, x_dtype, params_ptr, out_ptr, ws_ptr, ws_bytes, int(train), mode, stream,
+                                          flags), "mshgnn_forward_ex")
+            return
         check(lib().mshgnn_forward(self.handle, B, arr, x_dtype, params_ptr, out_ptr, ws_ptr, ws_bytes, int(train), mode, stream),
               "mshgnn_forward")
+
+    def train_head(self, B, kind, labels_ptr, label_dtype, loss_scale, params_ptr, out_ptr, loss_ptr, grads_ptr, ws_ptr, ws_bytes,
+                   mode, stream):
+        check(lib().mshgnn_train_head(self.handle, B, kind, labels_ptr, label_dtype, loss_scale, params_ptr, out_ptr, loss_ptr,
+                                      grads_ptr, ws_ptr, ws_bytes, mode, stream), "mshgnn_train_head")
 
     def loss(self, B, kind, out_ptr, labels_ptr, label_dtype, loss_scale, loss_ptr, dout_ptr, ws_ptr, ws_bytes, stream):
         check(lib().mshgnn_loss(self.handle, B, kind, out_ptr, labels_ptr, label_dtype, loss_scale, loss_ptr, dout_ptr,
                                 ws_ptr, ws_bytes, stream), "mshgnn_loss")
 
-    def backward(self, B, x_ptrs, x_dtype, params_ptr, dout_ptr, grads_ptr, ws_ptr, ws_bytes, mode, stream, layers_ready_event=None):
+    def backward(self, B, x_ptrs, x_dtype, params_ptr, dout_ptr, grads_ptr, ws_ptr, ws_bytes, mode, stream, layers_ready_event=None,
+                 flags=0):
         arr = (C.c_void_p * len(x_ptrs))(*x_ptrs)
+        if flags:
+            check(lib().mshgnn_backward_ex(self.handle, B, arr, x_dtype, params_ptr, dout_ptr, grads_ptr, ws_ptr, ws_bytes, mode, stream,
+                                           layers_ready_event, flags), "mshgnn_backward_ex")
+            return
         check(lib().mshgnn_backward_staged(self.handle, B, arr, x_dtype, params_ptr, dout_ptr, grads_ptr, ws_ptr, ws_bytes, mode, stream,
                                            layers_ready_event), "mshgnn_backward")
 
diff --git a/morphsym-hgnn_b200/ms_hgnn/engine.py b/morphsym-hgnn_b200/ms_hgnn/engine.py
--- a/morphsym-hgnn_b200/ms_hgnn/engine.py
+++ b/morphsym-hgnn_b200/ms_hgnn/engine.py
@@ -109,7 +109,23 @@
             raise ValueError("empty batch")
         return B, _dtype_code(x[0])
 
-    def forward(self, x: Sequence[torch.Tensor], flat_params: torch.Tensor, train: bool) -> torch.Tensor:
+    def has_train_head(self) -> bool:
+        return self.mode != N.MODE_FP32 and hasattr(N.lib(), "mshgnn_train_head")
+
+    def forward(self, x: Sequence[torch.Tensor], flat_params: torch.Tensor, train: bool, decode: bool = True) -> Optional[torch.Tensor]:
+        if not decode:
+            B, xd = self._check_inputs(x)
+            x = [t.contiguous() for t in x]
+            dev = x[0].device
+            if flat_params.device != dev or flat_params.dtype != torch.float32 or flat_params.numel() != self.n_params:
+                raise RuntimeError("flat parameter buffer mismatch")
+            ws = self.workspace(B, train, dev)
+            stream = torch.cuda.current_stream(dev).cuda_stream
+            with torch.cuda.device(dev):
+                self.plan.forward(B, [t.data_ptr() for t in x], xd, flat_params.data_ptr(), None, ws.data_ptr(), ws.numel(), train,
+                                  self.mode, stream, flags=N.FWD_NO_DECODER)
+            self._train_ctx = (B, x, xd) if train else None
+            return None
         B, xd = self._check_inputs(x)
         x = [t.contiguous() for t in x]
         dev = x[0].device
@@ -142,20 +158,48 @@
                            dout.data_ptr() if want_grad else None, ws.data_ptr(), ws.numel(), stream)
         return loss, dout
 
+    def train_head(self, labels: torch.Tensor, kind: int, flat_params: torch.Tensor, grads: torch.Tensor, loss_scale: float = 1.0):
+        if self._train_ctx is None:
+            raise RuntimeError("train_head() needs a preceding forward(train=True) on the same engine")
+        B, x, _ = self._train_ctx
+        dev = x[0].device
+        C = self.spec["out_channels"]
+        rows = self.plan.out_rows(B)
+        labels = labels.contiguous()
+        n_expected = rows * C if kind == N.LOSS_MSE else rows
+        if labels.numel() != n_expected:
+            raise ValueError(f"labels have {labels.numel()} elements, expected {n_expected}")
+        if labels.device != dev:
+            raise ValueError("labels must live on the same device as the node features")
+        if grads.device != dev or grads.dtype != torch.float32 or grads.numel() != self.n_params or not grads.is_contiguous():
+            raise ValueError("grads must be a contiguous fp32 device buffer of n_params elements")
+        ws = self.workspace(B, True, dev)
+        out = torch.empty(rows, C, dtype=torch.float32, device=dev)
+        loss = torch.empty(1, dtype=torch.float32, device=dev)
+        stream = torch.cuda.current_stream(dev).cuda_stream
+        with torch.cuda.device(dev):
+            self.plan.train_head(B, kind, labels.data_ptr(), _dtype_code(labels), float(loss_scale), flat_params.data_ptr(), out.data_ptr(),
+                                 loss.data_ptr(), grads.data_ptr(), ws.data_ptr(), ws.numel(), self.mode, stream)
+        return loss, out
+
     def encoder_param_end(self) -> int:
         return min(o for (name, o, _) in self.param_layout() if not name.startswith("encoder."))
 
-    def backward(self, dout: torch.Tensor, flat_params: torch.Tensor, grads: Optional[torch.Tensor] = None,
-                 layers_ready: Optional[torch.cuda.Event] = None, param_grads: bool = True) -> Optional[torch.Tensor]:
+    def backward(self, dout: Optional[torch.Tensor], flat_params: torch.Tensor, grads: Optional[torch.Tensor] = None,
+                 layers_ready: Optional[torch.cuda.Event] = None, param_grads: bool = True, head_done: bool = False) -> Optional[torch.Tensor]:
         if self._train_ctx is None:
             raise RuntimeError("backward() needs a preceding forward(train=True) on the same engine")
         B, x, xd = self._train_ctx
         dev = x[0].device
-        dout = dout.contiguous()
-        if dout.dtype != torch.float32:
-            dout = dout.float()
-        if dout.numel() != self.plan.out_rows(B) * self.spec["out_channels"]:
-            raise ValueError("dout has the wrong number of elements")
+        if head_done:
+            if grads is None or not param_grads:
+                raise ValueError("head_done needs the grads buffer train_head() wrote")
+        else:
+            dout = dout.contiguous()
+            if dout.dtype != torch.float32:
+                dout = dout.float()
+            if dout.numel() != self.plan.out_rows(B) * self.spec["out_channels"]:
+                raise ValueError("dout has the wrong number of elements")
         if not param_grads:
             grads = None
         elif grads is None:
@@ -166,10 +210,11 @@
             if layers_ready is not None:
                 if layers_ready.cuda_event == 0:
                     layers_ready.record(torch.cuda.current_stream(dev))
-            self.plan.backward(B, [t.data_ptr() for t in x], xd, flat_params.data_ptr(), dout.data_ptr(),
+            self.plan.backward(B, [t.data_ptr() for t in x], xd, flat_params.data_ptr(), None if head_done else dout.data_ptr(),
                                grads.data_ptr() if grads is not None else None,
                                ws.data_ptr(), ws.numel(), self.mode, stream,
-                               layers_ready.cuda_event if layers_ready is not None else None)
+                               layers_ready.cuda_event if layers_ready is not None else None,
+                               flags=N.BWD_HEAD_DONE if head_done else 0)
         return grads
 
     def input_grad(self, which: Sequence[bool], flat_params: torch.Tensor) -> List[Optional[torch.Tensor]]:
diff --git a/morphsym-hgnn_b200/ms_hgnn/train.py b/morphsym-hgnn_b200/ms_hgnn/train.py
--- a/morphsym-hgnn_b200/ms_hgnn/train.py
+++ b/morphsym-hgnn_b200/ms_hgnn/train.py
@@ -56,9 +56,18 @@
             torch.distributed.broadcast(flat, src=torch.distributed.get_global_rank(self.pg, 0) if self.pg is not None else 0, group=self.pg)
         self._synced_params = True
 
+    def _forward_loss(self, eng, xs, batch, flat):
+        if eng.has_train_head():
+            eng.forward(xs, flat, train=True, decode=False)
+            loss, _ = eng.train_head(batch.y, self._loss_kind(), flat, self.grads, loss_scale=1.0 / self.world)
+            return loss, None
+        out = eng.forward(xs, flat, train=True)
+        return eng.loss(out, batch.y, self._loss_kind(), want_grad=True, loss_scale=1.0 / self.world)
+
     def _backward_and_reduce(self, eng, dout, flat, dev) -> None:
+        head_done = dout is None
         if self.world == 1 or self.skip_allreduce or not self.overlap_allreduce:
-            eng.backward(dout, flat, grads=self.grads)
+            eng.backward(dout, flat, grads=self.grads, head_done=head_done)
             if not self.skip_allreduce:
                 allreduce_flat_(self.grads, self.world, self.pg)
             return
@@ -66,7 +75,7 @@
             self._side = torch.cuda.Stream(dev)
             self._layers_ready = torch.cuda.Event()
         cur = torch.cuda.current_stream(dev)
-        eng.backward(dout, flat, grads=self.grads, layers_ready=self._layers_ready)
+        eng.backward(dout, flat, grads=self.grads, layers_ready=self._layers_ready, head_done=head_done)
         cut = eng.encoder_param_end()
         self._side.wait_event(self._layers_ready)
         with torch.cuda.stream(self._side):
@@ -84,9 +93,8 @@
             self.exp_avg = torch.zeros(n, dtype=torch.float32, device=dev)
             self.exp_avg_sq = torch.zeros(n, dtype=torch.float32, device=dev)
         self._sync_parameters(flat)
-        out = eng.forward(xs, flat, train=True)
+        loss, dout = self._forward_loss(eng, xs, batch, flat)
         model._fwd_token = object()
-        loss, dout = eng.loss(out, batch.y, self._loss_kind(), want_grad=True, loss_scale=1.0 / self.world)
         self._backward_and_reduce(eng, dout, flat, dev)
         self.step_count += 1
         self._optimizer_step(flat, n, dev)
@@ -113,9 +121,8 @@
             static_loss = torch.empty(1, dtype=torch.float32, device=dev)
             torch.cuda.synchronize(dev)
             with torch.cuda.graph(g):
-                out = eng.forward(xs, flat, train=True)
-                l, dout = eng.loss(out, batch.y, self._loss_kind(), want_grad=True, loss_scale=1.0 / self.world)
-                eng.backward(dout, flat, grads=self.grads)
+                l, dout = self._forward_loss(eng, xs, batch, flat)
+                eng.backward(dout, flat, grads=self.grads, head_done=dout is None)
                 static_loss.copy_(l)
             self._graphs[key] = (g, static_loss, batch, flat.numel(), dev)
             return loss
```

Result: no change. 5.605 million, median of 6 (+0.8%).
